# tiangexiang/OccNeRF

Hardware: AMD Instinct MI355X
Metric: rays/sec at 512x512x128spp, random-init ckpt (higher is better)
Workload: dtype f32; 1 GPU; BASELINE configs[1]: free-view frame, 512x512 image, 128 samples/ray, non-rigid motion on, seeded random-init checkpoint; synthetic SMPL-like body and camera; 183784 rays hit the body bbox (ray_mask); H2D of the ray batch and the prior and D2H of [R,5] inside the step; the frame's rays sharded over the ranks; samples whose motion-weight sum is exactly 0 are dropped after the warp (bit-identical pi; rays_per_frame=183784, samples_per_ray=128, skip_empty_samples=True, dedup_repeated_samples=False, knn_center_cache=True, warp_bone_culling=True, world_size_formed=1

## Files before the change

### include/occnerf_hip.h

```cpp
#ifndef OCCNERF_HIP_H
#define OCCNERF_HIP_H

#include <stdint.h>

#ifdef __cplusplus
extern "C" {
#endif

#define OCCNERF_ABI_VERSION 5

int occnerf_abi_version(void);
const char *occnerf_last_error(void);

int occnerf_experiment_knob(const char *name, int value);


int occnerf_grid_encode_forward(const float *inputs, const float *embeddings,
                                const int32_t *offsets, float *outputs, uint32_t B, uint32_t D,
                                uint32_t C, uint32_t L, float S, uint32_t H, float *dy_dx,
                                uint32_t gridtype, int align_corners, uint32_t interp,
                                void *stream);

int occnerf_grid_encode_backward(const float *grad, const float *inputs, const float *embeddings,
                                 const int32_t *offsets, float *grad_embeddings, uint32_t B,
                                 uint32_t D, uint32_t C, uint32_t L, float S, uint32_t H,
                                 const float *dy_dx, float *grad_inputs, uint32_t gridtype,
                                 int align_corners, uint32_t interp, void *stream);

int occnerf_grid_encode_forward_h(const float *inputs, const float *embeddings, const int32_t *offsets,
                                  const int32_t *h_offsets, float *outputs, uint32_t B, uint32_t D, uint32_t C, uint32_t L,
                                  float S, uint32_t H, float *dy_dx, uint32_t gridtype, int align_corners,
                                  uint32_t interp, void *stream);

int occnerf_grid_grad_runs(const float *grad_rows, const float *inputs, int64_t B, uint32_t D, uint32_t L, uint32_t C,
                           float *grad, void *stream);

int occnerf_grid_encode_backward_h(const float *grad, const float *inputs, const float *embeddings,
                                   const int32_t *offsets, const int32_t *h_offsets, float *grad_embeddings,
                                   uint32_t B, uint32_t D, uint32_t C, uint32_t L, float S, uint32_t H,
                                   const float *dy_dx, float *grad_inputs, uint32_t gridtype, int align_corners,
                                   uint32_t interp, void *scratch, int64_t scratch_bytes, void *stream);

int occnerf_grid_encode_forward_f16(const float *inputs, const void *embeddings, const int32_t *offsets, void *outputs,
                                    uint32_t B, uint32_t D, uint32_t C, uint32_t L, float S, uint32_t H, void *dy_dx,
                                    uint32_t gridtype, int align_corners, uint32_t interp, void *stream);
int occnerf_grid_encode_backward_f16(const void *grad, const float *inputs, const void *embeddings, const int32_t *offsets,
                                     void *grad_embeddings, uint32_t B, uint32_t D, uint32_t C, uint32_t L, float S,
                                     uint32_t H, const void *dy_dx, void *grad_inputs, uint32_t gridtype, int align_corners,
                                     uint32_t interp, void *stream);

int occnerf_grid_encode_forward_f64(const float *inputs, const double *embeddings, const int32_t *offsets, double *outputs,
                                    uint32_t B, uint32_t D, uint32_t C, uint32_t L, float S, uint32_t H, double *dy_dx,
                                    uint32_t gridtype, int align_corners, uint32_t interp, void *stream);
int occnerf_grid_encode_backward_f64(const double *grad, const float *inputs, const double *embeddings, const int32_t *offsets,
                                     double *grad_embeddings, uint32_t B, uint32_t D, uint32_t C, uint32_t L, float S,
                                     uint32_t H, const double *dy_dx, double *grad_inputs, uint32_t gridtype, int align_corners,
                                     uint32_t interp, void *stream);

int occnerf_grad_total_variation(const float *inputs, const float *embeddings, float *grad,
                                 const int32_t *offsets, float weight, uint32_t B, uint32_t D,
                                 uint32_t C, uint32_t L, float S, uint32_t H, uint32_t gridtype,
                                 int align_corners, void *stream);


int occnerf_sample_warp(const float *rays, int64_t n, int32_t S, const float *t_vals,
                        const float *t_rand, const float *Rs, const float *Ts, const float *vol,
                        int32_t nb, int32_t G, const float *h_bbox_min, const float *h_bbox_scale,
                        float *z_vals, float *pts, float *x_skel, float *mask, void *stream);
int occnerf_bone_boxes(const float *vol, int32_t nb, int32_t G, int32_t *boxes, void *stream);
int occnerf_sample_warp_culled(const float *rays, int64_t n, int32_t S, const float *t_vals,
                               const float *Rs, const float *Ts, const float *vol, int32_t nb, int32_t G,
                               const int32_t *boxes, const float *h_bbox_min, const float *h_bbox_scale,
                               float *z_vals, float *x_skel, float *mask, void *stream);

int64_t occnerf_ray_order_temp_bytes(int64_t R);
int occnerf_ray_order(const float *dirs, int64_t R, int64_t stride, int64_t *order, void *temp, int64_t temp_bytes,
                      void *stream);

int occnerf_gen_rays(const double *h_Kinv, const double *h_R, const double *h_T, int32_t f32_camera,
                     int32_t H, int32_t W, const double *h_bbox_min, const double *h_bbox_max, float *rays8,
                     uint8_t *mask, void *stream);

int64_t occnerf_nonrigid_packed_floats(void);
int occnerf_nonrigid_pack(const float *const *h_W, const float *const *h_b, float *packed,
                          void *stream);
int occnerf_nonrigid(const float *xyz_in, int64_t N, const float *cond, const float *h_hann,
                     const float *W0, const float *b0, float *packed, float *xyz_out,
                     void *stream);
int occnerf_nonrigid_rows(float *xyz, int64_t N_max, const int32_t *rows, const int32_t *n_dev,
                          const float *cond, const float *h_hann, const float *W0, const float *b0,
                          float *packed, void *stream);
int occnerf_nonrigid_direct(const float *xyz_in, int64_t N, const float *cond, const float *h_hann,
                            const float *W0, const float *b0, float *packed, float *xyz_out,
                            void *stream);

int64_t occnerf_nonrigid_packed_bf16_bytes(void);
int occnerf_nonrigid_pack_bf16(const float *const *h_W, void *packed_bf16, void *stream);
int occnerf_nonrigid_bf16x3(const float *xyz_in, int64_t N, const float *cond, const float *h_hann,
                            const float *W0, const float *b0, float *packed, const void *packed_bf16,
                            float *xyz_out, void *stream);
int occnerf_nonrigid_bf16x3_rows(float *xyz, int64_t N_max, const int32_t *rows, const int32_t *n_dev,
                                 const float *cond, const float *h_hann, const float *W0, const float *b0,
                                 float *packed, const void *packed_bf16, void *stream);

int occnerf_msknn(const float *xyz, int64_t N, const float *points, const int32_t *index_map,
                  const int32_t *h_scale_begin, const int32_t *h_seed_from_coarser,
                  int32_t nscale, int32_t *knn_idxs, void *stream);

int occnerf_msknn_clustered(const float *xyz, const float *mask, int64_t n_rays, int32_t samples_per_ray,
                            const float *points, const float *centers,
                            const int32_t *cluster_ranges, const float *cluster_radius, int32_t ncl,
                            const float *group_centers, const int32_t *group_ranges, const float *group_radius, int32_t ngrp,
                            const int32_t *h_coarse_rows, const int32_t *h_seed_from_coarser,
                            int32_t nscale, const int32_t *query_rows, const int32_t *n_query_dev, int32_t *ray_start,
                            int32_t *knn_idxs, void *stream);
int occnerf_knn_center(const float *c, const float *points, const int32_t *index_map, const int32_t *h_scale_begin,
                       int32_t nscale, float *center_out, int32_t *idx_out, void *stream);
int occnerf_msknn_clustered_centered(const float *xyz, const float *mask, int64_t n_rays, int32_t samples_per_ray,
                                     const float *points, const float *centers,
                                     const int32_t *cluster_ranges, const float *cluster_radius, int32_t ncl,
                                     const float *group_centers, const int32_t *group_ranges, const float *group_radius, int32_t ngrp,
                                     const int32_t *h_coarse_rows, const int32_t *h_seed_from_coarser,
                                     int32_t nscale, const int32_t *query_rows, const int32_t *n_query_dev, int32_t *ray_start,
                                     const float *center, const int32_t *center_idx, int32_t *knn_idxs, void *stream);

int occnerf_knn_small(const float *q, int32_t nq, const float *s, int32_t ns, int32_t k,
                      int32_t *idx, void *stream);

int occnerf_unit_normals(const double *normals, int32_t P, double *unit, void *stream);

int occnerf_point_sdf(const float *point_cloud, const float *point_base, const double *normals,
                      const double *unit_normals, const int32_t *kidx, int32_t P,
                      double *knn_base, float *dist, void *stream);

int occnerf_point_sdf_backward(const float *point_cloud, const float *point_base, const double *normals,
                               const double *unit_normals, const int32_t *kidx, int32_t P, const double *d_knn_base,
                               const float *d_dist, float *d_point_dist, void *stream);
int32_t occnerf_point_table_stride(void);
int occnerf_point_table(const double *knn_base, const float *point_sdf, const float *learnable,
                        int32_t P, float bound, float two_bound, const float *embeddings,
                        const int32_t *offsets, const int32_t *h_offsets, uint32_t L, float S,
                        uint32_t H, float *table, void *stream);

int occnerf_point_pack(const float *point_base, const double *normals, const double *unit_normals,
                       const float *counter, const float *table, int32_t P, float *point_geo,
                       float *point_tail, void *stream);
int occnerf_sample_features(const float *xyz, int64_t N, const int32_t *knn_idxs, int32_t nscale,
                            const float *point_base, const double *normals,
                            const double *unit_normals, const float *counter,
                            const float *table, float bound, float two_bound,
                            const float *embeddings, const int32_t *offsets,
                            const int32_t *h_offsets, uint32_t L, float S, uint32_t H,
                            const int32_t *geo_idxs, const float *att_in, const int32_t *rows,
                            const int32_t *n_dev, const float *point_geo, const float *point_tail, int32_t P,
                            float *mlp_in, float *raw, float *enc_in, void *stream);
int occnerf_sample_features_centered(const float *xyz, int64_t N, const int32_t *knn_idxs, int32_t nscale,
                            const float *point_base, const double *normals,
                            const double *unit_normals, const float *counter,
                            const float *table, float bound, float two_bound,
                            const float *embeddings, const int32_t *offsets,
                            const int32_t *h_offsets, uint32_t L, float S, uint32_t H,
                            const int32_t *geo_idxs, const float *att_in, const int32_t *rows,
                            const int32_t *n_dev, const float *point_geo, const float *point_tail, int32_t P,
                            const float *center, const float *center_agg,
                                     float *mlp_in, float *raw, float *enc_in, void *stream);

int occnerf_agg_forward(const float *feats, int32_t F, const int32_t *knn, const float *atts, int64_t N, int32_t K,
                        float *agg, void *stream);
int32_t occnerf_agg_backward_slices(int64_t N);
int64_t occnerf_agg_backward_scratch_bytes(int64_t N, int32_t F);
int occnerf_agg_backward(const float *grad_agg, int32_t F, const int32_t *knn, const float *atts, int64_t N,
                         int32_t K, int32_t P, float *partial, void *scratch, int64_t scratch_bytes, void *stream);

int64_t occnerf_live_rows_temp_bytes(int64_t N);
int occnerf_live_rows(const float *mask, int64_t N, int32_t *rows, int32_t *count, void *temp,
                      int64_t temp_bytes, void *stream);
int occnerf_scatter_raw(const float *raw_c, const int32_t *rows, const int32_t *n_dev, int64_t N_max,
                        float *raw_full, void *stream);

int64_t occnerf_repeat_heads_temp_bytes(int64_t N_max);
int occnerf_repeat_heads(const void *keys, int64_t stride_dwords, int32_t key_dwords, const int32_t *rows,
                         const int32_t *n_dev, int64_t N_max, int32_t *scan, int32_t *heads, int32_t *head_count,
                         float *head_mask, void *temp, int64_t temp_bytes, void *stream);
int64_t occnerf_unique_heads_temp_bytes(int64_t cap);
int occnerf_unique_heads(const void *keys, int64_t stride_dwords, int32_t key_dwords, const int32_t *heads,
                         const int32_t *n_dev, int64_t cap, int32_t *heads_out, int32_t *count_out, int32_t *scan,
                         const int32_t *n_scan_dev, int64_t scan_cap, void *temp, int64_t temp_bytes, void *stream);
int occnerf_scatter_raw_heads(const float *raw_h, const float *raw_c, const int32_t *rows, const int32_t *n_dev,
                              const int32_t *scanA, const int32_t *scanB, int64_t N_max, float *raw_full, void *stream);
int occnerf_canonical_mlp_rows(const float *mlp_in, const int32_t *in_rows, int64_t N_max, const int32_t *n_dev,
                               const float *packed, float *raw, void *stream);

int64_t occnerf_canonical_mlp_packed_floats(void);
int occnerf_canonical_mlp_pack(const float *const *h_W, const float *const *h_b, float *packed,
                               void *stream);

int occnerf_canonical_mlp(const float *mlp_in, int64_t N, const float *packed, float *raw,
                          void *stream);
int occnerf_canonical_mlp_direct(const float *mlp_in, int64_t N, const float *packed, float *raw,
                                 void *stream);
int occnerf_canonical_mlp_counted(const float *mlp_in, int64_t N_max, const int32_t *n_dev,
                                  const float *packed, float *raw, void *stream);

int64_t occnerf_canonical_mlp_packed_bf16_bytes(void);
int occnerf_canonical_mlp_pack_bf16(const float *const *h_W, void *packed_bf16, void *stream);
int occnerf_canonical_mlp_bf16x3(const float *mlp_in, int64_t N, const float *packed,
                                 const void *packed_bf16, float *raw, int32_t variant,
                                 void *stream);
int occnerf_canonical_mlp_bf16x3_rows(const float *mlp_in, const int32_t *in_rows, int64_t N_max,
                                      const int32_t *n_dev, const float *packed, const void *packed_bf16,
                                      float *raw, int32_t variant, void *stream);

int occnerf_canonical_mlp_pack_f16(const float *const *h_W, void *packed_f16, void *stream);
int occnerf_canonical_mlp_f16x3(const float *mlp_in, const int32_t *in_rows, int64_t N_max, const int32_t *n_dev,
                                const float *packed, const void *packed_f16, float *raw, uint32_t *domain_flag,
                                void *stream);
int occnerf_nonrigid_pack_f16(const float *const *h_W, void *packed_f16, void *stream);
int occnerf_nonrigid_f16x3(const float *xyz_in, int64_t N_max, const int32_t *rows, const int32_t *n_dev,
                           const float *cond, const float *h_hann, const float *W0, const float *b0, float *packed,
                           const void *packed_f16, float *xyz_out, uint32_t *domain_flag, void *stream);

int occnerf_composite(const float *raw, const float *mask, const float *z_vals, const float *rays,
                      const float *h_bgcolor, int64_t n, int32_t S, float *rgb, float *acc,
                      float *depth, float *weights, int32_t *term, const int64_t *out_rows, void *stream);


int occnerf_linear_pack(const float *W, const float *b, int32_t out_dim, int32_t in_dim, const int32_t *row_map,
                        int32_t n_pad, const int32_t *col_map, int32_t k_pad, int32_t bf16, void *Wp, void *Wt,
                        float *bias_p, void *stream);
int occnerf_linear_forward(const void *x0, int64_t ld0, int32_t k0, const void *x1, int64_t ld1, int32_t k1,
                           const void *W, const float *bias, int32_t relu, const void *mask, int64_t ldm, void *y,
                           int64_t ldy, int32_t out_f32, int32_t n_store, float *aux, int32_t aux_col,
                           int64_t aux_stride, int64_t M, int32_t n_pad, int32_t bf16, void *stream);
int32_t occnerf_linear_wgrad_slices(int64_t M);
int occnerf_linear_wgrad(const void *dz, int64_t lddz, int32_t n_pad, const void *x, int64_t ldx, int32_t k_pad,
                         int64_t M, int32_t bf16, float *part, float *dbpart, void *stream);
int occnerf_linear_wgrad_reduce(const float *part, const float *dbpart, int32_t G, int32_t n_pad, int32_t k_pad,
                                const int32_t *row_map, const int32_t *col_map, float *dW, int32_t in_dim, float *db,
                                int32_t accumulate, void *stream);

int64_t occnerf_trunks_packed_bytes(void);
int occnerf_trunks_pack_bf16(const float *const *h_W, void *packed, void *stream);
int occnerf_trunks_forward_bf16(const float *agg, const float *var, const float *enc, int64_t M, const float *packed_f32,
                                const void *packed_bf16, void *X0, void *const *h_A, void *GEO, void *const *h_B, float *raw4,
                                void *stream);

int occnerf_composite_backward(const float *raw, const float *mask, const float *z_vals, const float *rays,
                               const float *h_bgcolor, int64_t n, int32_t S, const float *g_rgb, const float *g_acc,
                               const float *g_depth, float *d_raw, float *d_mask, void *stream);

int32_t occnerf_warp_backward_slices(int64_t n_samples);
int occnerf_warp_backward(const float *rays, int64_t n, int32_t S, const float *z_vals, const float *g_mask,
                          const float *Rs, const float *Ts, const float *vol, int32_t nb, int32_t G,
                          const float *h_bbox_min, const float *h_bbox_scale, float *d_vol_part, float *d_rt_part,
                          void *stream);

int occnerf_agg_weights(const float *counter, const int32_t *knn, int64_t N, int32_t K, float *atts, float *var,
                        void *stream);

int occnerf_pose_motion_bases_backward(const float *const *h_W, const float *const *h_b, const float *posevec,
                                       const float *dst_Rs, const float *dst_Ts, const float *cnl_gtfms,
                                       const float *dRs, const float *dTs, float *const *h_dW, float *const *h_db,
                                       void *stream);

int occnerf_pose_motion_bases(const float *const *h_W, const float *const *h_b, const float *posevec, int32_t refine,
                              const float *dst_Rs, const float *dst_Ts, const float *cnl_gtfms, float *Rs, float *Ts,
                              void *stream);
int occnerf_prior_softmax(const float *decoded, const float *prior, int32_t C, int64_t V, float *vol, void *stream);
int occnerf_pack_rays(const float *rays, const float *near, const float *far, const int64_t *order, int64_t R, float *rays8,
                      void *stream);

int occnerf_assemble_image(const float *rgb, const float *alpha, const int64_t *ray_index, int64_t R, int32_t height,
                           int32_t width, const float *h_bgcolor01, uint8_t *out_rgb, uint8_t *out_alpha, void *stream);

int occnerf_convt3d_col2im(const float *cols, const float *bias, int32_t Cout, int32_t D, int32_t H, int32_t W,
                           float *out, void *stream);
int occnerf_convt3d_im2col(const float *gy, int32_t Cout, int32_t D, int32_t H, int32_t W, float *dcols, void *stream);

int32_t occnerf_adam_table_row_bytes(void);
int occnerf_adam_step(const void *table, int32_t n_tensors, const int32_t *chunks, int32_t n_chunks,
                      int32_t chunk_elems, double beta1, double beta2, double eps, double max_grad_norm, float *scratch,
                      void *stream);

int64_t occnerf_lpips_packed_floats(void);
int64_t occnerf_lpips_workspace_floats(int32_t N, int32_t H, int32_t W);
int occnerf_lpips_pack(const float *const *h_conv_w, const float *const *h_conv_b, const float *const *h_lin,
                       const float *shift, const float *scale, float *packed, void *stream);
int occnerf_lpips_forward(const float *packed, const float *in0, const float *in1, int32_t N, int32_t H, int32_t W,
                          int32_t in_nhwc, float *work, float *val, float *res, void *stream);
int occnerf_lpips_backward(const float *packed, float *work, int32_t N, int32_t H, int32_t W, int32_t in_nhwc,
                           const float *gres, float *d_in0, float *d_in1, void *stream);

int occnerf_patch_assemble(const float *rgb, const int32_t *row_of_pix, int64_t R, int32_t n_patches, int32_t size,
                           const float *h_bgcolor01, float *img, void *stream);
int occnerf_patch_assemble_backward(const float *d_img, const int32_t *pix_of_row, int64_t R, float *d_rgb, void *stream);

int32_t occnerf_patch_batch_max_patches(void);
int occnerf_patch_batch(const uint8_t *image, const uint8_t *alpha, const float *rays8, const uint8_t *box_mask, int32_t H,
                        int32_t W, int32_t n_patches, int32_t size, const double *h_u, double subject_ratio,
                        const float *h_bgcolor, int32_t *row_counts, float *rays, float *near, float *far, float *target_rgbs,
                        float *target_patches, uint8_t *patch_masks, int32_t *patch_div_indices, int32_t *xy_min,
                        int32_t *pix_of_row, int32_t *row_of_pix, int32_t *n_rows, void *stream);

int occnerf_whole_frame_count(const uint8_t *box_mask, int32_t H, int32_t W, int32_t *row_start, void *stream);
int occnerf_whole_frame_gather(const uint8_t *image, const uint8_t *alpha, const float *rays8, const uint8_t *box_mask,
                               int32_t H, int32_t W, const float *h_bgcolor, const int32_t *row_start, int32_t R,
                               int64_t *ray_index, float *rays, float *near, float *far, float *target_rgbs,
                               double *ray_alpha, uint8_t *truth_u8, float *gt_vis, float *gt_alpha, void *stream);

int occnerf_view_frame_gather(const float *rays8, const uint8_t *box_mask, int32_t H, int32_t W, const int32_t *row_start,
                              int32_t R, int64_t *ray_index, float *rays, float *near, float *far, void *stream);

#define OCCNERF_FRAME_METRICS_RECORD 14
int64_t occnerf_frame_metrics_workspace_bytes(int32_t N, int32_t H, int32_t W);
int occnerf_frame_metrics(const uint8_t *pred, const uint8_t *truth, const float *alpha, const uint8_t *body,
                          const float *gt_vis_alpha, const float *gt_alpha, int32_t N, int32_t H, int32_t W,
                          double data_range, double *record, double *ssim_map, void *workspace, void *stream);

#ifdef __cplusplus
}
#endif
#endif
```

### occnerf_amd/_lib.py

```python
import ctypes as C
import os

_HERE = os.path.dirname(os.path.abspath(__file__))
LIB_PATH = os.environ.get('OCCNERF_HIP_LIB') or os.path.join(_HERE, 'liboccnerf_hip.so')

ABI_VERSION = 5

_vp, _i32, _i64, _u32, _f32 = C.c_void_p, C.c_int32, C.c_int64, C.c_uint32, C.c_float

SIGNATURES = {
    'occnerf_abi_version': (C.c_int, []),
    'occnerf_last_error': (C.c_char_p, []),
    'occnerf_experiment_knob': (C.c_int, [C.c_char_p, C.c_int]),
    'occnerf_grid_encode_forward': (C.c_int, [_vp, _vp, _vp, _vp, _u32, _u32, _u32, _u32, _f32, _u32,
                                               _vp, _u32, C.c_int, _u32, _vp]),
    'occnerf_grid_encode_backward': (C.c_int, [_vp, _vp, _vp, _vp, _vp, _u32, _u32, _u32, _u32, _f32,
                                                _u32, _vp, _vp, _u32, C.c_int, _u32, _vp]),
    'occnerf_grid_grad_runs': (C.c_int, [_vp, _vp, _i64, _u32, _u32, _u32, _vp, _vp]),
    'occnerf_grid_encode_forward_h': (C.c_int, [_vp, _vp, _vp, _vp, _vp, _u32, _u32, _u32, _u32, _f32, _u32,
                                                 _vp, _u32, C.c_int, _u32, _vp]),
    'occnerf_grid_encode_backward_h': (C.c_int, [_vp, _vp, _vp, _vp, _vp, _vp, _u32, _u32, _u32, _u32, _f32,
                                                  _u32, _vp, _vp, _u32, C.c_int, _u32, _vp, _i64, _vp]),
    'occnerf_grid_encode_forward_f16': (C.c_int, [_vp, _vp, _vp, _vp, _u32, _u32, _u32, _u32, _f32, _u32,
                                                   _vp, _u32, C.c_int, _u32, _vp]),
    'occnerf_grid_encode_backward_f16': (C.c_int, [_vp, _vp, _vp, _vp, _vp, _u32, _u32, _u32, _u32, _f32,
                                                    _u32, _vp, _vp, _u32, C.c_int, _u32, _vp]),
    'occnerf_grid_encode_forward_f64': (C.c_int, [_vp, _vp, _vp, _vp, _u32, _u32, _u32, _u32, _f32, _u32,
                                                   _vp, _u32, C.c_int, _u32, _vp]),
    'occnerf_grid_encode_backward_f64': (C.c_int, [_vp, _vp, _vp, _vp, _vp, _u32, _u32, _u32, _u32, _f32,
                                                    _u32, _vp, _vp, _u32, C.c_int, _u32, _vp]),
    'occnerf_trunks_packed_bytes': (_i64, []),
    'occnerf_trunks_pack_bf16': (C.c_int, [_vp, _vp, _vp]),
    'occnerf_trunks_forward_bf16': (C.c_int, [_vp, _vp, _vp, _i64, _vp, _vp, _vp, _vp, _vp, _vp, _vp, _vp]),
    'occnerf_grad_total_variation': (C.c_int, [_vp, _vp, _vp, _vp, _f32, _u32, _u32, _u32, _u32, _f32,
                                                _u32, _u32, C.c_int, _vp]),
    'occnerf_sample_warp': (C.c_int, [_vp, _i64, _i32, _vp, _vp, _vp, _vp, _vp, _i32, _i32, _vp, _vp,
                                       _vp, _vp, _vp, _vp, _vp]),
    'occnerf_bone_boxes': (C.c_int, [_vp, _i32, _i32, _vp, _vp]),
    'occnerf_sample_warp_culled': (C.c_int, [_vp, _i64, _i32, _vp, _vp, _vp, _vp, _i32, _i32, _vp, _vp, _vp, _vp, _vp, _vp, _vp]),
    'occnerf_nonrigid_packed_floats': (_i64, []),
    'occnerf_nonrigid_pack': (C.c_int, [_vp, _vp, _vp, _vp]),
    'occnerf_nonrigid': (C.c_int, [_vp, _i64, _vp, _vp, _vp, _vp, _vp, _vp, _vp]),
    'occnerf_nonrigid_direct': (C.c_int, [_vp, _i64, _vp, _vp, _vp, _vp, _vp, _vp, _vp]),
    'occnerf_nonrigid_packed_bf16_bytes': (_i64, []),
    'occnerf_nonrigid_pack_bf16': (C.c_int, [_vp, _vp, _vp]),
    'occnerf_nonrigid_bf16x3': (C.c_int, [_vp, _i64, _vp, _vp, _vp, _vp, _vp, _vp, _vp, _vp]),
    'occnerf_nonrigid_bf16x3_rows': (C.c_int, [_vp, _i64, _vp, _vp, _vp, _vp, _vp, _vp, _vp, _vp, _vp]),
    'occnerf_msknn': (C.c_int, [_vp, _i64, _vp, _vp, _vp, _vp, _i32, _vp, _vp]),
    'occnerf_msknn_clustered': (C.c_int, [_vp, _vp, _i64, _i32, _vp, _vp, _vp, _vp, _i32, _vp, _vp, _vp, _i32, _vp, _vp, _i32,
                                           _vp, _vp, _vp, _vp, _vp]),
    'occnerf_msknn_clustered_centered': (C.c_int, [_vp, _vp, _i64, _i32, _vp, _vp, _vp, _vp, _i32, _vp, _vp, _vp, _i32, _vp, _vp, _i32,
                                           _vp, _vp, _vp, _vp, _vp, _vp, _vp]),
    'occnerf_knn_center': (C.c_int, [_vp, _vp, _vp, _vp, _i32, _vp, _vp, _vp]),
    'occnerf_knn_small': (C.c_int, [_vp, _i32, _vp, _i32, _i32, _vp, _vp]),
    'occnerf_unit_normals': (C.c_int, [_vp, _i32, _vp, _vp]),
    'occnerf_point_sdf': (C.c_int, [_vp, _vp, _vp, _vp, _vp, _i32, _vp, _vp, _vp]),
    'occnerf_ray_order_temp_bytes': (_i64, [_i64]),
    'occnerf_ray_order': (C.c_int, [_vp, _i64, _i64, _vp, _vp, _i64, _vp]),
    'occnerf_point_sdf_backward': (C.c_int, [_vp, _vp, _vp, _vp, _vp, _i32, _vp, _vp, _vp, _vp]),
    'occnerf_gen_rays': (C.c_int, [_vp, _vp, _vp, _i32, _i32, _i32, _vp, _vp, _vp, _vp, _vp]),
    'occnerf_agg_forward': (C.c_int, [_vp, _i32, _vp, _vp, _i64, _i32, _vp, _vp]),
    'occnerf_agg_backward_slices': (_i32, [_i64]),
    'occnerf_agg_backward_scratch_bytes': (_i64, [_i64, _i32]),
    'occnerf_agg_backward': (C.c_int, [_vp, _i32, _vp, _vp, _i64, _i32, _i32, _vp, _vp, _i64, _vp]),
    'occnerf_live_rows_temp_bytes': (_i64, [_i64]),
    'occnerf_live_rows': (C.c_int, [_vp, _i64, _vp, _vp, _vp, _i64, _vp]),
    'occnerf_scatter_raw': (C.c_int, [_vp, _vp, _vp, _i64, _vp, _vp]),
    'occnerf_repeat_heads_temp_bytes': (_i64, [_i64]),
    'occnerf_repeat_heads': (C.c_int, [_vp, _i64, _i32, _vp, _vp, _i64, _vp, _vp, _vp, _vp, _vp, _i64, _vp]),
    'occnerf_unique_heads_temp_bytes': (_i64, [_i64]),
    'occnerf_unique_heads': (C.c_int, [_vp, _i64, _i32, _vp, _vp, _i64, _vp, _vp, _vp, _vp, _i64, _vp, _i64, _vp]),
    'occnerf_scatter_raw_heads': (C.c_int, [_vp, _vp, _vp, _vp, _vp, _vp, _i64, _vp, _vp]),
    'occnerf_canonical_mlp_rows': (C.c_int, [_vp, _vp, _i64, _vp, _vp, _vp, _vp]),
    'occnerf_canonical_mlp_counted': (C.c_int, [_vp, _i64, _vp, _vp, _vp, _vp]),
    'occnerf_nonrigid_rows': (C.c_int, [_vp, _i64, _vp, _vp, _vp, _vp, _vp, _vp, _vp, _vp]),
    'occnerf_point_table_stride': (_i32, []),
    'occnerf_point_table': (C.c_int, [_vp, _vp, _vp, _i32, _f32, _f32, _vp, _vp, _vp, _u32, _f32, _u32, _vp,
                                       _vp]),
    'occnerf_point_pack': (C.c_int, [_vp, _vp, _vp, _vp, _vp, _i32, _vp, _vp, _vp]),
    'occnerf_sample_features': (C.c_int, [_vp, _i64, _vp, _i32, _vp, _vp, _vp, _vp, _vp, _f32, _f32, _vp,
                                           _vp, _vp, _u32, _f32, _u32, _vp, _vp, _vp, _vp, _vp, _vp, _i32, _vp, _vp,
                                           _vp, _vp]),
    'occnerf_sample_features_centered': (C.c_int, [_vp, _i64, _vp, _i32, _vp, _vp, _vp, _vp, _vp, _f32, _f32, _vp,
                                                    _vp, _vp, _u32, _f32, _u32, _vp, _vp, _vp, _vp, _vp, _vp, _i32, _vp, _vp,
                                                    _vp, _vp, _vp, _vp]),
    'occnerf_canonical_mlp_packed_floats': (_i64, []),
    'occnerf_canonical_mlp_pack': (C.c_int, [_vp, _vp, _vp, _vp]),
    'occnerf_canonical_mlp': (C.c_int, [_vp, _i64, _vp, _vp, _vp]),
    'occnerf_canonical_mlp_direct': (C.c_int, [_vp, _i64, _vp, _vp, _vp]),
    'occnerf_canonical_mlp_packed_bf16_bytes': (_i64, []),
    'occnerf_canonical_mlp_pack_bf16': (C.c_int, [_vp, _vp, _vp]),
    'occnerf_canonical_mlp_bf16x3': (C.c_int, [_vp, _i64, _vp, _vp, _vp, _i32, _vp]),
    'occnerf_canonical_mlp_pack_f16': (C.c_int, [_vp, _vp, _vp]),
    'occnerf_canonical_mlp_f16x3': (C.c_int, [_vp, _vp, _i64, _vp, _vp, _vp, _vp, _vp, _vp]),
    'occnerf_nonrigid_pack_f16': (C.c_int, [_vp, _vp, _vp]),
    'occnerf_nonrigid_f16x3': (C.c_int, [_vp, _i64, _vp, _vp, _vp, _vp, _vp, _vp, _vp, _vp, _vp, _vp, _vp]),
    'occnerf_canonical_mlp_bf16x3_rows': (C.c_int, [_vp, _vp, _i64, _vp, _vp, _vp, _vp, _i32, _vp]),
    'occnerf_composite': (C.c_int, [_vp, _vp, _vp, _vp, _vp, _i64, _i32, _vp, _vp, _vp, _vp, _vp, _vp, _vp]),
    'occnerf_linear_pack': (C.c_int, [_vp, _vp, _i32, _i32, _vp, _i32, _vp, _i32, _i32, _vp, _vp, _vp, _vp]),
    'occnerf_linear_forward': (C.c_int, [_vp, _i64, _i32, _vp, _i64, _i32, _vp, _vp, _i32, _vp, _i64, _vp, _i64, _i32,
                                          _i32, _vp, _i32, _i64, _i64, _i32, _i32, _vp]),
    'occnerf_linear_wgrad_slices': (_i32, [_i64]),
    'occnerf_linear_wgrad': (C.c_int, [_vp, _i64, _i32, _vp, _i64, _i32, _i64, _i32, _vp, _vp, _vp]),
    'occnerf_linear_wgrad_reduce': (C.c_int, [_vp, _vp, _i32, _i32, _i32, _vp, _vp, _vp, _i32, _vp, _i32, _vp]),
    'occnerf_composite_backward': (C.c_int, [_vp, _vp, _vp, _vp, _vp, _i64, _i32, _vp, _vp, _vp, _vp, _vp, _vp]),
    'occnerf_warp_backward_slices': (_i32, [_i64]),
    'occnerf_warp_backward': (C.c_int, [_vp, _i64, _i32, _vp, _vp, _vp, _vp, _vp, _i32, _i32, _vp, _vp, _vp, _vp, _vp]),
    'occnerf_agg_weights': (C.c_int, [_vp, _vp, _i64, _i32, _vp, _vp, _vp]),
    'occnerf_pose_motion_bases': (C.c_int, [_vp, _vp, _vp, _i32, _vp, _vp, _vp, _vp, _vp, _vp]),
    'occnerf_pose_motion_bases_backward': (C.c_int, [_vp, _vp, _vp, _vp, _vp, _vp, _vp, _vp, _vp, _vp, _vp]),
    'occnerf_prior_softmax': (C.c_int, [_vp, _vp, _i32, _i64, _vp, _vp]),
    'occnerf_pack_rays': (C.c_int, [_vp, _vp, _vp, _vp, _i64, _vp, _vp]),
    'occnerf_assemble_image': (C.c_int, [_vp, _vp, _vp, _i64, _i32, _i32, _vp, _vp, _vp, _vp]),
    'occnerf_convt3d_col2im': (C.c_int, [_vp, _vp, _i32, _i32, _i32, _i32, _vp, _vp]),
    'occnerf_convt3d_im2col': (C.c_int, [_vp, _i32, _i32, _i32, _i32, _vp, _vp]),
    'occnerf_adam_table_row_bytes': (_i32, []),
    'occnerf_adam_step': (C.c_int, [_vp, _i32, _vp, _i32, _i32] + [C.c_double] * 4 + [_vp, _vp]),
    'occnerf_lpips_packed_floats': (_i64, []),
    'occnerf_lpips_workspace_floats': (_i64, [_i32, _i32, _i32]),
    'occnerf_lpips_pack': (C.c_int, [_vp, _vp, _vp, _vp, _vp, _vp, _vp]),
    'occnerf_lpips_forward': (C.c_int, [_vp, _vp, _vp, _i32, _i32, _i32, _i32, _vp, _vp, _vp, _vp]),
    'occnerf_lpips_backward': (C.c_int, [_vp, _vp, _i32, _i32, _i32, _i32, _vp, _vp, _vp, _vp]),
    'occnerf_patch_assemble': (C.c_int, [_vp, _vp, _i64, _i32, _i32, _vp, _vp, _vp]),
    'occnerf_patch_assemble_backward': (C.c_int, [_vp, _vp, _i64, _vp, _vp]),
    'occnerf_patch_batch_max_patches': (_i32, []),
    'occnerf_patch_batch': (C.c_int, [_vp, _vp, _vp, _vp, _i32, _i32, _i32, _i32, _vp, C.c_double, _vp] + [_vp] * 12 + [_vp]),
    'occnerf_whole_frame_count': (C.c_int, [_vp, _i32, _i32, _vp, _vp]),
    'occnerf_whole_frame_gather': (C.c_int, [_vp, _vp, _vp, _vp, _i32, _i32, _vp, _vp, _i32] + [_vp] * 9 + [_vp]),
    'occnerf_view_frame_gather': (C.c_int, [_vp, _vp, _i32, _i32, _vp, _i32, _vp, _vp, _vp, _vp, _vp]),
    'occnerf_frame_metrics_workspace_bytes': (_i64, [_i32, _i32, _i32]),
    'occnerf_frame_metrics': (C.c_int, [_vp, _vp, _vp, _vp, _vp, _vp, _i32, _i32, _i32, C.c_double, _vp, _vp, _vp, _vp]),
}

_lib = None


def lib():
    global _lib
    if _lib is None:
        if not os.path.exists(LIB_PATH):
            raise ImportError(
                f'{LIB_PATH} not found: the gfx950 kernels are not built. Run '
                '`python -c "import __graft_entry__ as g; g.build()"` (or `make -C '
                'occnerf_amd/csrc`). There is no CPU fallback for this path.')
        import torch
        handle = C.CDLL(LIB_PATH)
        for name, (res, args) in SIGNATURES.items():
            fn = getattr(handle, name)
            fn.restype, fn.argtypes = res, args
        if handle.occnerf_abi_version() != ABI_VERSION:
            raise ImportError(f'liboccnerf_hip.so: ABI version {handle.occnerf_abi_version()}, this binding was written '
                              f'for {ABI_VERSION} (include/occnerf_hip.h OCCNERF_ABI_VERSION): rebuild the library')
        _lib = handle
    return _lib


def check(rc, what):
    if rc != 0:
        msg = lib().occnerf_last_error().decode(errors='replace')
        raise RuntimeError(f'{what} failed ({rc}): {msg}')
```

### occnerf_amd/config.py

```python
import argparse
import ast
import copy
import os

import yaml


class CfgNode(dict):
    def __getattr__(self, k):
        try:
            return self[k]
        except KeyError:
            raise AttributeError(k)

    def __setattr__(self, k, v):
        self[k] = v

    def get(self, k, default=None):
        return dict.get(self, k, default)

    @staticmethod
    def wrap(d):
        if isinstance(d, dict) and not isinstance(d, CfgNode):
            return CfgNode({k: CfgNode.wrap(v) for k, v in d.items()})
        return d

    def merge(self, other):
        for k, v in other.items():
            if isinstance(v, dict) and isinstance(self.get(k), dict):
                self[k].merge(v)
            else:
                self[k] = CfgNode.wrap(copy.deepcopy(v))
        return self

    def merge_from_file(self, path):
        with open(path) as f:
            return self.merge(yaml.safe_load(f) or {})

    def merge_from_list(self, opts):
        assert len(opts) % 2 == 0, 'opts must be KEY VALUE pairs'
        for key, val in zip(opts[0::2], opts[1::2]):
            node = self
            parts = key.split('.')
            for p in parts[:-1]:
                node = node[p]
            try:
                val = ast.literal_eval(val)
            except (ValueError, SyntaxError):
                pass
            node[parts[-1]] = val
        return self

    def clone(self):
        return CfgNode.wrap(copy.deepcopy(dict(self)))


_DEFAULTS = {
    'category': 'occnerf', 'task': 'zju_mocap', 'subject': 'p387', 'experiment': 'occnerf',
    'resume': False, 'eval_iter': 10000000, 'render_folder_name': '',
    'ignore_non_rigid_motions': False, 'render_skip': 1, 'render_frames': 100, 'num_workers': 4,
    'network_module': 'core.nets.occnerf.network',
    'embedder': {'module': 'core.nets.occnerf.embedders.fourier'},
    'non_rigid_embedder': {'module': 'core.nets.occnerf.embedders.hannw_fourier'},
    'canonical_mlp': {'module': 'core.nets.occnerf.canonical_mlps.occnerf_mlp', 'mlp_depth': 4,
                      'mlp_width': 256, 'multires': 10, 'i_embed': 0},
    'mweight_volume': {'module': 'core.nets.occnerf.mweight_vol_decoders.deconv_vol_decoder',
                       'embedding_size': 256, 'volume_size': 32, 'dst_voxel_size': 0.0625},
    'non_rigid_motion_mlp': {'module': 'core.nets.occnerf.non_rigid_motion_mlps.mlp_offset',
                             'condition_code_size': 69, 'mlp_width': 128, 'mlp_depth': 6,
                             'skips': [4], 'multires': 6, 'i_embed': 0, 'kick_in_iter': 100000,
                             'full_band_iter': 200000},
    'pose_decoder': {'module': 'core.nets.occnerf.pose_decoders.mlp_delta_body_pose',
                     'embedding_size': 69, 'mlp_width': 256, 'mlp_depth': 4,
                     'kick_in_iter': 2000000},
    'sex': 'neutral', 'total_bones': 24, 'bbox_offset': 0.3, 'load_net': 'latest',
    'N_samples': 128, 'perturb': 1.0, 'netchunk_per_gpu': 300000, 'chunk': 32768, 'n_gpus': 1,
    'bgcolor': [0.0, 0.0, 0.0], 'resize_img_scale': 0.5, 'show_alpha': False, 'show_truth': False,
    'patch': {'sample_subject_ratio': 0.8, 'N_patches': 6, 'size': 32},
    'freeview': {'frame_idx': 0, 'src_type': 'zju_mocap'}, 'tpose': {}, 'movement': {},
    'train': {'dataset_path': None, 'images_prescaled': False, 'seed': 0, 'prefetch': True},
    'occlude': False, 'occlusion': {'range': 405, 'mid': 451, 'width': 86},
    'eval': {'lpips': False, 'lpips_model_path': None, 'lpips_vgg16_path': None},
    'smpl_model': 'auto',
    'max_samples_per_pass': 1 << 28,
    'mlp_precision': 'fp32',
    'f16x3_domain_check': True,
    'train_fused_trunks': True,
    'skip_empty_samples': True,
    'device_rays': True,
    'device_frames': True,
    'ray_patch_order': True,
    'knn_culling': True,
    'knn_center_cache': True,
    'warp_bone_culling': True,
}

_cfg = None


def default_cfg():
    return CfgNode.wrap(copy.deepcopy(_DEFAULTS))


def get_cfg():
    global _cfg
    if _cfg is None:
        _cfg = default_cfg()
        _finish(_cfg)
    return _cfg


def set_cfg(cfg):
    global _cfg
    _cfg = cfg
    return cfg


def _finish(cfg):
    import torch
    cfg.logdir = os.path.join('experiments', cfg.category, cfg.task, cfg.subject, cfg.experiment)
    n = torch.cuda.device_count()
    cfg.n_gpus = n
    cfg.primary_gpus = [0] if n > 0 else ['cpu']
    cfg.secondary_gpus = ([g for g in range(n) if g != 0] or cfg.primary_gpus) if n > 1 \
        else cfg.primary_gpus


def make_cfg(argv=None):
    parser = argparse.ArgumentParser()
    parser.add_argument('--cfg', required=True, type=str)
    parser.add_argument('--eval', default='full', type=str)
    parser.add_argument('--type', default='skip', type=str)
    parser.add_argument('opts', default=None, nargs=argparse.REMAINDER)
    args = parser.parse_args(argv)
    cfg = default_cfg()
    here = os.path.dirname(os.path.dirname(os.path.abspath(__file__)))
    default_yaml = os.path.join(here, 'configs', 'default.yaml')
    if os.path.exists(default_yaml):
        cfg.merge_from_file(default_yaml)
    cfg.merge_from_file(args.cfg)
    cfg.merge_from_list(args.opts or [])
    _finish(cfg)
    set_cfg(cfg)
    return cfg, args
```

### occnerf_amd/csrc/common.h

```cpp
#pragma once

#include <hip/hip_runtime.h>
#include <stdint.h>

#include <cstdio>
#include <cstring>

#include "../../include/occnerf_hip.h"

#define OCC_API extern "C" __attribute__((visibility("default")))

namespace occ {

constexpr int kWave = 64;
constexpr int kNumCU = 256;

void set_error(const char *fmt, ...);

inline hipStream_t as_stream(void *s) { return reinterpret_cast<hipStream_t>(s); }

inline int check_launch(const char *what) {
    hipError_t e = hipGetLastError();
    if (e != hipSuccess) {
        set_error("%s: %s", what, hipGetErrorString(e));
        return 2;
    }
    return 0;
}

enum Knob : int { kKnobAggSlices = 0, kKnobGridXcd = 1, kKnobCount = 2 };
int knob(Knob k);

#define OCC_REQUIRE(cond, ...)         \
    do {                               \
        if (!(cond)) {                 \
            occ::set_error(__VA_ARGS__); \
            return 1;                  \
        }                              \
    } while (0)

template <typename T>
__device__ __forceinline__ T ld32(const T *base, uint32_t byte_off) {
    return *reinterpret_cast<const T *>(reinterpret_cast<const char *>(base) + byte_off);
}

constexpr int kMaxLevels = 16;

struct GridLevels {
    float scale[kMaxLevels];
    uint32_t resolution[kMaxLevels];
};

enum GridIndexMode : uint32_t { kGridDense = 0, kGridHashPow2 = 1, kGridGeneric = 2 };
struct GridModes4 {
    uint32_t mode[kMaxLevels];
};
GridModes4 make_grid_modes_d4(uint32_t L, const GridLevels &lv, const uint32_t *h_level_sizes);

GridLevels make_grid_levels(uint32_t L, float S, uint32_t H);

template <uint32_t D>
__device__ __forceinline__ uint32_t grid_index(uint32_t gridtype, bool align_corners,
                                               uint32_t hashmap_size, uint32_t resolution,
                                               const uint32_t (&pos_grid)[D]) {
    constexpr uint32_t primes[7] = {1u,          2654435761u, 805459861u, 3674653429u,
                                    2097192037u, 1434869437u, 2165219737u};
    uint32_t stride = 1, index = 0;
#pragma unroll
    for (uint32_t d = 0; d < D; d++) {
        if (stride <= hashmap_size) {
            index += pos_grid[d] * stride;
            stride *= align_corners ? resolution : (resolution + 1);
        }
    }
    if (gridtype == 0 && stride > hashmap_size) {
        uint32_t h = 0;
#pragma unroll
        for (uint32_t d = 0; d < D; d++) h ^= pos_grid[d] * primes[d];
        index = h;
    }
    return index % hashmap_size;
}

struct LevelTaps4 {
    float fr[4];
    float2 v[16];
};
__device__ __forceinline__ void encode_level_d4c2_taps(const float (&x)[4], const float2 *grid,
                                                       uint32_t hashmap_size, float scale, uint32_t resolution,
                                                       uint32_t mode, uint32_t entry0, LevelTaps4 &tp) {
    uint32_t pg[4];
#pragma unroll
    for (int d = 0; d < 4; d++) {
        float pos = __fmaf_rn(x[d], scale, 0.5f);
        const float fl = floorf(pos);
        pg[d] = (uint32_t)fl;
        pos -= fl;
        tp.fr[d] = pos;
    }
    uint32_t t[4][2];
    if (mode == kGridDense) {
        uint32_t stride = 1;
#pragma unroll
        for (int d = 0; d < 4; d++) {
            t[d][0] = pg[d] * stride;
            t[d][1] = (pg[d] + 1) * stride;
            stride *= resolution + 1;
        }
    } else if (mode == kGridHashPow2) {
        constexpr uint32_t primes[4] = {1u, 2654435761u, 805459861u, 3674653429u};
#pragma unroll
        for (int d = 0; d < 4; d++) {
            t[d][0] = pg[d] * primes[d];
            t[d][1] = (pg[d] + 1) * primes[d];
        }
    }
#pragma unroll
    for (uint32_t idx = 0; idx < 16; idx++) {
        const int b0 = idx & 1, b1 = (idx >> 1) & 1, b2 = (idx >> 2) & 1, b3 = (idx >> 3) & 1;
        uint32_t index;
        if (mode == kGridDense) {
            index = t[0][b0] + t[1][b1] + t[2][b2] + t[3][b3];
        } else if (mode == kGridHashPow2) {
            index = (t[0][b0] ^ t[1][b1] ^ t[2][b2] ^ t[3][b3]) & (hashmap_size - 1);
        } else {
            const uint32_t pl[4] = {pg[0] + b0, pg[1] + b1, pg[2] + b2, pg[3] + b3};
            index = grid_index<4>(0, false, hashmap_size, resolution, pl);
        }
        tp.v[idx] = ld32(grid, (entry0 + index) * 8u);
    }
}
__device__ __forceinline__ float2 encode_level_d4c2_reduce(const LevelTaps4 &tp) {
    float f[4][2];
#pragma unroll
    for (int d = 0; d < 4; d++) {
        f[d][0] = __fsub_rn(1.f, tp.fr[d]);
        f[d][1] = tp.fr[d];
    }
    float2 r = make_float2(0.f, 0.f);
    float w01[4];
#pragma unroll
    for (int i = 0; i < 4; i++) w01[i] = __fmul_rn(f[0][i & 1], f[1][i >> 1]);
#pragma unroll
    for (uint32_t idx = 0; idx < 16; idx++) {
        const int b0 = idx & 1, b1 = (idx >> 1) & 1, b2 = (idx >> 2) & 1, b3 = (idx >> 3) & 1;
        const float w = __fmul_rn(__fmul_rn(w01[b0 | (b1 << 1)], f[2][b2]), f[3][b3]);
        r.x = __fmaf_rn(w, tp.v[idx].x, r.x);
        r.y = __fmaf_rn(w, tp.v[idx].y, r.y);
    }
    return r;
}
__device__ __forceinline__ float2 encode_level_d4c2(const float (&x)[4], const float2 *grid,
                                                    uint32_t hashmap_size, float scale,
                                                    uint32_t resolution, uint32_t mode, uint32_t entry0 = 0) {
    LevelTaps4 tp;
    encode_level_d4c2_taps(x, grid, hashmap_size, scale, resolution, mode, entry0, tp);
    return encode_level_d4c2_reduce(tp);
}

__device__ __forceinline__ float norm3(float x, float y, float z) {
    return sqrtf(__fmaf_rn(z, z, __fmaf_rn(y, y, __fmul_rn(x, x))));
}

int64_t mlp_lds_packed_floats();
int mlp_lds_pack(const float *const *h_W, const float *const *h_b, float *packed, hipStream_t st);
int mlp_lds_launch(const float *mlp_in, const int32_t *in_rows, int64_t N, const int32_t *n_dev, const float *packed,
                   float *raw, hipStream_t st);

int64_t nr_lds_packed_floats();
int nr_lds_pack(const float *const *h_W, const float *const *h_b, float *packed, hipStream_t st);
int nr_lds_launch(const float *xyz_in, int64_t N, const int32_t *rows, const int32_t *n_dev, const float *cond,
                  const float *h_hann, const float *W0, const float *b0, float *packed, float *xyz_out,
                  hipStream_t st);

}
```

### occnerf_amd/csrc/compact.hip

```cpp
#include "common.h"

#include <hipcub/hipcub.hpp>

namespace occ {

struct LivePredicate {
    const float *mask;
    __device__ bool operator()(const int &i) const { return mask[i] != 0.0f; }
};

__global__ void scatter_raw_kernel(const float *__restrict__ raw_c, const int32_t *__restrict__ rows,
                                   const int32_t *__restrict__ n_dev, float *__restrict__ raw_full) {
    const int64_t m = (int64_t)blockIdx.x * blockDim.x + threadIdx.x;
    if (m >= (int64_t)*n_dev) return;
    const int64_t n = rows[m];
#pragma unroll
    for (int c = 0; c < 5; c++) raw_full[n * 5 + c] = raw_c[m * 5 + c];
}

struct RepeatFlag {
    const uint32_t *keys;
    int64_t stride;
    int K;
    const int32_t *rows;
    const int32_t *n_dev;
    __device__ int operator()(const int &m) const {
        if (m >= *n_dev) return 0;
        if (m == 0) return 1;
        const uint32_t *a = keys + (rows ? (int64_t)rows[m] : (int64_t)m) * stride;
        const uint32_t *b = keys + (rows ? (int64_t)rows[m - 1] : (int64_t)(m - 1)) * stride;
        if (((K | (int)stride) & 3) == 0) {
            for (int k = 0; k < K; k += 4) {
                const uint4 x = *reinterpret_cast<const uint4 *>(a + k), y = *reinterpret_cast<const uint4 *>(b + k);
                if (x.x != y.x || x.y != y.y || x.z != y.z || x.w != y.w) return 1;
            }
            return 0;
        }
        for (int k = 0; k < K; k++)
            if (a[k] != b[k]) return 1;
        return 0;
    }
};

__global__ void repeat_flags_wide_kernel(const uint4 *__restrict__ keys, int64_t stride4, int K4,
                                         const int32_t *__restrict__ rows, const int32_t *__restrict__ n_dev,
                                         int64_t N_max, int32_t *__restrict__ flags) {
    const int g = threadIdx.x & 7;
    const int64_t m = ((int64_t)blockIdx.x * blockDim.x + threadIdx.x) >> 3;
    if (m >= N_max) return;
    const int64_t n = *n_dev;
    int diff = 0;
    if (m < n && m > 0) {
        const uint4 *a = keys + (rows ? (int64_t)rows[m] : m) * stride4;
        const uint4 *b = keys + (rows ? (int64_t)rows[m - 1] : m - 1) * stride4;
        for (int k = g; k < K4; k += 8) {
            const uint4 x = a[k], y = b[k];
            diff |= (x.x != y.x) | (x.y != y.y) | (x.z != y.z) | (x.w != y.w);
        }
    }
    diff |= __shfl_xor(diff, 1, 8);
    diff |= __shfl_xor(diff, 2, 8);
    diff |= __shfl_xor(diff, 4, 8);
    if (g == 0) flags[m] = m >= n ? 0 : (m == 0 ? 1 : diff);
}

__global__ void repeat_heads_kernel(const int32_t *__restrict__ scan, const int32_t *__restrict__ rows,
                                    const int32_t *__restrict__ n_dev, int32_t *__restrict__ heads,
                                    int32_t *__restrict__ head_count, float *__restrict__ head_mask) {
    const int64_t m = (int64_t)blockIdx.x * blockDim.x + threadIdx.x;
    const int64_t n = *n_dev;
    if (m == 0 && n <= 0) *head_count = 0;
    if (m >= n) return;
    const int32_t s = scan[m], prev = m ? scan[m - 1] : 0;
    if (s != prev) {
        const int32_t r = rows ? rows[m] : (int32_t)m;
        heads[s - 1] = r;
        if (head_mask) head_mask[r] = 1.0f;
    }
    if (m == n - 1) *head_count = s;
}

__global__ void scatter_raw_heads_kernel(const float *__restrict__ raw_h, const float *__restrict__ raw_c,
                                         const int32_t *__restrict__ rows, const int32_t *__restrict__ n_dev,
                                         const int32_t *__restrict__ scanA, const int32_t *__restrict__ scanB,
                                         float *__restrict__ raw_full) {
    const int64_t m = (int64_t)blockIdx.x * blockDim.x + threadIdx.x;
    if (m >= (int64_t)*n_dev) return;
    const int64_t n = rows[m];
    const int64_t a = scanA ? scanA[m] - 1 : m;
    const int64_t h = scanB ? scanB[a] - 1 : a;
#pragma unroll
    for (int c = 0; c < 4; c++) raw_full[n * 5 + c] = raw_h[h * 5 + c];
    raw_full[n * 5 + 4] = raw_c[a * 5 + 4];
}

__device__ __forceinline__ uint64_t mix64(uint64_t h) {
    h ^= h >> 33;
    h *= 0xff51afd7ed558ccdull;
    h ^= h >> 33;
    h *= 0xc4ceb9fe1a85ec53ull;
    h ^= h >> 33;
    return h;
}

template <int G >
__global__ void unique_insert_kernel(const uint32_t *__restrict__ keys, int64_t stride, int K,
                                     const int32_t *__restrict__ heads, const int32_t *__restrict__ n_dev,
                                     int32_t *__restrict__ table, uint32_t tmask, int32_t *__restrict__ rep) {
    const int g = threadIdx.x % G;
    const int64_t j = ((int64_t)blockIdx.x * blockDim.x + threadIdx.x) / G;
    if (j >= (int64_t)*n_dev) return;
    const uint32_t *a = keys + (heads ? (int64_t)heads[j] : j) * stride;
    uint64_t h = 0x9E3779B97F4A7C15ull * (uint64_t)(g + 1);
    for (int k = g; k < K; k += G) h = mix64(h ^ ((uint64_t)a[k] + ((uint64_t)(k + 1) << 32)));
    if (G > 1) {
        h ^= __shfl_xor(h, 1, G);
        h ^= __shfl_xor(h, 2, G);
        h ^= __shfl_xor(h, 4, G);
    }
    uint32_t slot = (uint32_t)mix64(h) & tmask;
    int32_t r = (int32_t)j;
    for (int probe = 0; probe < 32; probe++) {
        int32_t prev = 0;
        if (g == 0) prev = atomicCAS(&table[slot], -1, (int32_t)j);
        if (G > 1) prev = __shfl(prev, 0, G);
        if (prev == -1) break;
        const uint32_t *b = keys + (heads ? (int64_t)heads[prev] : (int64_t)prev) * stride;
        int diff = 0;
        for (int k = g; k < K; k += G) diff |= a[k] != b[k];
        if (G > 1) {
            diff |= __shfl_xor(diff, 1, G);
            diff |= __shfl_xor(diff, 2, G);
            diff |= __shfl_xor(diff, 4, G);
        }
        if (!diff) {
            r = prev;
            break;
        }
        slot = (slot + 1) & tmask;
    }
    if (g == 0) rep[j] = r;
}

struct IsRepresentative {
    const int32_t *rep, *n_dev;
    __device__ int operator()(const int &j) const { return j < *n_dev && rep[j] == j; }
};

__global__ void unique_finish_kernel(const int32_t *__restrict__ heads, const int32_t *__restrict__ n_dev,
                                     const int32_t *__restrict__ scan2, int32_t *__restrict__ rep,
                                     int32_t *__restrict__ heads_out, int32_t *__restrict__ count_out) {
    const int64_t j = (int64_t)blockIdx.x * blockDim.x + threadIdx.x;
    const int64_t n = *n_dev;
    if (j == 0 && n <= 0) *count_out = 0;
    if (j >= n) return;
    const int32_t r = rep[j];
    if (r == (int32_t)j) heads_out[scan2[j] - 1] = heads ? heads[j] : (int32_t)j;
    if (j == n - 1) *count_out = scan2[j];
    rep[j] = scan2[r] - 1;
}

__global__ void unique_remap_kernel(int32_t *__restrict__ scan, const int32_t *__restrict__ n_scan_dev,
// ... 2 lines not shown
    if (m >= (int64_t)*n_scan_dev) return;
    scan[m] = pos[scan[m] - 1] + 1;
}

}

OCC_API int64_t occnerf_repeat_heads_temp_bytes(int64_t N) {
    using namespace occ;
    if (N <= 0 || N >= (1ll << 31)) return 0;
    size_t bytes = 0;
    hipcub::CountingInputIterator<int> it(0);
    hipcub::TransformInputIterator<int, RepeatFlag, hipcub::CountingInputIterator<int>> flags(it, RepeatFlag{});
    if (hipcub::DeviceScan::InclusiveSum(nullptr, bytes, flags, (int *)nullptr, (int)N, (hipStream_t)0) != hipSuccess)
        return -1;
    size_t bytes2 = 0;
    if (hipcub::DeviceScan::InclusiveSum(nullptr, bytes2, (int *)nullptr, (int *)nullptr, (int)N, (hipStream_t)0) != hipSuccess)
        return -1;
    return (int64_t)(bytes > bytes2 ? bytes : bytes2);
}

OCC_API int occnerf_repeat_heads(const void *keys, int64_t stride_dwords, int32_t key_dwords, const int32_t *rows,
                                 const int32_t *n_dev, int64_t N_max, int32_t *scan, int32_t *heads,
                                 int32_t *head_count, float *head_mask, void *temp, int64_t temp_bytes,
                                 void *stream) {
    using namespace occ;
    OCC_REQUIRE(keys && n_dev && scan && heads && head_count && temp, "repeat_heads: null argument");
    OCC_REQUIRE(N_max > 0 && N_max < (1ll << 31), "repeat_heads: N=%lld out of range", (long long)N_max);
    OCC_REQUIRE(key_dwords > 0 && stride_dwords >= key_dwords, "repeat_heads: key of %d dwords in rows of %lld",
                key_dwords, (long long)stride_dwords);
    size_t bytes = (size_t)temp_bytes;
    hipError_t e;
    if (key_dwords >= 32 && ((key_dwords | stride_dwords) & 3) == 0) {
        const int64_t fblocks = (N_max * 8 + 255) / 256;
        OCC_REQUIRE(fblocks < (1ll << 31), "repeat_heads: N too large");
        hipLaunchKernelGGL(repeat_flags_wide_kernel, dim3((unsigned)fblocks), dim3(256), 0, as_stream(stream),
                           reinterpret_cast<const uint4 *>(keys), stride_dwords / 4, key_dwords / 4, rows, n_dev, N_max, scan);
        e = hipcub::DeviceScan::InclusiveSum(temp, bytes, scan, scan, (int)N_max, as_stream(stream));
    } else {
        hipcub::CountingInputIterator<int> it(0);
        hipcub::TransformInputIterator<int, RepeatFlag, hipcub::CountingInputIterator<int>> flags(
            it, RepeatFlag{reinterpret_cast<const uint32_t *>(keys), stride_dwords, key_dwords, rows, n_dev});
        e = hipcub::DeviceScan::InclusiveSum(temp, bytes, flags, scan, (int)N_max, as_stream(stream));
    }
    OCC_REQUIRE(e == hipSuccess, "repeat_heads: %s", hipGetErrorString(e));
    const int64_t blocks = (N_max + 255) / 256;
    hipLaunchKernelGGL(repeat_heads_kernel, dim3((unsigned)blocks), dim3(256), 0, as_stream(stream), scan, rows, n_dev,
                       heads, head_count, head_mask);
    return check_launch("repeat_heads");
}

static inline int64_t unique_table_entries(int64_t cap) {
    int64_t t = 1024;
    while (t < cap) t <<= 1;
    return t;
}

OCC_API int64_t occnerf_unique_heads_temp_bytes(int64_t cap) {
    using namespace occ;
    if (cap <= 0 || cap >= (1ll << 30)) return 0;
    size_t bytes = 0;
    hipcub::CountingInputIterator<int> it(0);
    hipcub::TransformInputIterator<int, IsRepresentative, hipcub::CountingInputIterator<int>> flags(it, IsRepresentative{});
    if (hipcub::DeviceScan::InclusiveSum(nullptr, bytes, flags, (int *)nullptr, (int)cap, (hipStream_t)0) != hipSuccess)
        return -1;
    const int64_t words = unique_table_entries(cap) + 2 * ((cap + 63) & ~63ll);
    return words * 4 + (int64_t)((bytes + 255) & ~(size_t)255);
}

OCC_API int occnerf_unique_heads(const void *keys, int64_t stride_dwords, int32_t key_dwords, const int32_t *heads,
                                 const int32_t *n_dev, int64_t cap, int32_t *heads_out, int32_t *count_out,
                                 int32_t *scan, const int32_t *n_scan_dev, int64_t scan_cap, void *temp,
                                 int64_t temp_bytes, void *stream) {
    using namespace occ;
    OCC_REQUIRE(keys && n_dev && heads_out && count_out && temp, "unique_heads: null argument");
    OCC_REQUIRE(cap > 0 && cap < (1ll << 30), "unique_heads: cap=%lld out of range", (long long)cap);
    OCC_REQUIRE(key_dwords > 0 && stride_dwords >= key_dwords, "unique_heads: key of %d dwords in rows of %lld", key_dwords,
                (long long)stride_dwords);
    OCC_REQUIRE(!scan == !n_scan_dev, "unique_heads: scan and its length come together");
    OCC_REQUIRE(temp_bytes >= occnerf_unique_heads_temp_bytes(cap), "unique_heads: temp too small");
    const int64_t T = unique_table_entries(cap), capr = (cap + 63) & ~63ll;
    int32_t *table = reinterpret_cast<int32_t *>(temp), *rep = table + T, *scan2 = rep + capr;
    void *cub_temp = scan2 + capr;
    size_t cub_bytes = (size_t)temp_bytes - (size_t)(T + 2 * capr) * 4;
    hipStream_t st = as_stream(stream);
    OCC_REQUIRE(hipMemsetAsync(table, 0xFF, (size_t)T * 4, st) == hipSuccess, "unique_heads: memset");
    const uint32_t *k32 = reinterpret_cast<const uint32_t *>(keys);
    if (key_dwords >= 32)
        hipLaunchKernelGGL(unique_insert_kernel<8>, dim3((unsigned)((cap * 8 + 255) / 256)), dim3(256), 0, st, k32,
                           stride_dwords, key_dwords, heads, n_dev, table, (uint32_t)(T - 1), rep);
    else
        hipLaunchKernelGGL(unique_insert_kernel<1>, dim3((unsigned)((cap + 255) / 256)), dim3(256), 0, st, k32,
                           stride_dwords, key_dwords, heads, n_dev, table, (uint32_t)(T - 1), rep);
    hipcub::CountingInputIterator<int> it(0);
    hipcub::TransformInputIterator<int, IsRepresentative, hipcub::CountingInputIterator<int>> flags(
        it, IsRepresentative{rep, n_dev});
    const hipError_t e = hipcub::DeviceScan::InclusiveSum(cub_temp, cub_bytes, flags, scan2, (int)cap, st);
    OCC_REQUIRE(e == hipSuccess, "unique_heads: %s", hipGetErrorString(e));
    hipLaunchKernelGGL(unique_finish_kernel, dim3((unsigned)((cap + 255) / 256)), dim3(256), 0, st, heads, n_dev, scan2, rep,
                       heads_out, count_out);
    if (scan)
        hipLaunchKernelGGL(unique_remap_kernel, dim3((unsigned)((scan_cap + 255) / 256)), dim3(256), 0, st, scan, n_scan_dev,
                           rep);
    return check_launch("unique_heads");
}

OCC_API int occnerf_scatter_raw_heads(const float *raw_h, const float *raw_c, const int32_t *rows, const int32_t *n_dev,
                                      const int32_t *scanA, const int32_t *scanB, int64_t N_max, float *raw_full,
                                      void *stream) {
    using namespace occ;
    if (N_max <= 0) return 0;
    OCC_REQUIRE(raw_h && raw_c && rows && n_dev && raw_full, "scatter_raw_heads: null argument");
    const int64_t blocks = (N_max + 255) / 256;
    OCC_REQUIRE(blocks < (1ll << 31), "scatter_raw_heads: N too large");
    hipLaunchKernelGGL(scatter_raw_heads_kernel, dim3((unsigned)blocks), dim3(256), 0, as_stream(stream), raw_h, raw_c,
                       rows, n_dev, scanA, scanB, raw_full);
    return check_launch("scatter_raw_heads");
}

OCC_API int64_t occnerf_live_rows_temp_bytes(int64_t N) {
    using namespace occ;
    if (N <= 0 || N >= (1ll << 31)) return 0;
    size_t bytes = 0;
    hipcub::CountingInputIterator<int> it(0);
    if (hipcub::DeviceSelect::If(nullptr, bytes, it, (int *)nullptr, (int *)nullptr, (int)N, LivePredicate{nullptr},
                                 (hipStream_t)0) != hipSuccess)
        return -1;
    return (int64_t)bytes;
}

OCC_API int occnerf_live_rows(const float *mask, int64_t N, int32_t *rows, int32_t *count, void *temp,
                              int64_t temp_bytes, void *stream) {
    using namespace occ;
    OCC_REQUIRE(mask && rows && count && temp, "live_rows: null argument");
    OCC_REQUIRE(N > 0 && N < (1ll << 31), "live_rows: N=%lld out of range", (long long)N);
    size_t bytes = (size_t)temp_bytes;
    hipcub::CountingInputIterator<int> it(0);
    const hipError_t e = hipcub::DeviceSelect::If(temp, bytes, it, rows, count, (int)N, LivePredicate{mask},
                                                  as_stream(stream));
    OCC_REQUIRE(e == hipSuccess, "live_rows: %s", hipGetErrorString(e));
    return check_launch("live_rows");
}

OCC_API int occnerf_scatter_raw(const float *raw_c, const int32_t *rows, const int32_t *n_dev, int64_t N_max,
                                float *raw_full, void *stream) {
    using namespace occ;
    if (N_max <= 0) return 0;
    OCC_REQUIRE(raw_c && rows && n_dev && raw_full, "scatter_raw: null argument");
    const int64_t blocks = (N_max + 255) / 256;
    OCC_REQUIRE(blocks < (1ll << 31), "scatter_raw: N too large");
    hipLaunchKernelGGL(scatter_raw_kernel, dim3((unsigned)blocks), dim3(256), 0, as_stream(stream), raw_c, rows, n_dev,
                       raw_full);
    return check_launch("scatter_raw");
}
```

### occnerf_amd/csrc/features.hip

```cpp
#include "common.h"

#include <cstdlib>

namespace occ {

constexpr int kKnn = 10;
constexpr int kTableCols = 36;
constexpr int kTableStride = 64;

__device__ __forceinline__ double cos3_unit(const float (&a)[3], const double *__restrict__ un) {
    float na = norm3(a[0], a[1], a[2]);
    na = na < 1e-8f ? 1e-8f : na;
    const double t0 = __dmul_rn((double)__fdiv_rn(a[0], na), un[0]);
    const double t1 = __dmul_rn((double)__fdiv_rn(a[1], na), un[1]);
    const double t2 = __dmul_rn((double)__fdiv_rn(a[2], na), un[2]);
    return __dadd_rn(__dadd_rn(t0, t1), t2);
}

__global__ void unit_normals_kernel(const double *__restrict__ normals, int P,
                                    double *__restrict__ unit) {
    const int i = blockIdx.x * blockDim.x + threadIdx.x;
    if (i >= P) return;
    const double b0 = normals[i * 3], b1 = normals[i * 3 + 1], b2 = normals[i * 3 + 2];
    double nb = __dsqrt_rn(__dadd_rn(__dadd_rn(__dmul_rn(b0, b0), __dmul_rn(b1, b1)), __dmul_rn(b2, b2)));
// ... 218 lines not shown
            }
        }
        float dist = __fdiv_rn(dsum, (float)kKnn);
        if (2 * neg > kKnn) dist = -dist;
        float nd = __fdiv_rn(__fadd_rn(dist, 0.2f), 0.5f);
        nd = nd < 0.0f ? 0.0f : (nd > 1.0f ? 1.0f : nd);
        float x[4];
#pragma unroll
        for (int c = 0; c < 3; c++) x[c] = (float)__ddiv_rn(num[c], den);
        x[3] = nd;
        if (enc_in_out) {
#pragma unroll
            for (int c = 0; c < 4; c++) enc_in_out[i * 4 + c] = x[c];
        }
        raw[i * 5 + 4] = dist;

        float *out = mlp_in + i * 68;

        bool oob = false;
#pragma unroll
        for (int d = 0; d < 4; d++) oob |= (x[d] < 0.f || x[d] > 1.f);
        for (int l = 0; l < prm.L; l++) {
            float2 v = make_float2(0.f, 0.f);
            if (!oob) {
                const uint32_t o0 = (uint32_t)offsets[l];
                v = encode_level_d4c2(x, embeddings + o0, (uint32_t)offsets[l + 1] - o0,
                                      lv.scale[l], lv.resolution[l], gm.mode[l]);
            }
            *reinterpret_cast<float2 *>(out + 36 + l * 2) = v;
        }

        float att[4 * kKnn];
        float amin = INFINITY;
#pragma unroll
        for (int j = 0; j < 4 * kKnn; j++) {
            att[j] = j < nk ? (att_in ? att_in[i * nk + j] : counter[id[j]]) : INFINITY;
            amin = fminf(amin, att[j]);
        }
        float amax = -INFINITY;
#pragma unroll
        for (int j = 0; j < 4 * kKnn; j++) {
            if (j < nk) {
                att[j] = __fadd_rn(att[j], __fsub_rn(1.0f, amin));
                amax = fmaxf(amax, att[j]);
            }
        }
        float mean = 0.0f;
#pragma unroll
        for (int j = 0; j < 4 * kKnn; j++) {
            if (j < nk) {
                att[j] = __fdiv_rn(att[j], amax);
                mean = __fadd_rn(mean, att[j]);
            }
        }
        mean = __fdiv_rn(mean, (float)nk);
        float var = 0.0f, smax = -INFINITY;
#pragma unroll
        for (int j = 0; j < 4 * kKnn; j++) {
            if (j < nk) {
                const float dlt = __fsub_rn(att[j], mean);
                var = __fadd_rn(var, __fmul_rn(dlt, dlt));
                smax = fmaxf(smax, att[j]);
            }
        }
        var = __fdiv_rn(var, (float)(nk - 1));
        float ssum = 0.0f;
#pragma unroll
        for (int j = 0; j < 4 * kKnn; j++) {
            if (j < nk) {
                att[j] = expf(__fsub_rn(att[j], smax));
                ssum = __fadd_rn(ssum, att[j]);
            }
        }
        float agg[kTableCols];
#pragma unroll
        for (int f = 0; f < kTableCols; f++) agg[f] = 0.0f;
#pragma unroll
        for (int j = 0; j < 4 * kKnn; j++) {
            if (j < nk) {
                const float a = __fdiv_rn(att[j], ssum);
                const float4 *row = table + (size_t)id[j] * (kTableStride / 4);
#pragma unroll
                for (int v = 0; v < kTableCols / 4; v++) {
                    const float4 t = row[v];
                    agg[v * 4 + 0] = __fadd_rn(agg[v * 4 + 0], __fmul_rn(a, t.x));
                    agg[v * 4 + 1] = __fadd_rn(agg[v * 4 + 1], __fmul_rn(a, t.y));
                    agg[v * 4 + 2] = __fadd_rn(agg[v * 4 + 2], __fmul_rn(a, t.z));
                    agg[v * 4 + 3] = __fadd_rn(agg[v * 4 + 3], __fmul_rn(a, t.w));
                }
            }
        }
        agg[35] = var;
#pragma unroll
        for (int v = 0; v < kTableCols / 4; v++)
            *reinterpret_cast<float4 *>(out + v * 4) =
                make_float4(agg[v * 4], agg[v * 4 + 1], agg[v * 4 + 2], agg[v * 4 + 3]);
    }
}


__global__ void point_pack_kernel(const float *__restrict__ point_base, const double *__restrict__ normals,
                                  const double *__restrict__ unit, const float *__restrict__ counter,
                                  const float *__restrict__ table, int P, float *__restrict__ geo,
                                  float4 *__restrict__ tailc) {
    const int i = blockIdx.x * blockDim.x + threadIdx.x;
    if (i >= P) return;
    float *r = geo + (size_t)i * 16;
    r[0] = point_base[i * 3], r[1] = point_base[i * 3 + 1], r[2] = point_base[i * 3 + 2], r[3] = 0.0f;
    double *d = reinterpret_cast<double *>(r + 4);
    d[0] = normals[i * 3], d[1] = normals[i * 3 + 1], d[2] = normals[i * 3 + 2];
    d[3] = unit[i * 3], d[4] = unit[i * 3 + 1], d[5] = unit[i * 3 + 2];
    const float *t = table + (size_t)i * kTableStride + 32;
    tailc[i] = make_float4(t[0], t[1], t[2], counter[i]);
}

__device__ __forceinline__ float grp_sum8(float v) {
    v += __shfl_xor(v, 1, 8);
    v += __shfl_xor(v, 2, 8);
    v += __shfl_xor(v, 4, 8);
    return v;
}
__device__ __forceinline__ float grp_min8(float v) {
    v = fminf(v, __shfl_xor(v, 1, 8));
    v = fminf(v, __shfl_xor(v, 2, 8));
    return fminf(v, __shfl_xor(v, 4, 8));
}
__device__ __forceinline__ float grp_max8(float v) {
    v = fmaxf(v, __shfl_xor(v, 1, 8));
    v = fmaxf(v, __shfl_xor(v, 2, 8));
    return fmaxf(v, __shfl_xor(v, 4, 8));
}

template <int Q>
__device__ __forceinline__ float quad_bcast(float v) {
    return __builtin_bit_cast(float, __builtin_amdgcn_mov_dpp(__builtin_bit_cast(int, v), Q * 0x55, 0xf, 0xf, true));
}
template <int Q>
__device__ __forceinline__ double quad_bcast_f64(float lo, float hi) {
    return __hiloint2double(__builtin_amdgcn_mov_dpp(__builtin_bit_cast(int, hi), Q * 0x55, 0xf, 0xf, true),
                            __builtin_amdgcn_mov_dpp(__builtin_bit_cast(int, lo), Q * 0x55, 0xf, 0xf, true));
}

constexpr int kLdsTailPoints = 9216;

template <bool GENERIC ,
          bool LDS_TAIL >
__global__ __launch_bounds__(LDS_TAIL ? 768 : 256, 3) void sample_features8_kernel(
    const float *__restrict__ xyz, int64_t N_max, const int32_t *__restrict__ knn_idxs,
    const float4 *__restrict__ geo , const float4 *__restrict__ tailc ,
    const float4 *__restrict__ table, const float2 *__restrict__ embeddings,
    LevelRecs levels, LevelRecs8 levels8, FeatParams prm, const int32_t *__restrict__ rows ,
    const int32_t *__restrict__ n_dev , float *__restrict__ mlp_in, float *__restrict__ raw, float *__restrict__ enc_in_out,
    const float *__restrict__ center ,
    const float *__restrict__ center_agg ) {
    constexpr int NK = 4 * kKnn;
    float ccx = 0.f, ccy = 0.f, ccz = 0.f, cr2 = 0.f;
    if (center) ccx = center[0], ccy = center[1], ccz = center[2], cr2 = center[3];
    __shared__ float4 s_tail[LDS_TAIL ? kLdsTailPoints : 1];
    __shared__ float4 s_out[LDS_TAIL ? 768 : 256];
    static_assert(sizeof(float4) * (size_t)kLdsTailPoints + sizeof(float4) * 768 <= 160 * 1024,
                  "sample_features8_kernel<LDS_TAIL>: (tail, count) image + per-lane encoding slots exceed gfx950's 160 KiB of LDS");
    if constexpr (LDS_TAIL) {
        for (int i = threadIdx.x; i < prm.P; i += blockDim.x) s_tail[i] = tailc[i];
        __syncthreads();
    }
    const int g = threadIdx.x & 7;
    const int lane64 = threadIdx.x & 63;
    const int tr = ((lane64 & 7) << 3) | (lane64 >> 3);
    const int64_t N = n_dev ? (int64_t)*n_dev : N_max;
    if (N <= 0) return;
    const int64_t group0 = ((int64_t)blockIdx.x * blockDim.x + threadIdx.x) >> 3;
    const int64_t ngroups = ((int64_t)gridDim.x * blockDim.x) >> 3;
    const int64_t iters = (N + ngroups - 1) / ngroups;

    struct StageA {
        float p[3];
        int idg, id89;
        int id5[5];
    };
    auto out_row = [&](int64_t it) {
        const int64_t i_raw = group0 + it * ngroups;
        return i_raw < N ? i_raw : N - 1;
    };
    auto load_a = [&](int64_t i, StageA &a) {
        const int32_t *id = knn_idxs + i * NK;
        struct __attribute__((packed, aligned(4))) F3 { float v[3]; };
        struct __attribute__((packed, aligned(4))) I4 { int v[4]; };
        const F3 pq = *reinterpret_cast<const F3 *>(xyz + i * 3);
        a.p[0] = pq.v[0], a.p[1] = pq.v[1], a.p[2] = pq.v[2];
        a.idg = id[g];
        a.id89 = id[8 + (g >> 2)];
        const I4 q = *reinterpret_cast<const I4 *>(id + g * 5);
        a.id5[0] = q.v[0], a.id5[1] = q.v[1], a.id5[2] = q.v[2], a.id5[3] = q.v[3];
        a.id5[4] = id[g * 5 + 4];
    };
    StageA cur, nxt;
    int32_t i1;
    {
        const int64_t o0 = out_row(0), o1 = out_row(1);
        load_a(rows ? (int64_t)rows[o0] : o0, cur);
        i1 = rows ? rows[o1] : (int32_t)o1;
    }
    for (int64_t it = 0; it < iters; it++) {
        const bool live = group0 + it * ngroups < N;
        const int64_t o = out_row(it);
        const int64_t o2 = out_row(it + 2);
        float *out = mlp_in + o * 68;

        bool cached_agg = false;
        if (cr2 > 0.0f) {
            const float dx = cur.p[0] - ccx, dy = cur.p[1] - ccy, dz = cur.p[2] - ccz;
            const bool inside = __builtin_fmaf(dz, dz, __builtin_fmaf(dy, dy, dx * dx)) < cr2;
            cached_agg = __builtin_amdgcn_ballot_w64(live && !inside) == 0;
        }
        float4 tl[5];
#pragma unroll
        for (int k = 0; k < 5; k++) tl[k] = make_float4(0.f, 0.f, 0.f, 0.f);
        if (!cached_agg) {
#pragma unroll
            for (int k = 0; k < 5; k++) tl[k] = LDS_TAIL ? s_tail[cur.id5[k]] : ld32(tailc, (uint32_t)cur.id5[k] * 16u);
        }

        float nrm[5];
        int negf[5];
        double t_att[2] = {0.0, 0.0}, t_num[2][3] = {{0.0, 0.0, 0.0}, {0.0, 0.0, 0.0}};
        {
            float4 pc[5];
#pragma unroll
            for (int k = 0; k < 5; k++) {
                const int nid = k < 4 ? __shfl(cur.idg, 2 * k + (g >> 2), 8) : cur.id89;
                pc[k] = ld32(geo, (uint32_t)nid * 64u + (uint32_t)(g & 3) * 16u);
            }
#pragma unroll
            for (int k = 0; k < 5; k++) {
                const float nbr[3] = {quad_bcast<0>(pc[k].x), quad_bcast<0>(pc[k].y), quad_bcast<0>(pc[k].z)};
                const double nx = quad_bcast_f64<1>(pc[k].x, pc[k].y), ny = quad_bcast_f64<1>(pc[k].z, pc[k].w);
                const double nz = quad_bcast_f64<2>(pc[k].x, pc[k].y);
                float dir[3];
#pragma unroll
                for (int c = 0; c < 3; c++) dir[c] = __fsub_rn(cur.p[c], nbr[c]);
                double dot = __dadd_rn(0.0, __dmul_rn((double)dir[0], nx));
                dot = __dadd_rn(dot, __dmul_rn((double)dir[1], ny));
                dot = __dadd_rn(dot, __dmul_rn((double)dir[2], nz));
                negf[k] = dot < 0.0;
                nrm[k] = norm3(dir[0], dir[1], dir[2]);
                if (k < 2) {
                    const double un[3] = {quad_bcast_f64<2>(pc[k].z, pc[k].w), quad_bcast_f64<3>(pc[k].x, pc[k].y),
                                          quad_bcast_f64<3>(pc[k].z, pc[k].w)};
                    t_att[k] = fabs(cos3_unit(dir, un));
#pragma unroll
                    for (int c = 0; c < 3; c++) {
                        const float pn = __fdiv_rn(__fadd_rn(nbr[c], prm.bound), prm.two_bound);
                        t_num[k][c] = __dmul_rn(t_att[k], (double)pn);
                    }
                }
            }
        }
        float dsum = 0.0f;
        int neg = 0;
#pragma unroll
        for (int j = 0; j < kKnn; j++) {
            dsum = __fadd_rn(dsum, __shfl(nrm[j >> 1], 4 * (j & 1), 8));
            neg += __shfl(negf[j >> 1], 4 * (j & 1), 8);
        }
        double num[3] = {0.0, 0.0, 0.0}, den = 0.0;
#pragma unroll
        for (int j = 0; j < 3; j++) {
#pragma unroll
            for (int c = 0; c < 3; c++) num[c] = __dadd_rn(num[c], __shfl(t_num[j >> 1][c], 4 * (j & 1), 8));
            den = __dadd_rn(den, __shfl(t_att[j >> 1], 4 * (j & 1), 8));
        }
        float dist = __fdiv_rn(dsum, (float)kKnn);
        if (2 * neg > kKnn) dist = -dist;
        float nd = __fdiv_rn(__fadd_rn(dist, 0.2f), 0.5f);
        nd = nd < 0.0f ? 0.0f : (nd > 1.0f ? 1.0f : nd);
        float x[4];
#pragma unroll
        for (int c = 0; c < 3; c++) x[c] = (float)__ddiv_rn(num[c], den);
        x[3] = nd;
        if (live && g == 0) {
            raw[o * 5 + 4] = dist;
            if (enc_in_out) *reinterpret_cast<float4 *>(enc_in_out + o * 4) = make_float4(x[0], x[1], x[2], x[3]);
        }

        float a5[5] = {0.f, 0.f, 0.f, 0.f, 0.f};
        float var = 0.0f;
        float tail[3] = {0.f, 0.f, 0.f};
        if (!cached_agg) {
            float lmin = INFINITY;
#pragma unroll
            for (int k = 0; k < 5; k++) {
                a5[k] = tl[k].w;
                lmin = fminf(lmin, a5[k]);
            }
            const float amin = grp_min8(lmin);
            float lmax = -INFINITY;
#pragma unroll
            for (int k = 0; k < 5; k++) {
                a5[k] = __fadd_rn(a5[k], __fsub_rn(1.0f, amin));
                lmax = fmaxf(lmax, a5[k]);
            }
            const float amax = grp_max8(lmax);
            float lsum = 0.0f;
#pragma unroll
            for (int k = 0; k < 5; k++) {
                a5[k] = __fdiv_rn(a5[k], amax);
                lsum += a5[k];
            }
            const float mean = __fdiv_rn(grp_sum8(lsum), (float)NK);
            float lvar = 0.0f, lsm = -INFINITY;
#pragma unroll
            for (int k = 0; k < 5; k++) {
                const float dl = a5[k] - mean;
                lvar += dl * dl;
                lsm = fmaxf(lsm, a5[k]);
            }
            var = __fdiv_rn(grp_sum8(lvar), (float)(NK - 1));
            const float smax = grp_max8(lsm);
            float le = 0.0f;
#pragma unroll
            for (int k = 0; k < 5; k++) {
                a5[k] = expf(__fsub_rn(a5[k], smax));
                le += a5[k];
            }
            const float ssum = grp_sum8(le);
#pragma unroll
            for (int k = 0; k < 5; k++) a5[k] = __fdiv_rn(a5[k], ssum);

#pragma unroll
            for (int k = 0; k < 5; k++) {
                tail[0] += a5[k] * tl[k].x;
                tail[1] += a5[k] * tl[k].y;
                tail[2] += a5[k] * tl[k].z;
            }
        }

        bool cached_enc = false;
        if (cached_agg) {
            const bool eq = __float_as_uint(x[0]) == __float_as_uint(center_agg[36]) && __float_as_uint(x[1]) == __float_as_uint(center_agg[37]) &&
                            __float_as_uint(x[2]) == __float_as_uint(center_agg[38]) && __float_as_uint(x[3]) == __float_as_uint(center_agg[39]);
            cached_enc = __builtin_amdgcn_ballot_w64(live && !eq) == 0;
        }
        float2 ev[2];
        int32_t i2;
        if (!cached_enc) {
            LevelTaps4 tp[2];
            bool oob = false;
            float xt[4];
#pragma unroll
            for (int d = 0; d < 4; d++) xt[d] = __shfl(x[d], tr);
#pragma unroll
            for (int d = 0; d < 4; d++) oob |= (xt[d] < 0.f || xt[d] > 1.f);
            __builtin_amdgcn_sched_barrier(0);
            if (oob) {
#pragma unroll
                for (int d = 0; d < 4; d++) xt[d] = 0.5f;
            }
#pragma unroll
            for (int a = 0; a < 2; a++) {
                if constexpr (GENERIC) {
                    const LevelRec4 lr = levels.r[2 * (lane64 >> 3) + a];
                    encode_level_d4c2_taps(xt, embeddings, lr.size, lr.scale, lr.res_mode & 0xFFFFFFu, lr.res_mode >> 24,
                                           lr.entry0, tp[a]);
                } else {
                    level_taps_select(xt, embeddings, levels8.r[2 * (lane64 >> 3) + a], tp[a]);
                }
            }
            load_a(i1, nxt);
            i2 = rows ? rows[o2] : (int32_t)o2;
            __builtin_amdgcn_sched_barrier(0);
            float2 evt[2];
#pragma unroll
            for (int a = 0; a < 2; a++) {
                evt[a] = encode_level_d4c2_reduce(tp[a]);
                if (oob) evt[a] = make_float2(0.f, 0.f);
            }
#pragma unroll
            for (int a = 0; a < 2; a++) ev[a] = make_float2(__shfl(evt[a].x, tr), __shfl(evt[a].y, tr));
        } else {
            load_a(i1, nxt);
            i2 = rows ? rows[o2] : (int32_t)o2;
            const float4 ce = *reinterpret_cast<const float4 *>(center_agg + 40 + 4 * g);
            ev[0] = make_float2(ce.x, ce.y), ev[1] = make_float2(ce.z, ce.w);
        }
        s_out[threadIdx.x] = make_float4(ev[0].x, ev[0].y, ev[1].x, ev[1].y);

        float agg[4] = {0.f, 0.f, 0.f, 0.f};
        if (!cached_agg) {
            const uint32_t piece = (uint32_t)g * 16u;
            auto issue_chunk = [&](int c, float4 (&t)[10]) {
#pragma unroll
                for (int h = 0; h < 2; h++) {
#pragma unroll
                    for (int k = 0; k < 5; k++)
#ifdef OCC_FEAT_EXP_RESIDENT_ROWS
                        t[h * 5 + k] = ld32(table, (uint32_t)(__shfl(cur.id5[k], 2 * c + h, 8) & 15) * (uint32_t)(kTableStride * 4) + piece);
#else
                        t[h * 5 + k] = ld32(table, (uint32_t)__shfl(cur.id5[k], 2 * c + h, 8) * (uint32_t)(kTableStride * 4) + piece);
#endif
                }
            };
            float4 b0[10], b1[10], b2[10];
            issue_chunk(0, b0);
            issue_chunk(1, b1);
    #pragma unroll 1
            for (int c = 0; c < 4; c++) {
                const int cn = c + 2 < 4 ? c + 2 : 3;
                issue_chunk(cn, b2);
#pragma unroll
                for (int h = 0; h < 2; h++) {
#pragma unroll
                    for (int k = 0; k < 5; k++) {
                        const float w = __shfl(a5[k], 2 * c + h, 8);
                        const float4 t = b0[h * 5 + k];
                        agg[0] = __fadd_rn(agg[0], __fmul_rn(w, t.x));
                        agg[1] = __fadd_rn(agg[1], __fmul_rn(w, t.y));
                        agg[2] = __fadd_rn(agg[2], __fmul_rn(w, t.z));
                        agg[3] = __fadd_rn(agg[3], __fmul_rn(w, t.w));
                    }
                }
#pragma unroll
                for (int k = 0; k < 10; k++) b0[k] = b1[k], b1[k] = b2[k];
            }
#pragma unroll
            for (int c = 0; c < 3; c++) tail[c] = grp_sum8(tail[c]);
        } else {
            const float4 ca = *reinterpret_cast<const float4 *>(center_agg + 4 * g);
            agg[0] = ca.x, agg[1] = ca.y, agg[2] = ca.z, agg[3] = ca.w;
            tail[0] = center_agg[32], tail[1] = center_agg[33], tail[2] = center_agg[34], var = center_agg[35];
        }
        if (live) {
            *reinterpret_cast<float4 *>(out + 4 * g) = make_float4(agg[0], agg[1], agg[2], agg[3]);
            if (g == 0) *reinterpret_cast<float4 *>(out + 32) = make_float4(tail[0], tail[1], tail[2], var);
            *reinterpret_cast<float4 *>(out + 36 + 4 * g) = s_out[threadIdx.x];
        }
        cur = nxt;
        i1 = i2;
    }
}


}

OCC_API int occnerf_unit_normals(const double *normals, int32_t P, double *unit, void *stream) {
    using namespace occ;
    OCC_REQUIRE(normals && unit, "unit_normals: null argument");
    if (P <= 0) return 0;
    hipLaunchKernelGGL(unit_normals_kernel, dim3((P + 255) / 256), dim3(256), 0, as_stream(stream), normals, P, unit);
    return check_launch("unit_normals");
}

OCC_API int occnerf_point_sdf(const float *point_cloud, const float *point_base,
                              const double *normals, const double *unit_normals,
                              const int32_t *kidx, int32_t P, double *knn_base, float *dist,
                              void *stream) {
    using namespace occ;
    OCC_REQUIRE(point_cloud && point_base && normals && unit_normals && kidx && knn_base && dist,
                "point_sdf: null argument");
    if (P <= 0) return 0;
    hipLaunchKernelGGL(point_sdf_kernel, dim3((P + 255) / 256), dim3(256), 0, as_stream(stream), point_cloud,
                       point_base, normals, unit_normals, kidx, P, knn_base, dist);
    return check_launch("point_sdf");
}

OCC_API int occnerf_point_sdf_backward(const float *point_cloud, const float *point_base, const double *normals,
                                       const double *unit_normals, const int32_t *kidx, int32_t P, const double *d_knn_base,
                                       const float *d_dist, float *d_point_dist, void *stream) {
    using namespace occ;
    OCC_REQUIRE(point_cloud && point_base && normals && unit_normals && kidx && d_knn_base && d_dist && d_point_dist,
                "point_sdf_backward: null argument");
    if (P <= 0) return 0;
    hipLaunchKernelGGL(point_sdf_backward_kernel, dim3((P + 255) / 256), dim3(256), 0, as_stream(stream), point_cloud, point_base,
                       normals, unit_normals, kidx, P, d_knn_base, d_dist, d_point_dist);
    return check_launch("point_sdf_backward");
}

OCC_API int32_t occnerf_point_table_stride(void) { return occ::kTableStride; }

OCC_API int occnerf_point_table(const double *knn_base, const float *point_sdf,
                                const float *learnable, int32_t P, float bound, float two_bound,
                                const float *embeddings, const int32_t *offsets,
                                const int32_t *h_offsets, uint32_t L, float S, uint32_t H, float *table,
                                void *stream) {
    using namespace occ;
    OCC_REQUIRE(knn_base && point_sdf && learnable && embeddings && offsets && table, "point_table: null argument");
    OCC_REQUIRE(L >= 1 && L <= 16, "point_table: L=%u unsupported", L);
    if (P <= 0) return 0;
    const GridLevels lv = make_grid_levels(L, S, H);
    const GridModes4 gm = modes_from_host_offsets(L, lv, h_offsets);
    hipLaunchKernelGGL(point_table_kernel, dim3((P + 255) / 256), dim3(256), 0, as_stream(stream), knn_base,
                       point_sdf, learnable, P, bound, two_bound, reinterpret_cast<const float2 *>(embeddings),
                       offsets, (int)L, lv, gm, table);
    return check_launch("point_table");
}

OCC_API int occnerf_point_pack(const float *point_base, const double *normals, const double *unit_normals,
                               const float *counter, const float *table, int32_t P, float *point_geo,
                               float *point_tail, void *stream) {
    using namespace occ;
    OCC_REQUIRE(point_base && normals && unit_normals && counter && table && point_geo && point_tail,
                "point_pack: null argument");
    if (P <= 0) return 0;
    hipLaunchKernelGGL(point_pack_kernel, dim3((P + 255) / 256), dim3(256), 0, as_stream(stream), point_base, normals,
                       unit_normals, counter, table, P, point_geo, reinterpret_cast<float4 *>(point_tail));
    return check_launch("point_pack");
}

OCC_API int occnerf_sample_features(const float *xyz, int64_t N, const int32_t *knn_idxs,
                                    int32_t nscale, const float *point_base, const double *normals,
                                    const double *unit_normals, const float *counter,
                                    const float *table, float bound, float two_bound,
                                    const float *embeddings, const int32_t *offsets,
                                    const int32_t *h_offsets, uint32_t L, float S, uint32_t H,
                                    const int32_t *geo_idxs,
                                    const float *att_in, const int32_t *rows, const int32_t *n_dev,
                                    const float *point_geo, const float *point_tail, int32_t P,
                                    float *mlp_in, float *raw, float *enc_in, void *stream) {
    return occnerf_sample_features_centered(xyz, N, knn_idxs, nscale, point_base, normals, unit_normals, counter, table, bound,
                                            two_bound, embeddings, offsets, h_offsets, L, S, H, geo_idxs, att_in, rows, n_dev,
                                            point_geo, point_tail, P, nullptr, nullptr, mlp_in, raw, enc_in, stream);
}

OCC_API int occnerf_sample_features_centered(const float *xyz, int64_t N, const int32_t *knn_idxs,
                                             int32_t nscale, const float *point_base, const double *normals,
                                             const double *unit_normals, const float *counter,
                                             const float *table, float bound, float two_bound,
                                             const float *embeddings, const int32_t *offsets,
                                             const int32_t *h_offsets, uint32_t L, float S, uint32_t H,
                                             const int32_t *geo_idxs,
                                             const float *att_in, const int32_t *rows, const int32_t *n_dev,
                                             const float *point_geo, const float *point_tail, int32_t P,
                                             const float *center, const float *center_agg,
                                             float *mlp_in, float *raw, float *enc_in, void *stream) {
    using namespace occ;
    OCC_REQUIRE(!center == !center_agg, "sample_features: center and center_agg come together");
    if (N <= 0) return 0;
    OCC_REQUIRE(xyz && knn_idxs && point_base && normals && unit_normals && (counter || att_in) && table &&
                    embeddings && offsets && mlp_in && raw, "sample_features: null argument");
    OCC_REQUIRE(nscale >= 1 && nscale <= 4, "sample_features: nscale=%d unsupported", nscale);
    OCC_REQUIRE(L == 16, "sample_features: built for the 16-level encoder of occnerf_mlp.py:45 (L=%u)", L);
    if (N <= 0) return 0;
    const GridLevels lv = make_grid_levels(L, S, H);
    const GridModes4 gm = modes_from_host_offsets(L, lv, h_offsets);
    FeatParams prm{bound, two_bound, nscale, (int)L, (int)P};
    OCC_REQUIRE(!n_dev || rows, "sample_features: a device-side count needs the row list");
    OCC_REQUIRE(!point_geo == !point_tail, "sample_features: point_geo and point_tail come together (occnerf_point_pack)");
    const bool lanes8 = nscale == 4 && !geo_idxs && !att_in && counter && h_offsets && point_geo;
    OCC_REQUIRE(!rows || lanes8,
                "sample_features: a row list is only supported on the renderer's path (4 scales, per-point inputs, "
                "packed point records)");
    if (lanes8) {
        LevelRecs levels;
        for (uint32_t l = 0; l < kMaxLevels; l++)
            levels.r[l] = LevelRec4{(uint32_t)h_offsets[l], (uint32_t)(h_offsets[l + 1] - h_offsets[l]), lv.scale[l],
                                    lv.resolution[l] | (gm.mode[l] << 24)};
        LevelRecs8 levels8;
        bool generic = false;
        for (uint32_t l = 0; l < kMaxLevels; l++) {
            const uint32_t size = (uint32_t)(h_offsets[l + 1] - h_offsets[l]), r1 = lv.resolution[l] + 1;
            const bool dense = gm.mode[l] == kGridDense;
            generic |= gm.mode[l] == kGridGeneric;
            levels8.r[l] = LevelRec8{(uint32_t)h_offsets[l], dense ? 0xFFFFFFFFu : size - 1, lv.scale[l], dense ? 1u : 0u,
                                     dense ? r1 : 2654435761u, dense ? r1 * r1 : 805459861u,
                                     dense ? r1 * r1 * r1 : 3674653429u, 0u};
        }
        OCC_REQUIRE(P > 0, "sample_features: P=%d rows of packed point records", P);
        const bool lds_tail = P <= kLdsTailPoints && N >= 96 * 64;
        const int threads = lds_tail ? 768 : 256;
        int64_t blocks8 = (N * 8 + threads - 1) / threads;
        const int64_t cap = lds_tail ? (int64_t)kNumCU : (int64_t)kNumCU * 32;
        if (blocks8 > cap) blocks8 = cap;
        auto kern = generic ? (lds_tail ? sample_features8_kernel<true, true> : sample_features8_kernel<true, false>)
                            : (lds_tail ? sample_features8_kernel<false, true> : sample_features8_kernel<false, false>);
        hipLaunchKernelGGL(kern, dim3((unsigned)blocks8), dim3(threads), 0, as_stream(stream), xyz,
                           N, knn_idxs, reinterpret_cast<const float4 *>(point_geo),
                           reinterpret_cast<const float4 *>(point_tail),
                           reinterpret_cast<const float4 *>(table), reinterpret_cast<const float2 *>(embeddings),
                           levels, levels8, prm, rows, n_dev, mlp_in, raw, enc_in, center, center_agg);
        return check_launch("sample_features");
    }
    OCC_REQUIRE(!center, "sample_features: the centre aggregate is only supported on the renderer's path");
    int64_t blocks = (N + 255) / 256;
    if (blocks > (int64_t)kNumCU * 16) blocks = (int64_t)kNumCU * 16;
    hipLaunchKernelGGL(sample_features_kernel, dim3((unsigned)blocks), dim3(256), 0, as_stream(stream), xyz, N,
                       knn_idxs, point_base, normals, unit_normals, counter,
                       reinterpret_cast<const float4 *>(table), reinterpret_cast<const float2 *>(embeddings),
                       offsets, lv, gm, prm, geo_idxs, att_in, mlp_in, raw, enc_in);
    return check_launch("sample_features");
}
```

### occnerf_amd/csrc/knn.hip

```cpp
#include "common.h"

#include <map>
#include <mutex>
#include <utility>

#include <cmath>
#include <vector>

namespace occ {

typedef float f32x2 __attribute__((ext_vector_type(2)));

constexpr int kK = 10;

struct KBest {
    float s[kK];
    int i[kK];
};

__device__ __forceinline__ void kbest_reset(KBest &b) {
#pragma unroll
    for (int p = 0; p < kK; p++) {
        b.s[p] = INFINITY;
        b.i[p] = 0;
// ... 216 lines not shown
            OCC_PT1(p0) OCC_PT1(p1) OCC_PT1(p2) OCC_PT1(p3)                                 \
        }                                                                                   \
    }
#define OCC_EMIT1(L)                                                                        \
    if (q.live) {                                                                           \
        struct __attribute__((packed, aligned(4))) I4 { int v[4]; };                        \
        struct __attribute__((packed, aligned(4))) I2 { int v[2]; };                        \
        int32_t *out = knn_idxs + (qi * sc.nscale + (L)) * kK;                              \
        int r_[kK];                                                                         \
        _Pragma("unroll") for (int p = 0; p < kK; p++) r_[p] = key_row(best.k[p]) & 0xFFFF; \
        *reinterpret_cast<I4 *>(out) = I4{{r_[0], r_[1], r_[2], r_[3]}};                    \
        *reinterpret_cast<I4 *>(out + 4) = I4{{r_[4], r_[5], r_[6], r_[7]}};                \
        *reinterpret_cast<I2 *>(out + 8) = I2{{r_[8], r_[9]}};                              \
    }

__device__ __forceinline__ void search_one_query(const OneQuery q, const int64_t qi, const int lane,
                                                 const float4 *__restrict__ points, const float4 *__restrict__ centers,
                                                 const int2 *__restrict__ ranges, const float *__restrict__ radius,
                                                 const float4 *__restrict__ gcenters, const int2 *__restrict__ granges,
                                                 const float *__restrict__ gradius, const ClusteredScales &sc,
                                                 int32_t *__restrict__ knn_idxs) {
    KBest64 best;
    float thr = q.live ? INFINITY : -1.0f, sb = INFINITY;
    kbest64_reset(best);
    OCC_SCAN1(sc.coarse_begin, sc.coarse_end)
    OCC_EMIT1(sc.nscale - 1)
    const unsigned long long lv = __builtin_amdgcn_ballot_w64(q.live);
    const int first = lv ? __builtin_ctzll(lv) : 0;
    const float rx = __shfl(q.x, first), ry = __shfl(q.y, first), rz = __shfl(q.z, first);
    for (int l = sc.nscale - 2; l >= 0; l--) {
        sb = sc.seed[l] ? key_dist(best.k[kK - 1]) : INFINITY;
        thr = q.live ? filter_bound(sb) : -1.0f;
        kbest64_reset(best);
        const int2 *rg = ranges + (size_t)l * sc.ncl;
        const float *rd = radius + (size_t)l * sc.ncl;
        int k_first;
        {
            float bd = INFINITY;
            int bk = 0;
            for (int k = lane; k < sc.ncl; k += kWave) {
                const float4 c = centers[k];
                const float dx = rx - c.x, dy = ry - c.y, dz = rz - c.z;
                const float d = dx * dx + dy * dy + dz * dz;
                const bool has = rg[k].x < rg[k].y;
                if (has && d < bd) {
                    bd = d;
                    bk = k;
                }
            }
#pragma unroll
            for (int o = 32; o > 0; o >>= 1) {
                const float od = __shfl_xor(bd, o);
                const int ok = __shfl_xor(bk, o);
                if (od < bd || (od == bd && ok < bk)) {
                    bd = od;
                    bk = ok;
                }
            }
            k_first = __builtin_amdgcn_readfirstlane(bk);
        }
        {
            const int2 range = rg[k_first];
            OCC_SCAN1(range.x, range.y)
        }
        auto in_reach = [&](const float4 c, const float r) -> bool {
            const float dx = q.x - c.x, dy = q.y - c.y, dz = q.z - c.z;
            const float d2 = __builtin_fmaf(dz, dz, __builtin_fmaf(dy, dy, dx * dx));
            const float lim = (sb + r) * 1.00001f;
            return __builtin_amdgcn_ballot_w64(q.live && !(d2 > lim * lim)) != 0;
        };
        const int ngrp = sc.ngrp > 0 ? sc.ngrp : 1;
        for (int gi = 0; gi < ngrp; gi++) {
            int k_lo = 0, k_hi = sc.ncl;
            if (sc.ngrp > 0) {
                const float gr = gradius[(size_t)l * sc.ngrp + gi];
                if (gr < 0.0f) continue;
                if (!in_reach(gcenters[gi], gr)) continue;
                const int2 gk = granges[gi];
                k_lo = gk.x, k_hi = gk.y;
            }
            for (int k = k_lo; k < k_hi; k++) {
                if (k == k_first) continue;
                const int2 range = rg[k];
                if (range.x >= range.y) continue;
                if (!in_reach(centers[k], rd[k])) continue;
                OCC_SCAN1(range.x, range.y)
            }
        }
        OCC_EMIT1(l)
    }
}
#undef OCC_PT1
#undef OCC_SCAN1
#undef OCC_EMIT1

constexpr float kSplitExtent2 = 0.04f;

template <bool SPLIT >
__global__ __launch_bounds__(256) void msknn_clustered_kernel(
    const float *__restrict__ xyz, const float *__restrict__ mask , int64_t n_rays, int S,
    const float4 *__restrict__ points, const float4 *__restrict__ centers,
    const int2 *__restrict__ ranges , const float *__restrict__ radius ,
    const float4 *__restrict__ gcenters , const int2 *__restrict__ granges ,
    const float *__restrict__ gradius ,
    ClusteredScales sc, int32_t *__restrict__ knn_idxs, unsigned *__restrict__ ticket,
    const int32_t *__restrict__ qrows ,
    const int32_t *__restrict__ ray_start ,
    const float *__restrict__ center ,
    const int32_t *__restrict__ center_idx ,
    const float split_extent2 ) {
    const int lane = threadIdx.x & 63;
    float ccx = 0.f, ccy = 0.f, ccz = 0.f, cr2 = 0.f;
    if (center) ccx = center[0], ccy = center[1], ccz = center[2], cr2 = center[3];
    const int tiles_per_chunk = (S + 3) / 4;
    const int64_t n_tiles = ((n_rays + 63) / 64) * tiles_per_chunk;
    for (;;) {
        unsigned t32 = 0;
        if (lane == 0) t32 = atomicAdd(ticket, 1u);
        const int64_t job = (int64_t)(unsigned)__builtin_amdgcn_readfirstlane((int)t32);
        const int64_t tile = SPLIT ? job >> 2 : job;
        const int part = SPLIT ? (int)(job & 3) : 0;
        if (tile >= n_tiles) break;
        const int64_t n_blocks = (n_rays + 63) / 64;
        const int64_t blk = qrows ? tile % n_blocks : tile / tiles_per_chunk;
        const int64_t ray = blk * 64 + lane;
        const int s0 = (int)(qrows ? tile / n_blocks : tile % tiles_per_chunk) * 4;
        int64_t qi[kQ];
        bool live[kQ];
        f32x2 qx[2], qy[2], qz[2];
        int32_t hs = 0, hn = 0;
        if (qrows) {
            const int64_t r = ray < n_rays ? ray : n_rays - 1;
            hs = ray_start[r];
            hn = ray < n_rays ? ray_start[r + 1] - hs : 0;
        }
#pragma unroll
        for (int a = 0; a < kQ; a++) {
            live[a] = ray < n_rays && (s0 + a) < S;
            const int64_t r = ray < n_rays ? ray : n_rays - 1;
            const int sm = (s0 + a) < S ? (s0 + a) : S - 1;
            qi[a] = r * S + sm;
            if (qrows) {
                live[a] = (s0 + a) < hn;
                qi[a] = live[a] ? (int64_t)qrows[hs + s0 + a] : r * S;
            }
            if (mask && mask[qi[a]] == 0.0f) live[a] = false;
            qx[a >> 1][a & 1] = xyz[qi[a] * 3 + 0];
            qy[a >> 1][a & 1] = xyz[qi[a] * 3 + 1];
            qz[a >> 1][a & 1] = xyz[qi[a] * 3 + 2];
        }
        if (cr2 > 0.0f) {
#pragma unroll
            for (int a = 0; a < kQ; a++) {
                const float dx = qx[a >> 1][a & 1] - ccx, dy = qy[a >> 1][a & 1] - ccy, dz = qz[a >> 1][a & 1] - ccz;
                const float d2 = __builtin_fmaf(dz, dz, __builtin_fmaf(dy, dy, dx * dx));
                if (live[a] && d2 < cr2) {
                    live[a] = false;
                    struct __attribute__((packed, aligned(4))) I4 { int v[4]; };
                    struct __attribute__((packed, aligned(4))) I2 { int v[2]; };
                    for (int l = 0; part == 0 && l < sc.nscale; l++) {
                        int32_t *out = knn_idxs + (qi[a] * sc.nscale + l) * kK;
                        const int32_t *ci = center_idx + l * kK;
                        *reinterpret_cast<I4 *>(out) = I4{{ci[0], ci[1], ci[2], ci[3]}};
                        *reinterpret_cast<I4 *>(out + 4) = I4{{ci[4], ci[5], ci[6], ci[7]}};
                        *reinterpret_cast<I2 *>(out + 8) = I2{{ci[8], ci[9]}};
                    }
                }
            }
        }
        if (__builtin_amdgcn_ballot_w64(live[0] || live[1] || live[2] || live[3]) == 0) continue;
        if constexpr (SPLIT) {
            float lo[3] = {INFINITY, INFINITY, INFINITY}, hi[3] = {-INFINITY, -INFINITY, -INFINITY};
#pragma unroll
            for (int a = 0; a < kQ; a++) {
                if (live[a]) {
                    const float v[3] = {qx[a >> 1][a & 1], qy[a >> 1][a & 1], qz[a >> 1][a & 1]};
#pragma unroll
                    for (int d = 0; d < 3; d++) lo[d] = fminf(lo[d], v[d]), hi[d] = fmaxf(hi[d], v[d]);
                }
            }
#pragma unroll
            for (int o = 32; o > 0; o >>= 1) {
#pragma unroll
                for (int d = 0; d < 3; d++) {
                    lo[d] = fminf(lo[d], __shfl_xor(lo[d], o));
                    hi[d] = fmaxf(hi[d], __shfl_xor(hi[d], o));
                }
            }
            const float ex = hi[0] - lo[0], ey = hi[1] - lo[1], ez = hi[2] - lo[2];
            const float ext2 = __int_as_float(__builtin_amdgcn_readfirstlane(__float_as_int(ex * ex + ey * ey + ez * ez)));
            const bool spread = ext2 > split_extent2;
            if (!spread && part != 0) continue;
            if (spread) {
                OneQuery q1{0.f, 0.f, 0.f, false};
                int64_t q1i = 0;
#pragma unroll
                for (int a = 0; a < kQ; a++) {
                    if (a == part) {
                        q1 = OneQuery{qx[a >> 1][a & 1], qy[a >> 1][a & 1], qz[a >> 1][a & 1], live[a]};
                        q1i = qi[a];
                    }
                }
                if (__builtin_amdgcn_ballot_w64(q1.live) != 0)
                    search_one_query(q1, q1i, lane, points, centers, ranges, radius, gcenters, granges, gradius, sc, knn_idxs);
                continue;
            }
        }
        KBest64 best[kQ];
        float thr[kQ], sb[kQ];

     \
#define OCC_PT4(P)                                                                          \
    {                                                                                       \
        const f32x2 dx0 = qx[0] - P.x, dy0 = qy[0] - P.y, dz0 = qz[0] - P.z;                \
        const f32x2 dx1 = qx[1] - P.x, dy1 = qy[1] - P.y, dz1 = qz[1] - P.z;                \
        const f32x2 da = __builtin_elementwise_fma(dz0, dz0, __builtin_elementwise_fma(dy0, dy0, dx0 * dx0)); \
        const f32x2 db = __builtin_elementwise_fma(dz1, dz1, __builtin_elementwise_fma(dy1, dy1, dx1 * dx1)); \
        if ((da[0] < thr[0]) | (da[1] < thr[1]) | (db[0] < thr[2]) | (db[1] < thr[3])) {    \
            const int row = __float_as_int(P.w);                                            \
            consider_lex(best[0], thr[0], sb[0], da[0], row);                               \
            consider_lex(best[1], thr[1], sb[1], da[1], row);                               \
            consider_lex(best[2], thr[2], sb[2], db[0], row);                               \
            consider_lex(best[3], thr[3], sb[3], db[1], row);                               \
        }                                                                                   \
    }
        \
#define OCC_SCAN(JB, JE)                                                                    \
    {                                                                                       \
        const int je_ = (JE);                                                               \
        int j = (JB);                                                                       \
        float4 n0 = points[j], n1 = points[j + 1], n2 = points[j + 2], n3 = points[j + 3];  \
        for (; j < je_; j += 4) {                                                           \
            const float4 p0 = n0, p1 = n1, p2 = n2, p3 = n3;                                \
            const int jn = j + 4 < je_ ? j + 4 : j;                                         \
            n0 = points[jn], n1 = points[jn + 1], n2 = points[jn + 2], n3 = points[jn + 3]; \
            OCC_PT4(p0) OCC_PT4(p1) OCC_PT4(p2) OCC_PT4(p3)                                 \
        }                                                                                   \
    }
       \
#define OCC_EMIT(L)                                                                         \
    _Pragma("unroll") for (int a = 0; a < kQ; a++) {                                        \
        if (live[a]) {                                                                      \
            struct __attribute__((packed, aligned(4))) I4 { int v[4]; };                    \
            struct __attribute__((packed, aligned(4))) I2 { int v[2]; };                    \
            int32_t *out = knn_idxs + (qi[a] * sc.nscale + (L)) * kK;                       \
            int r_[kK];                                                                     \
            _Pragma("unroll") for (int p = 0; p < kK; p++) r_[p] = key_row(best[a].k[p]) & 0xFFFF; \
            *reinterpret_cast<I4 *>(out) = I4{{r_[0], r_[1], r_[2], r_[3]}};                \
            *reinterpret_cast<I4 *>(out + 4) = I4{{r_[4], r_[5], r_[6], r_[7]}};            \
            *reinterpret_cast<I2 *>(out + 8) = I2{{r_[8], r_[9]}};                          \
        }                                                                                   \
    }

#pragma unroll
        for (int a = 0; a < kQ; a++) {
            thr[a] = live[a] ? INFINITY : -1.0f;
            sb[a] = INFINITY;
            kbest64_reset(best[a]);
        }
        OCC_SCAN(sc.coarse_begin, sc.coarse_end)
        OCC_EMIT(sc.nscale - 1)

        for (int l = sc.nscale - 2; l >= 0; l--) {
#pragma unroll
            for (int a = 0; a < kQ; a++) {
                sb[a] = sc.seed[l] ? key_dist(best[a].k[kK - 1]) : INFINITY;
                thr[a] = live[a] ? filter_bound(sb[a]) : -1.0f;
                kbest64_reset(best[a]);
            }
            const int2 *rg = ranges + (size_t)l * sc.ncl;
            const float *rd = radius + (size_t)l * sc.ncl;
            int k_first;
            {
                const float rx = __int_as_float(__builtin_amdgcn_readfirstlane(__float_as_int(qx[0][0])));
                const float ry = __int_as_float(__builtin_amdgcn_readfirstlane(__float_as_int(qy[0][0])));
                const float rz = __int_as_float(__builtin_amdgcn_readfirstlane(__float_as_int(qz[0][0])));
                float bd = INFINITY;
                int bk = 0;
                for (int k = lane; k < sc.ncl; k += kWave) {
                    const float4 c = centers[k];
                    const float dx = rx - c.x, dy = ry - c.y, dz = rz - c.z;
                    const float d = dx * dx + dy * dy + dz * dz;
                    const bool has = rg[k].x < rg[k].y;
                    if (has && d < bd) {
                        bd = d;
                        bk = k;
                    }
                }
#pragma unroll
                for (int o = 32; o > 0; o >>= 1) {
                    const float od = __shfl_xor(bd, o);
                    const int ok = __shfl_xor(bk, o);
                    if (od < bd || (od == bd && ok < bk)) {
                        bd = od;
                        bk = ok;
                    }
                }
                k_first = __builtin_amdgcn_readfirstlane(bk);
            }
            {
                const int2 range = rg[k_first];
                OCC_SCAN(range.x, range.y)
            }
            auto in_reach = [&](const float4 c, const float r) -> bool {
                bool want = false;
#pragma unroll
                for (int h = 0; h < 2; h++) {
                    const f32x2 dx = qx[h] - c.x, dy = qy[h] - c.y, dz = qz[h] - c.z;
                    const f32x2 d2 = __builtin_elementwise_fma(dz, dz, __builtin_elementwise_fma(dy, dy, dx * dx));
// ... 271 lines not shown
```

### occnerf_amd/network.py

```python
import os

import numpy as np
import torch
import torch.nn as nn

from . import geometry, ops
from .canonical_mlp import CanonicalMLP
from .config import get_cfg
from .rayorder import ray_patch_order
from .modules import (BodyPoseRefiner, MotionBasisComputer, MotionWeightVolumeDecoder,
                      NonRigidMotionMLP, hann_window_weights)


class _Replica(nn.Module):

    def __init__(self, module):
        super().__init__()
        self.module = module

    def forward(self, *a, **k):
        return self.module(*a, **k)


def _load_smpl(cfg):
# ... 76 lines not shown
    def _f16x3_enqueue_check(self, flag, what):
        self._frames_rendered = getattr(self, '_frames_rendered', 0) + 1
        host = torch.empty(1, dtype=torch.int32, pin_memory=True)
        host.copy_(flag, non_blocking=True)
        flag.zero_()
        done = torch.cuda.Event()
        done.record(torch.cuda.current_stream(flag.device))
        self.__dict__.setdefault('_f16x3_pending', []).append((done, host, f'{what} {self._frames_rendered}'))

    def check_f16x3_domain(self, wait=True):
        pending = self.__dict__.get('_f16x3_pending')
        while pending:
            done, host, frame_no = pending[0]
            if not wait and not done.query():
                return
            done.synchronize()
            pending.pop(0)
            if int(host[0]) != 0:
                pending.clear()
                raise RuntimeError(f"occnerf_amd: {frame_no} of this Network left the domain of the f16x3 kernels (a hidden activation "
                                   'reached 4 094): its results are not fp32-grade -- use mlp_precision=\'fp32\' / '
                                   "train_nonrigid_f16x3=False (a render with cfg.f16x3_domain_check=True falls back by itself, at the "
                                   'price of one wait per frame)')

    def invalidate_cache(self):
        self._ctx = self._packed = self._wconst = None
        self._ray_orders = {}
        self.__dict__.pop('_per_step_graph', None)

    def load_state_dict(self, *a, **k):
        out = super().load_state_dict(*a, **k)
        self.invalidate_cache()
        return out

    def _apply(self, fn, *a, **k):
        out = super()._apply(fn, *a, **k)
        self.invalidate_cache()
        return out

    def _context(self):
        dev = self.point_base.device
        if self._ctx is not None and self._ctx['device'] == dev:
            return self._ctx
        base = self.point_base.detach()
        P = base.shape[0]
        sets = [torch.arange(P)] + [f.long() for f in self.fps_index]
        rows, imap, begin = [], [], [0]
        for idx in sets:
            pts = base[idx.to(dev)]
            pad = (-pts.shape[0]) % 4
            rows.append(torch.cat([pts, torch.full((pad, 3), float('inf'), device=dev)]))
            imap.append(torch.cat([idx, torch.zeros(pad, dtype=idx.dtype)]))
            begin.append(begin[-1] + pts.shape[0] + pad)
        pts4 = torch.cat(rows)
        pts4 = torch.cat([pts4, torch.zeros(pts4.shape[0], 1, device=dev)], dim=1).contiguous()
        as_sets = [set(s.tolist()) for s in sets]
        seed = [int(l + 1 < len(sets) and as_sets[l + 1] <= as_sets[l]) for l in range(len(sets))]
        normals = self.point_norms.to(dev).double().contiguous()
        cl = geometry.build_knn_clusters(base.cpu().numpy(), [s.numpy() for s in sets])
        clusters = {k: (torch.from_numpy(np.ascontiguousarray(v)).to(dev) if k in
                        ('points', 'index_map', 'centers', 'ranges', 'radius', 'group_centers', 'group_ranges', 'group_radius') else v)
                    for k, v in cl.items()}
        self._ctx = {
            'clusters': clusters,
            'device': dev, 'points': pts4, 'index_map': torch.cat(imap).int().to(dev),
            'scale_begin': begin, 'seed': seed, 'normals': normals,
            'unit': ops.unit_normals(normals),
            'bound32': float(np.float32(self.bound)),
            'two_bound32': float(np.float32(2 * np.float64(self.bound))),
        }
        return self._ctx

    def _packed_weights(self):
        cm, nr = self.cnl_mlp.module, self.non_rigid_mlp.module
        nr_lin = [m for m in nr.block_mlps if isinstance(m, nn.Linear)]
        cw, cb = cm.linear_params()
        prec = str(self.cfg.get('mlp_precision', 'fp32'))
        if prec not in ('fp32', 'bf16x3', 'f16x3'):
            raise RuntimeError(f"cfg.mlp_precision must be 'fp32', 'f16x3' or 'bf16x3', got {prec!r}")
        pack_c = {'bf16x3': ops.canonical_mlp_pack_bf16, 'f16x3': ops.canonical_mlp_pack_f16}.get(prec)
        pack_n = {'bf16x3': ops.nonrigid_pack_bf16, 'f16x3': ops.nonrigid_pack_f16}.get(prec)
        srcs = cw + cb + [m.weight for m in nr_lin] + [m.bias for m in nr_lin]
        key = (prec, str(self.cfg.get('f16x3_domain_check', True))) + tuple((t.data_ptr(), t._version) for t in srcs)
        if self._packed is not None and self._packed['key'] == key:
            return self._packed
        self._packed = {
            'key': key,
            'cnl': ops.canonical_mlp_pack(cw, cb),
            'cnl_bf16': pack_c(cw) if pack_c else None,
            'nr': ops.nonrigid_pack([m.weight.detach() for m in nr_lin],
                                    [m.bias.detach() for m in nr_lin]),
            'nr_bf16': pack_n([m.weight.detach() for m in nr_lin]) if pack_n else None,
            'nr_w0': nr_lin[0].weight.detach(), 'nr_b0': nr_lin[0].bias.detach(),
            'domain_flag': torch.zeros(1, device=cw[0].device, dtype=torch.int32)
            if (prec == 'f16x3' and self.cfg.get('f16x3_domain_check', True)) else None,
        }
        return self._packed

    def _weight_constants(self):
        dec_mod = self.mweight_vol_decoder
        enc = self.cnl_mlp.module.encoder
        srcs = list(dec_mod.parameters()) + [self.point_dist, self.point_base, enc.embeddings]
        key = tuple((t.data_ptr(), t._version) for t in srcs)
        if self._wconst is not None and self._wconst['key'] == key:
            return self._wconst
        with torch.no_grad():
            dec = dec_mod.decoder.forward_gemm(dec_mod.const_embedding[None])[0].contiguous()
            table = self._point_stage(self._context())
        self._wconst = {'key': key, 'dec': dec, 'table': table}
        return self._wconst

    def _point_pack(self, wc):
        srcs = [self.point_counter, self.point_base]
        key = (wc['table'].data_ptr(),) + tuple((t.data_ptr(), t._version) for t in srcs)
        if wc.get('pack_key') != key:
            ctx = self._context()
            wc['pack'] = ops.point_pack(self.point_base.detach(), ctx['normals'], ctx['unit'],
                                        self.point_counter.detach(), wc['table'])
            wc['pack_key'] = key
        return wc['pack']

    def _point_stage(self, ctx):
        enc = self.cnl_mlp.module.encoder
        pc = self.point_cloud.detach().float().contiguous()
        base = self.point_base.detach()
        kidx = ops.knn_small(pc, base, 3)
        knn_base, sdf = ops.point_sdf(pc, base, ctx['normals'], ctx['unit'], kidx)
        table = ops.point_table(knn_base, sdf, pc, ctx['bound32'], ctx['two_bound32'],
                                enc.embeddings.detach(), enc.offsets, enc.log2_per_level_scale,
                                enc.base_resolution)
        return table

    def _stage_features(self, rays8, z, xyz, mask, pk, cond, hann, table, pack, center=None):
        cfg, ctx = self.cfg, self._context()
        S = int(cfg.N_samples)
        enc = self.cnl_mlp.module.encoder
        rows, count = ops.live_rows(mask)
        self.last_live_count = count
        dedup = bool(cfg.get('dedup_repeated_samples', True))
        scan_a = scan_b = mrows = mcount = None
        frows, fcount, kmask = rows, count, mask
        if not cfg.ignore_non_rigid_motions:
            if pk['nr_bf16'] is not None:
                ops.nonrigid_bf16x3_rows(xyz, rows, count, cond, hann, pk['nr_w0'], pk['nr_b0'], pk['nr'], pk['nr_bf16'],
                                         domain_flag=pk['domain_flag'])
            else:
                ops.nonrigid_rows(xyz, rows, count, cond, hann, pk['nr_w0'], pk['nr_b0'], pk['nr'])
        if dedup:
            scan_a, frows, fcount, kmask = ops.repeat_heads(xyz, 3, count, rows=rows,
                                                            want_mask=not cfg.get('knn_query_list', True))
            if cfg.get('dedup_global_positions', False):
                frows, fcount = ops.unique_heads(xyz, 3, frows, fcount, scan=scan_a, scan_count=count)
        self.last_head_counts = (fcount, None)
        if cfg.get('knn_query_list', True):
            knn = ops.msknn_clustered(xyz, rays8.shape[0], S, ctx['clusters'], ctx['seed'], rows=frows, count=fcount, center=center)
        else:
            knn = ops.msknn_clustered(xyz, rays8.shape[0], S, ctx['clusters'], ctx['seed'], mask=kmask, center=center)
        if center is not None and len(center) > 3 and center[3] != self._center_stamp(table):
            raise RuntimeError('stale kNN centre: its cached feature row was computed from another table / counter / embedding '
                               'version than this frame\'s (ops.sample_features freshness contract)')
        mlp_in, raw_c, _ = ops.sample_features(
            xyz, knn, self.point_base.detach(), ctx['normals'], ctx['unit'],
            self.point_counter.detach(), table, ctx['bound32'], ctx['two_bound32'],
            enc.embeddings.detach(), enc.offsets, enc.log2_per_level_scale, enc.base_resolution,
            rows=frows, count=fcount, pack=pack, center=None if center is None else center[0],
            center_agg=None if center is None else center[2])
        del knn
        if dedup:
            scan_b, mrows, mcount, _ = ops.repeat_heads(mlp_in, 68, fcount)
            if cfg.get('dedup_global', True):
                mrows, mcount = ops.unique_heads(mlp_in, 68, mrows, mcount, scan=scan_b, scan_count=fcount)
            self.last_head_counts = (fcount, mcount)
        return {'dedup': dedup, 'rays8': rays8, 'z': z, 'mask': mask, 'rows': rows, 'count': count, 'mlp_in': mlp_in,
                'raw_c': raw_c, 'scan_a': scan_a, 'scan_b': scan_b, 'mrows': mrows, 'mcount': mcount, 'cnl': pk['cnl'],
                'cnl_bf16': pk['cnl_bf16'], 'domain_flag': pk['domain_flag'], 'N': xyz.shape[0]}

    @staticmethod
    def _stage_mlp_composite(st, bgcolor, out, out_rows):
        dev, N = st['mlp_in'].device, st['N']

        def mlp(raw_out, count, in_rows=None):
            if st['cnl_bf16'] is not None:
                ops.canonical_mlp_bf16x3(st['mlp_in'], st['cnl'], st['cnl_bf16'], raw_out, count=count, in_rows=in_rows,
                                         domain_flag=st['domain_flag'])
            else:
                ops.canonical_mlp(st['mlp_in'], st['cnl'], raw_out, count=count, in_rows=in_rows)
        if st['dedup']:
            raw_h = torch.empty(st['mlp_in'].shape[0], 5, device=dev)
            mlp(raw_h, st['mcount'], st['mrows'])
            raw = ops.scatter_raw_heads(raw_h, st['raw_c'], st['rows'], st['count'], st['scan_a'], st['scan_b'],
                                        torch.zeros(N, 5, device=dev))
        else:
            mlp(st['raw_c'], st['count'])
            raw = ops.scatter_raw(st['raw_c'], st['rows'], st['count'], torch.zeros(N, 5, device=dev))
        st['mlp_in'] = None
        return ops.composite(raw, st['mask'], st['z'], st['rays8'], bgcolor, out=out, out_rows=out_rows)[:3]

    def _nonrigid_f16_pack(self):
        pk = self._packed_weights()
        if pk.get('nr_f16_train') is None:
            nr_lin = [m for m in self.non_rigid_mlp.module.block_mlps if isinstance(m, nn.Linear)]
            pk['nr_f16_train'] = pk['nr_bf16'] if (pk['nr_bf16'] is not None and pk['nr_bf16'].dtype == torch.float16) else \
                ops.nonrigid_pack_f16([m.weight.detach() for m in nr_lin])
        return pk['nr_f16_train']

    def _knn_center_lists(self, cond, hann):
        ctx, pk = self._context(), self._packed_weights()
        c = torch.zeros(64, 3, device=self.point_base.device)
        if not self.cfg.ignore_non_rigid_motions:
            c = ops.nonrigid(c, cond, hann, pk['nr_w0'], pk['nr_b0'], pk['nr'], direct=True)
        return ops.knn_center(c[0].contiguous(), ctx['points'], ctx['index_map'], ctx['scale_begin'])

    def _knn_center(self, cond, hann, table, pack):
        ctx, pk = self._context(), self._packed_weights()
        c = torch.zeros(64, 3, device=self.point_base.device)
        if not self.cfg.ignore_non_rigid_motions:
            c = ops.nonrigid(c, cond, hann, pk['nr_w0'], pk['nr_b0'], pk['nr'], direct=True)
        center, idx = ops.knn_center(c[0].contiguous(), ctx['points'], ctx['index_map'], ctx['scale_begin'])
        enc = self.cnl_mlp.module.encoder
        row, _, enc_in = ops.sample_features(
            c[:8].contiguous(), idx[None].expand(8, -1, -1).contiguous(), self.point_base.detach(), ctx['normals'], ctx['unit'],
            self.point_counter.detach(), table, ctx['bound32'], ctx['two_bound32'], enc.embeddings.detach(), enc.offsets,
            enc.log2_per_level_scale, enc.base_resolution, pack=pack, want_enc_in=True)
        return center, idx, ops.center_row(row[0], enc_in[0]), self._center_stamp(table)

    def _center_stamp(self, table):
        return (table.data_ptr(), table._version, self.point_counter._version, self.cnl_mlp.module.encoder.embeddings._version)

    def _render_rays(self, rays8, Rs, Ts, vol, bbox_min, bbox_scale, bgcolor, cond, hann,
                     table, t_rand=None, out=None, out_rows=None, pack=None, boxes=None, center=None):
        cfg, ctx = self.cfg, self._context()
        S = int(cfg.N_samples)
        enc = self.cnl_mlp.module.encoder
        t_vals = torch.linspace(0., 1., steps=S, device=rays8.device)
        z, xyz, mask, _ = ops.sample_warp(rays8, S, t_vals, Rs, Ts, vol, bbox_min, bbox_scale,
                                          t_rand=t_rand, boxes=boxes)
        pk = self._packed_weights()
        N = xyz.shape[0]
        if cfg.get('skip_empty_samples', True) and cfg.get('knn_culling', True):
            st = self._stage_features(rays8, z, xyz, mask, pk, cond, hann, table, pack, center)
            return self._stage_mlp_composite(st, bgcolor, out, out_rows)

        if not cfg.ignore_non_rigid_motions:
            if pk['nr_bf16'] is not None:
                ops.nonrigid_bf16x3(xyz, cond, hann, pk['nr_w0'], pk['nr_b0'], pk['nr'], pk['nr_bf16'], out=xyz, domain_flag=pk['domain_flag'])
            else:
                ops.nonrigid(xyz, cond, hann, pk['nr_w0'], pk['nr_b0'], pk['nr'], out=xyz)
        if cfg.get('knn_culling', True):
            knn = ops.msknn_clustered(xyz, rays8.shape[0], S, ctx['clusters'], ctx['seed'], center=center)
        else:
            knn = ops.msknn(xyz, ctx['points'], ctx['index_map'], ctx['scale_begin'], ctx['seed'])
        mlp_in, raw, _ = ops.sample_features(
            xyz, knn, self.point_base.detach(), ctx['normals'], ctx['unit'],
            self.point_counter.detach(), table, ctx['bound32'], ctx['two_bound32'],
            enc.embeddings.detach(), enc.offsets, enc.log2_per_level_scale, enc.base_resolution, pack=pack)
        del knn
        if pk['cnl_bf16'] is not None:
            ops.canonical_mlp_bf16x3(mlp_in, pk['cnl'], pk['cnl_bf16'], raw, domain_flag=pk['domain_flag'])
        else:
            ops.canonical_mlp(mlp_in, pk['cnl'], raw)
        del mlp_in
        return ops.composite(raw, mask, z, rays8, bgcolor, out=out, out_rows=out_rows)[:3]

    @staticmethod
    def _ray_patch_order(rays_d):
        return ray_patch_order(rays_d)

    @staticmethod
    def _host3(v):
        return ops.host_float3(v)

    @torch.no_grad()
    def live_samples_per_ray(self, rays, dst_Rs, dst_Ts, cnl_gtfms, motion_weights_priors, dst_posevec=None,
                             near=None, far=None, iter_val=1e7, **kwargs):
        cfg, dev = self.cfg, self.point_base.device
        f32 = lambda t: t.detach().float().contiguous().to(dev)
        wc = self._weight_constants()
        refine = iter_val >= cfg.pose_decoder.get('kick_in_iter', 0)
        Rs, Ts = ops.pose_motion_bases(self.pose_decoder, f32(dst_posevec).reshape(-1), refine, f32(dst_Rs), f32(dst_Ts),
                                       f32(cnl_gtfms))
        vol = ops.prior_softmax(wc['dec'], f32(motion_weights_priors))
        rays8 = ops.pack_rays(f32(rays).reshape(2, -1, 3), f32(near).reshape(-1), f32(far).reshape(-1), None)
        S = int(cfg.N_samples)
        t_vals = torch.linspace(0., 1., steps=S, device=dev)
        boxes = ops.bone_boxes(vol, Rs.shape[0]) if cfg.get('warp_bone_culling', True) else None
        _, _, mask, _ = ops.sample_warp(rays8, S, t_vals, Rs, Ts, vol, self._host3(kwargs['cnl_bbox_min_xyz']),
                                        self._host3(kwargs['cnl_bbox_scale_xyz']), boxes=boxes)
        return (mask.view(-1, S) != 0).sum(dim=1)

    @torch.no_grad()
    def render_preamble(self, data, iter_val=1e7):
        f32 = lambda t: t.detach().float().contiguous().to(self.point_base.device)
        wc = self._weight_constants()
        refine = iter_val >= self.cfg.pose_decoder.get('kick_in_iter', 0)
        Rs, Ts = ops.pose_motion_bases(self.pose_decoder, f32(data['dst_posevec']).reshape(-1), refine, f32(data['dst_Rs']),
                                       f32(data['dst_Ts']), f32(data['cnl_gtfms']))
        return Rs, Ts, ops.prior_softmax(wc['dec'], f32(data['motion_weights_priors']))

    def forward(self, rays, dst_Rs, dst_Ts, cnl_gtfms, motion_weights_priors, dst_posevec=None,
                near=None, far=None, iter_val=1e7, **kwargs):
        cfg = self.cfg
        dev = self.point_base.device
        if dev.type != 'cuda':
            raise RuntimeError('occnerf_amd.Network renders on a GPU only; move the module with '
                               '.cuda() first (the reference has no CPU path either)')
        dst_Rs, dst_Ts = dst_Rs[None], dst_Ts[None]
        dst_posevec, cnl_gtfms = dst_posevec[None], cnl_gtfms[None]
        motion_weights_priors = motion_weights_priors[None]
        want_grad = torch.is_grad_enabled()
        fused = not want_grad and not self.training
        R = int(near.numel())
        shape = list(rays[1].shape[:-1])
        if R == 0:
            z = torch.zeros(0, device=dev)
            return {'rgb': z.reshape(shape + [3]), 'alpha': z.reshape(shape), 'depth': z.reshape(shape),
                    'comp_loss': torch.zeros(0 if self.training else 1, device=dev)}

        nr = cfg.non_rigid_motion_mlp
        hann = hann_window_weights(nr.multires, iter_val, nr.kick_in_iter, nr.full_band_iter)
        refine = iter_val >= cfg.pose_decoder.get('kick_in_iter', 0)
# ... 118 lines not shown
```

### occnerf_amd/ops.py

```python
import ctypes as C

import numpy as np
import torch

from . import _lib

_f32p = C.POINTER(C.c_float)


def _chk(t, dtype, name):
    if not torch.is_tensor(t):
        raise RuntimeError(f'{name} must be a tensor')
    if not t.is_cuda:
        raise RuntimeError(f'{name} must be a CUDA(HIP) tensor; there is no CPU path')
    if not t.is_contiguous():
        raise RuntimeError(f'{name} must be a contiguous tensor')
    if t.dtype != dtype:
        raise RuntimeError(f'{name} must be {dtype}, got {t.dtype}')
    return t.data_ptr()


def _guard_dev(dev):
    if torch.device(dev).type != 'cuda':
        raise RuntimeError(f'tensors are on {dev}: this path runs on a GPU only, there is no CPU path')
# ... 102 lines not shown
                         dy_dx=None, grad_inputs=None, gridtype=0, align_corners=False, interp=0):
    dt = _encoder_dtype(grad, 'grid_encode_backward')
    fp32 = dt == torch.float32
    scratch = torch.empty(int(L) * int(B), device=inputs.device, dtype=torch.int64) if (fp32 and int(D) == 4 and int(Cc) == 2
                                                                                      and int(B) >= 32768) else None
    with _guard(inputs):
        args = [_chk(grad, dt, 'grad'), _chk(inputs, torch.float32, 'inputs'), _chk(embeddings, dt, 'embeddings'),
                _chk(offsets, torch.int32, 'offsets')]
        if fp32:
            args.append(_host_offsets(offsets))
        args += [_chk(grad_embeddings, dt, 'grad_embeddings'), int(B), int(D), int(Cc), int(L), float(S), int(H),
                 _opt(dy_dx, dt, 'dy_dx'), _opt(grad_inputs, dt, 'grad_inputs'), int(gridtype), int(bool(align_corners)),
                 int(interp)]
        if fp32:
            args += [None if scratch is None else scratch.data_ptr(), 0 if scratch is None else scratch.numel() * 8]
        rc = getattr(_lib.lib(), 'occnerf_grid_encode_backward' + _ENCODER_ENTRY[dt])(*args, _stream(inputs))
    _lib.check(rc, 'grid_encode_backward')


def grad_total_variation(inputs, embeddings, grad, offsets, weight, B, D, Cc, L, S, H, gridtype=0,
                         align_corners=False):
    rc = _lib.lib().occnerf_grad_total_variation(None, None, None, None, float(weight), int(B), int(D),
                                                 int(Cc), int(L), float(S), int(H), int(gridtype),
                                                 int(bool(align_corners)), None)
    _lib.check(rc, 'grad_total_variation')


def _host_f64(vals, n):
    a = np.ascontiguousarray(np.asarray(vals, dtype=np.float64).ravel())
    assert a.size == n, (a.size, n)
    return a, a.ctypes.data_as(C.c_void_p)


def gen_rays(K, E, H, W, bbox_min, bbox_max, device, out=None):
    dev = torch.device(device)
    if dev.type != 'cuda':
        raise RuntimeError(f'gen_rays: needs a GPU device, got {dev}')
    f32 = int(np.asarray(K).dtype == np.float32 and np.asarray(E).dtype == np.float32)
    E = np.asarray(E, dtype=np.float64)
    k0, pk = _host_f64(np.linalg.inv(np.asarray(K)).astype(np.float64), 9)
    r0, pr = _host_f64(E[:3, :3], 9)
    t0, pt = _host_f64(E[:3, 3], 3)
    l0, pl = _host_f64(bbox_min, 3)
    h0, ph = _host_f64(bbox_max, 3)
    if out is None:
        rays8 = torch.empty(H * W, 8, device=dev, dtype=torch.float32)
        mask = torch.empty(H * W, device=dev, dtype=torch.uint8)
    else:
        rays8, mask = out
        _chk(rays8, torch.float32, 'rays8'), _chk(mask, torch.uint8, 'mask')
        if rays8.numel() != H * W * 8 or mask.numel() != H * W or rays8.device != mask.device:
            raise RuntimeError(f'gen_rays: out must be rays8[{H * W},8] and mask[{H * W}] on one device')
    with _guard_dev(rays8.device):
        rc = _lib.lib().occnerf_gen_rays(pk, pr, pt, f32, int(H), int(W), pl, ph, rays8.data_ptr(),
                                         mask.data_ptr(), _stream(rays8))
    _lib.check(rc, 'gen_rays')
    return rays8, mask


def bone_boxes(vol, nb):
    boxes = torch.empty(nb, 6, device=vol.device, dtype=torch.int32)
    with _guard(vol):
        rc = _lib.lib().occnerf_bone_boxes(_chk(vol, torch.float32, 'vol'), int(nb), int(vol.shape[-1]), boxes.data_ptr(), _stream(vol))
    _lib.check(rc, 'bone_boxes')
    return boxes


def sample_warp(rays8, S, t_vals, Rs, Ts, vol, bbox_min, bbox_scale, t_rand=None, want_pts=False, boxes=None):
    n = rays8.shape[0]
    dev = rays8.device
    if boxes is not None and t_rand is None and not want_pts:
        z = torch.empty(n, S, device=dev, dtype=torch.float32)
        xs = torch.empty(n * S, 3, device=dev, dtype=torch.float32)
        mk = torch.empty(n * S, device=dev, dtype=torch.float32)
        _kmin, pmin = _host_f32(bbox_min, 3)
        _ksc, psc = _host_f32(bbox_scale, 3)
        with _guard_dev(dev):
            rc = _lib.lib().occnerf_sample_warp_culled(
                _chk(rays8, torch.float32, 'rays'), n, int(S), _chk(t_vals, torch.float32, 't_vals'),
                _chk(Rs, torch.float32, 'Rs'), _chk(Ts, torch.float32, 'Ts'), _chk(vol, torch.float32, 'vol'), int(Rs.shape[0]),
                int(vol.shape[-1]), _chk(boxes, torch.int32, 'boxes'), pmin, psc, z.data_ptr(), xs.data_ptr(), mk.data_ptr(),
                _stream(rays8))
        _lib.check(rc, 'sample_warp_culled')
        return z, xs, mk, None
    z = torch.empty(n, S, device=dev, dtype=torch.float32)
    xs = torch.empty(n * S, 3, device=dev, dtype=torch.float32)
    mk = torch.empty(n * S, device=dev, dtype=torch.float32)
    pts = torch.empty(n * S, 3, device=dev, dtype=torch.float32) if want_pts else None
    _kmin, pmin = _host_f32(bbox_min, 3)
    _ksc, psc = _host_f32(bbox_scale, 3)
    with _guard_dev(dev):
        rc = _lib.lib().occnerf_sample_warp(
            _chk(rays8, torch.float32, 'rays'), n, int(S), _chk(t_vals, torch.float32, 't_vals'),
            _opt(t_rand, torch.float32, 't_rand'), _chk(Rs, torch.float32, 'Rs'),
            _chk(Ts, torch.float32, 'Ts'), _chk(vol, torch.float32, 'vol'), int(Rs.shape[0]),
            int(vol.shape[-1]), pmin, psc, z.data_ptr(), None if pts is None else pts.data_ptr(),
            xs.data_ptr(), mk.data_ptr(), _stream(rays8))
    _lib.check(rc, 'sample_warp')
    return z, xs, mk, pts


def nonrigid_pack(weights, biases):
    dev = weights[0].device
    n = _lib.lib().occnerf_nonrigid_packed_floats()
    packed = torch.zeros(n, device=dev, dtype=torch.float32)
    with _guard_dev(dev):
        rc = _lib.lib().occnerf_nonrigid_pack(_ptr_table(weights, 'W'), _ptr_table(biases, 'b'),
                                              packed.data_ptr(), _stream(packed))
    _lib.check(rc, 'nonrigid_pack')
    return packed


def nonrigid(xyz, cond, hann, W0, b0, packed, out=None, direct=False):
    out = torch.empty_like(xyz) if out is None else out
    _kh, ph = _host_f32(hann, 6)
    fn = _lib.lib().occnerf_nonrigid_direct if direct else _lib.lib().occnerf_nonrigid
    with _guard(xyz):
        rc = fn(
            _chk(xyz, torch.float32, 'xyz'), xyz.shape[0], _chk(cond, torch.float32, 'cond'), ph,
            _chk(W0, torch.float32, 'W0'), _chk(b0, torch.float32, 'b0'),
            _chk(packed, torch.float32, 'packed'), _chk(out, torch.float32, 'xyz_out'), _stream(xyz))
    _lib.check(rc, 'nonrigid')
    return out


def nonrigid_rows(xyz, rows, count, cond, hann, W0, b0, packed):
    _kh, ph = _host_f32(hann, 6)
    with _guard(xyz):
        rc = _lib.lib().occnerf_nonrigid_rows(
            _chk(xyz, torch.float32, 'xyz'), rows.shape[0], _chk(rows, torch.int32, 'rows'),
            _chk(count, torch.int32, 'count'), _chk(cond, torch.float32, 'cond'), ph,
            _chk(W0, torch.float32, 'W0'), _chk(b0, torch.float32, 'b0'), _chk(packed, torch.float32, 'packed'),
            _stream(xyz))
    _lib.check(rc, 'nonrigid_rows')
    return xyz


def live_rows(mask):
    N = mask.shape[0]
    dev = mask.device
    nbytes = int(_lib.lib().occnerf_live_rows_temp_bytes(N))
    if nbytes < 0:
        raise RuntimeError('live_rows: temp size query failed')
    temp = torch.empty(max(nbytes, 16), device=dev, dtype=torch.uint8)
    rows = torch.empty(N, device=dev, dtype=torch.int32)
    count = torch.empty(1, device=dev, dtype=torch.int32)
    with _guard(mask):
        rc = _lib.lib().occnerf_live_rows(_chk(mask, torch.float32, 'mask'), N, rows.data_ptr(), count.data_ptr(),
                                          temp.data_ptr(), nbytes, _stream(mask))
    _lib.check(rc, 'live_rows')
    return rows, count


def scatter_raw(raw_c, rows, count, raw_full):
    with _guard(raw_c):
        rc = _lib.lib().occnerf_scatter_raw(_chk(raw_c, torch.float32, 'raw_c'), _chk(rows, torch.int32, 'rows'),
                                            _chk(count, torch.int32, 'count'), rows.shape[0],
                                            _chk(raw_full, torch.float32, 'raw_full'), _stream(raw_c))
    _lib.check(rc, 'scatter_raw')
    return raw_full


def repeat_heads(keys, key_cols, count, rows=None, want_mask=False):
    dev = keys.device
    if keys.dim() != 2 or not keys.is_contiguous() or keys.element_size() != 4:
        raise RuntimeError('repeat_heads: keys must be a contiguous [M, C] tensor of 4-byte elements')
    cap = keys.shape[0] if rows is None else rows.shape[0]
    scan = torch.empty(cap, device=dev, dtype=torch.int32)
    heads = torch.empty(cap, device=dev, dtype=torch.int32)
    head_count = torch.empty(1, device=dev, dtype=torch.int32)
    head_mask = torch.zeros(keys.shape[0], device=dev, dtype=torch.float32) if want_mask else None
    if cap == 0:
        head_count.zero_()
        return scan, heads, head_count, head_mask
    nbytes = int(_lib.lib().occnerf_repeat_heads_temp_bytes(cap))
    if nbytes < 0:
        raise RuntimeError('repeat_heads: temp size query failed')
    temp = torch.empty(max(nbytes, 16), device=dev, dtype=torch.uint8)
    with _guard_dev(dev):
        rc = _lib.lib().occnerf_repeat_heads(
            keys.data_ptr(), keys.shape[1], int(key_cols), _opt(rows, torch.int32, 'rows'),
            _chk(count, torch.int32, 'count'), cap, scan.data_ptr(), heads.data_ptr(), head_count.data_ptr(),
            None if head_mask is None else head_mask.data_ptr(), temp.data_ptr(), nbytes, _stream(keys))
    _lib.check(rc, 'repeat_heads')
    return scan, heads, head_count, head_mask


def unique_heads(keys, key_cols, heads, count, scan=None, scan_count=None):
    dev = keys.device
    if keys.dim() != 2 or not keys.is_contiguous() or keys.element_size() != 4:
        raise RuntimeError('unique_heads: keys must be a contiguous [M, C] tensor of 4-byte elements')
    cap = keys.shape[0] if heads is None else heads.shape[0]
    heads_out = torch.empty(cap, device=dev, dtype=torch.int32)
    count_out = torch.empty(1, device=dev, dtype=torch.int32)
    if cap == 0:
        count_out.zero_()
        return heads_out, count_out
    nbytes = int(_lib.lib().occnerf_unique_heads_temp_bytes(cap))
    if nbytes <= 0:
        raise RuntimeError('unique_heads: temp size query failed')
    temp = torch.empty(nbytes, device=dev, dtype=torch.uint8)
    with _guard_dev(dev):
        rc = _lib.lib().occnerf_unique_heads(
            keys.data_ptr(), keys.shape[1], int(key_cols), _opt(heads, torch.int32, 'heads'),
            _chk(count, torch.int32, 'count'), cap, heads_out.data_ptr(), count_out.data_ptr(),
            _opt(scan, torch.int32, 'scan'), _opt(scan_count, torch.int32, 'scan_count'),
            0 if scan is None else scan.shape[0], temp.data_ptr(), nbytes, _stream(keys))
    _lib.check(rc, 'unique_heads')
    return heads_out, count_out


def scatter_raw_heads(raw_h, raw_c, rows, count, scan_a, scan_b, raw_full):
    with _guard(raw_c):
        rc = _lib.lib().occnerf_scatter_raw_heads(
            _chk(raw_h, torch.float32, 'raw_h'), _chk(raw_c, torch.float32, 'raw_c'), _chk(rows, torch.int32, 'rows'),
            _chk(count, torch.int32, 'count'), _opt(scan_a, torch.int32, 'scan_a'), _opt(scan_b, torch.int32, 'scan_b'),
            rows.shape[0], _chk(raw_full, torch.float32, 'raw_full'), _stream(raw_c))
    _lib.check(rc, 'scatter_raw_heads')
    return raw_full


def nonrigid_pack_bf16(weights):
    dev = weights[0].device
    n = _lib.lib().occnerf_nonrigid_packed_bf16_bytes()
    packed = torch.zeros(n // 2, device=dev, dtype=torch.bfloat16)
    with _guard_dev(dev):
        rc = _lib.lib().occnerf_nonrigid_pack_bf16(_ptr_table(weights[:6], 'W'), packed.data_ptr(), _stream(packed))
    _lib.check(rc, 'nonrigid_pack_bf16')
    return packed


def nonrigid_pack_f16(weights):
    dev = weights[0].device
    n = _lib.lib().occnerf_nonrigid_packed_bf16_bytes()
    packed = torch.zeros(n // 2, device=dev, dtype=torch.float16)
    with _guard_dev(dev):
        rc = _lib.lib().occnerf_nonrigid_pack_f16(_ptr_table(weights[:6], 'W'), packed.data_ptr(), _stream(packed))
    _lib.check(rc, 'nonrigid_pack_f16')
    return packed


def _nonrigid_f16x3(xyz, rows, count, cond, hann, W0, b0, packed, packed_f16, out, domain_flag=None):
    _kh, ph = _host_f32(hann, 6)
    n_max = xyz.shape[0] if rows is None else rows.shape[0]
    with _guard(xyz):
        rc = _lib.lib().occnerf_nonrigid_f16x3(
            _chk(xyz, torch.float32, 'xyz'), n_max, _opt(rows, torch.int32, 'rows'), _opt(count, torch.int32, 'count'),
            _chk(cond, torch.float32, 'cond'), ph, _chk(W0, torch.float32, 'W0'), _chk(b0, torch.float32, 'b0'),
            _chk(packed, torch.float32, 'packed'), _chk(packed_f16, torch.float16, 'packed_f16'),
            _chk(out, torch.float32, 'xyz_out'), _opt(domain_flag, torch.int32, 'domain_flag'), _stream(xyz))
    _lib.check(rc, 'nonrigid_f16x3')
    return out


def nonrigid_bf16x3(xyz, cond, hann, W0, b0, packed, packed_bf16, out=None, domain_flag=None):
    out = torch.empty_like(xyz) if out is None else out
    if packed_bf16.dtype == torch.float16:
        return _nonrigid_f16x3(xyz, None, None, cond, hann, W0, b0, packed, packed_bf16, out, domain_flag)
    _kh, ph = _host_f32(hann, 6)
    with _guard(xyz):
        rc = _lib.lib().occnerf_nonrigid_bf16x3(
            _chk(xyz, torch.float32, 'xyz'), xyz.shape[0], _chk(cond, torch.float32, 'cond'), ph,
            _chk(W0, torch.float32, 'W0'), _chk(b0, torch.float32, 'b0'), _chk(packed, torch.float32, 'packed'),
            _chk(packed_bf16, torch.bfloat16, 'packed_bf16'), _chk(out, torch.float32, 'xyz_out'), _stream(xyz))
    _lib.check(rc, 'nonrigid_bf16x3')
    return out


def nonrigid_bf16x3_rows(xyz, rows, count, cond, hann, W0, b0, packed, packed_bf16, domain_flag=None):
    if packed_bf16.dtype == torch.float16:
        return _nonrigid_f16x3(xyz, rows, count, cond, hann, W0, b0, packed, packed_bf16, xyz, domain_flag)
    _kh, ph = _host_f32(hann, 6)
    with _guard(xyz):
        rc = _lib.lib().occnerf_nonrigid_bf16x3_rows(
            _chk(xyz, torch.float32, 'xyz'), rows.shape[0], _chk(rows, torch.int32, 'rows'), _chk(count, torch.int32, 'count'),
            _chk(cond, torch.float32, 'cond'), ph, _chk(W0, torch.float32, 'W0'), _chk(b0, torch.float32, 'b0'),
            _chk(packed, torch.float32, 'packed'), _chk(packed_bf16, torch.bfloat16, 'packed_bf16'), _stream(xyz))
    _lib.check(rc, 'nonrigid_bf16x3_rows')
    return xyz


def msknn(xyz, points, index_map, scale_begin, seed_from_coarser):
    N = xyz.shape[0]
    nscale = len(scale_begin) - 1
    out = torch.empty(N, nscale, 10, device=xyz.device, dtype=torch.int32)
    _kb, pb = _host_i32(scale_begin)
    _ks, ps = _host_i32(seed_from_coarser)
    with _guard(xyz):
        rc = _lib.lib().occnerf_msknn(_chk(xyz, torch.float32, 'xyz'), N,
                                      _chk(points, torch.float32, 'points'),
                                      _chk(index_map, torch.int32, 'index_map'), pb, ps, nscale,
                                      out.data_ptr(), _stream(xyz))
    _lib.check(rc, 'msknn')
    return out


def knn_center(c, points, index_map, scale_begin):
    nscale = len(scale_begin) - 1
    center = torch.empty(4, device=c.device, dtype=torch.float32)
    idx = torch.empty(nscale, 10, device=c.device, dtype=torch.int32)
    _kb, pb = _host_i32(scale_begin)
    with _guard(c):
        rc = _lib.lib().occnerf_knn_center(_chk(c, torch.float32, 'c'), _chk(points, torch.float32, 'points'),
                                           _chk(index_map, torch.int32, 'index_map'), pb, nscale, center.data_ptr(), idx.data_ptr(),
                                           _stream(c))
    _lib.check(rc, 'knn_center')
    return center, idx


def msknn_clustered(xyz, n_rays, S, cl, seed_from_coarser, mask=None, rows=None, count=None, out=None, center=None):
    nscale = int(cl['ranges'].shape[0]) + 1
    if out is None:
        out = torch.empty(n_rays * S, nscale, 10, device=xyz.device, dtype=torch.int32)
    if (rows is None) != (count is None) or (rows is not None and mask is not None):
        raise RuntimeError('msknn_clustered: rows and count come together, instead of mask')
    ray_start = torch.empty(n_rays + 1, device=xyz.device, dtype=torch.int32) if rows is not None else None
    _kc, pc = _host_i32(cl['coarse_rows'])
    _ks, ps = _host_i32(seed_from_coarser)
    with _guard(xyz):
        rc = _lib.lib().occnerf_msknn_clustered_centered(
            _chk(xyz, torch.float32, 'xyz'), _opt(mask, torch.float32, 'mask'), int(n_rays), int(S),
            _chk(cl['points'], torch.float32, 'points'), _chk(cl['centers'], torch.float32, 'centers'), _chk(cl['ranges'], torch.int32, 'cluster_ranges'),
            _chk(cl['radius'], torch.float32, 'cluster_radius'), int(cl['ncl']),
            _opt(cl.get('group_centers'), torch.float32, 'group_centers'), _opt(cl.get('group_ranges'), torch.int32, 'group_ranges'),
            _opt(cl.get('group_radius'), torch.float32, 'group_radius'), int(cl.get('ngrp', 0)), pc, ps, nscale,
            _opt(rows, torch.int32, 'rows'), _opt(count, torch.int32, 'count'),
            None if ray_start is None else ray_start.data_ptr(),
            None if center is None else _chk(center[0], torch.float32, 'center'),
            None if center is None else _chk(center[1], torch.int32, 'center_idx'), out.data_ptr(), _stream(xyz))
    _lib.check(rc, 'msknn_clustered')
    return out


def knn_small(q, s, k):
    out = torch.empty(q.shape[0], k, device=q.device, dtype=torch.int32)
    with _guard(q):
        rc = _lib.lib().occnerf_knn_small(_chk(q, torch.float32, 'q'), q.shape[0],
                                          _chk(s, torch.float32, 's'), s.shape[0], int(k),
                                          out.data_ptr(), _stream(q))
    _lib.check(rc, 'knn_small')
    return out


def unit_normals(normals):
    out = torch.empty_like(normals)
    with _guard(normals):
        rc = _lib.lib().occnerf_unit_normals(_chk(normals, torch.float64, 'normals'), normals.shape[0],
                                             out.data_ptr(), _stream(normals))
    _lib.check(rc, 'unit_normals')
    return out


def point_sdf(point_cloud, point_base, normals, unit, kidx):
    P = point_cloud.shape[0]
    kb = torch.empty(P, 3, device=point_cloud.device, dtype=torch.float64)
    dist = torch.empty(P, device=point_cloud.device, dtype=torch.float32)
    with _guard(point_cloud):
        rc = _lib.lib().occnerf_point_sdf(
            _chk(point_cloud, torch.float32, 'point_cloud'), _chk(point_base, torch.float32, 'point_base'),
            _chk(normals, torch.float64, 'normals'), _chk(unit, torch.float64, 'unit_normals'),
            _chk(kidx, torch.int32, 'kidx'), P, kb.data_ptr(), dist.data_ptr(), _stream(point_cloud))
    _lib.check(rc, 'point_sdf')
    return kb, dist


def table_stride():
    return int(_lib.lib().occnerf_point_table_stride())


def point_table(knn_base, sdf, learnable, bound32, two_bound32, embeddings, offsets, S, H):
    P = knn_base.shape[0]
    table = torch.empty(P, table_stride(), device=knn_base.device, dtype=torch.float32)
    with _guard(knn_base):
        rc = _lib.lib().occnerf_point_table(
            _chk(knn_base, torch.float64, 'knn_base'), _chk(sdf, torch.float32, 'point_sdf'),
            _chk(learnable, torch.float32, 'learnable'), P, float(bound32), float(two_bound32),
            _chk(embeddings, torch.float32, 'embeddings'), _chk(offsets, torch.int32, 'offsets'),
            _host_offsets(offsets), int(offsets.shape[0] - 1), float(S), int(H), table.data_ptr(),
            _stream(knn_base))
    _lib.check(rc, 'point_table')
    return table


def point_pack(point_base, normals, unit, counter, table):
    P, dev = point_base.shape[0], point_base.device
    geo = torch.empty(P, 16, device=dev, dtype=torch.float32)
    tail = torch.empty(P, 4, device=dev, dtype=torch.float32)
    with _guard_dev(dev):
        rc = _lib.lib().occnerf_point_pack(
            _chk(point_base, torch.float32, 'point_base'), _chk(normals, torch.float64, 'normals'),
            _chk(unit, torch.float64, 'unit_normals'), _chk(counter, torch.float32, 'counter'),
            _chk(table, torch.float32, 'table'), P, geo.data_ptr(), tail.data_ptr(), _stream(point_base))
    _lib.check(rc, 'point_pack')
    return geo, tail


def center_row(mlp_in_row, enc_in_row):
    return torch.cat([mlp_in_row[:36], enc_in_row[:4], mlp_in_row[36:68]]).contiguous()


def sample_features(xyz, knn_idxs, point_base, normals, unit, counter, table, bound32, two_bound32,
                    embeddings, offsets, S, H, raw=None, want_enc_in=False, geo_idxs=None,
                    att_in=None, rows=None, count=None, pack=None, center=None, center_agg=None):
    N = xyz.shape[0] if rows is None else rows.shape[0]
    dev = xyz.device
    if (pack is None and N > 0 and knn_idxs.shape[1] == 4 and geo_idxs is None and att_in is None
            and counter is not None and table.dim() == 2 and table.shape[1] == table_stride()):
        pack = point_pack(point_base, normals, unit, counter, table)
    geo, tail = pack if pack is not None else (None, None)
    if table.dim() != 2 or table.shape[1] != table_stride():
        raise RuntimeError(f'sample_features: table must be [P,{table_stride()}] (ops.point_table), got {tuple(table.shape)}')
    mlp_in = torch.empty(N, 68, device=dev, dtype=torch.float32)
    raw = torch.empty(N, 5, device=dev, dtype=torch.float32) if raw is None else raw
    enc_in = torch.empty(N, 4, device=dev, dtype=torch.float32) if want_enc_in else None
    with _guard_dev(dev):
        rc = _lib.lib().occnerf_sample_features_centered(
            _chk(xyz, torch.float32, 'xyz'), N, _chk(knn_idxs, torch.int32, 'knn_idxs'),
            int(knn_idxs.shape[1]), _chk(point_base, torch.float32, 'point_base'),
            _chk(normals, torch.float64, 'normals'), _chk(unit, torch.float64, 'unit_normals'),
            _opt(counter, torch.float32, 'counter'), _chk(table, torch.float32, 'table'),
            float(bound32), float(two_bound32), _chk(embeddings, torch.float32, 'embeddings'),
            _chk(offsets, torch.int32, 'offsets'), _host_offsets(offsets), int(offsets.shape[0] - 1),
            float(S), int(H), _opt(geo_idxs, torch.int32, 'geo_idxs'), _opt(att_in, torch.float32, 'att_in'),
            _opt(rows, torch.int32, 'rows'), _opt(count, torch.int32, 'count'),
            _opt(geo, torch.float32, 'point_geo'), _opt(tail, torch.float32, 'point_tail'),
            0 if geo is None else int(geo.shape[0]),
            _opt(center, torch.float32, 'center'), _opt(center_agg, torch.float32, 'center_agg'),
            mlp_in.data_ptr(), _chk(raw, torch.float32, 'raw'),
            None if enc_in is None else enc_in.data_ptr(), _stream(xyz))
    _lib.check(rc, 'sample_features')
    return mlp_in, raw, enc_in


def canonical_mlp_pack(weights, biases):
    dev = weights[0].device
    n = _lib.lib().occnerf_canonical_mlp_packed_floats()
    packed = torch.zeros(n, device=dev, dtype=torch.float32)
    with _guard_dev(dev):
        rc = _lib.lib().occnerf_canonical_mlp_pack(_ptr_table(weights, 'W'), _ptr_table(biases, 'b'),
                                                   packed.data_ptr(), _stream(packed))
    _lib.check(rc, 'canonical_mlp_pack')
    return packed


def canonical_mlp(mlp_in, packed, raw, direct=False, count=None, in_rows=None):
    if in_rows is not None:
        with _guard(mlp_in):
            rc = _lib.lib().occnerf_canonical_mlp_rows(
                _chk(mlp_in, torch.float32, 'mlp_in'), _chk(in_rows, torch.int32, 'in_rows'), in_rows.shape[0],
                _chk(count, torch.int32, 'count'), _chk(packed, torch.float32, 'packed'),
                _chk(raw, torch.float32, 'raw'), _stream(mlp_in))
        _lib.check(rc, 'canonical_mlp_rows')
        return raw
    if count is not None:
        with _guard(mlp_in):
            rc = _lib.lib().occnerf_canonical_mlp_counted(
                _chk(mlp_in, torch.float32, 'mlp_in'), mlp_in.shape[0], _chk(count, torch.int32, 'count'),
                _chk(packed, torch.float32, 'packed'), _chk(raw, torch.float32, 'raw'), _stream(mlp_in))
        _lib.check(rc, 'canonical_mlp_counted')
        return raw
    fn = _lib.lib().occnerf_canonical_mlp_direct if direct else _lib.lib().occnerf_canonical_mlp
    with _guard(mlp_in):
        rc = fn(_chk(mlp_in, torch.float32, 'mlp_in'), mlp_in.shape[0], _chk(packed, torch.float32, 'packed'),
                _chk(raw, torch.float32, 'raw'), _stream(mlp_in))
    _lib.check(rc, 'canonical_mlp')
    return raw


def trunks_pack_bf16(weights, out=None):
    dev = weights[0].device
    if out is None:
        out = torch.zeros(_lib.lib().occnerf_trunks_packed_bytes() // 2, device=dev, dtype=torch.bfloat16)
    with _guard_dev(dev):
        rc = _lib.lib().occnerf_trunks_pack_bf16(_ptr_table(weights[:9], 'W'), out.data_ptr(), _stream(out))
    _lib.check(rc, 'trunks_pack_bf16')
    return out


def trunks_forward_bf16(agg, var, enc, packed_f32, packed_bf16):
    M, dev, bf = agg.shape[0], agg.device, torch.bfloat16
    X0 = torch.empty(M, 96, device=dev, dtype=bf)
    A = [torch.empty(M, 256, device=dev, dtype=bf) for _ in range(4)]
    GEO = torch.empty(M, 96, device=dev, dtype=bf)
    B = [torch.empty(M, 256, device=dev, dtype=bf) for _ in range(4)]
    raw4 = torch.empty(M, 4, device=dev, dtype=torch.float32)
    pa = (C.c_void_p * 4)(*[t.data_ptr() for t in A])
    pb = (C.c_void_p * 4)(*[t.data_ptr() for t in B])
    with _guard(agg):
        rc = _lib.lib().occnerf_trunks_forward_bf16(
            _chk(agg, torch.float32, 'agg'), _chk(var, torch.float32, 'var'), _chk(enc, torch.float32, 'enc'), M,
            _chk(packed_f32, torch.float32, 'packed_f32'), _chk(packed_bf16, torch.bfloat16, 'packed_bf16'), X0.data_ptr(), pa,
            GEO.data_ptr(), pb, raw4.data_ptr(), _stream(agg))
    _lib.check(rc, 'trunks_forward_bf16')
    return X0, A, GEO, B, raw4


def canonical_mlp_pack_bf16(weights):
    dev = weights[0].device
    n = _lib.lib().occnerf_canonical_mlp_packed_bf16_bytes()
    packed = torch.zeros(n // 2, device=dev, dtype=torch.bfloat16)
    with _guard_dev(dev):
        rc = _lib.lib().occnerf_canonical_mlp_pack_bf16(_ptr_table(weights, 'W'), packed.data_ptr(),
                                                        _stream(packed))
    _lib.check(rc, 'canonical_mlp_pack_bf16')
    return packed


def canonical_mlp_pack_f16(weights):
    dev = weights[0].device
    n = _lib.lib().occnerf_canonical_mlp_packed_bf16_bytes()
    packed = torch.zeros(n // 2, device=dev, dtype=torch.float16)
    with _guard_dev(dev):
        rc = _lib.lib().occnerf_canonical_mlp_pack_f16(_ptr_table(weights, 'W'), packed.data_ptr(), _stream(packed))
    _lib.check(rc, 'canonical_mlp_pack_f16')
    return packed


def canonical_mlp_bf16x3(mlp_in, packed, packed_bf16, raw, variant=0, count=None, in_rows=None, domain_flag=None):
    if packed_bf16.dtype == torch.float16:
        n_max = mlp_in.shape[0] if in_rows is None else in_rows.shape[0]
        with _guard(mlp_in):
            rc = _lib.lib().occnerf_canonical_mlp_f16x3(
                _chk(mlp_in, torch.float32, 'mlp_in'), _opt(in_rows, torch.int32, 'in_rows'), n_max,
                _opt(count, torch.int32, 'count'), _chk(packed, torch.float32, 'packed'),
                _chk(packed_bf16, torch.float16, 'packed_f16'), _chk(raw, torch.float32, 'raw'),
                _opt(domain_flag, torch.int32, 'domain_flag'), _stream(mlp_in))
        _lib.check(rc, 'canonical_mlp_f16x3')
        return raw
    with _guard(mlp_in):
        if count is None:
            assert in_rows is None
            rc = _lib.lib().occnerf_canonical_mlp_bf16x3(
                _chk(mlp_in, torch.float32, 'mlp_in'), mlp_in.shape[0], _chk(packed, torch.float32, 'packed'),
                _chk(packed_bf16, torch.bfloat16, 'packed_bf16'), _chk(raw, torch.float32, 'raw'),
                int(variant), _stream(mlp_in))
        else:
            n_max = mlp_in.shape[0] if in_rows is None else in_rows.shape[0]
            rc = _lib.lib().occnerf_canonical_mlp_bf16x3_rows(
                _chk(mlp_in, torch.float32, 'mlp_in'), _opt(in_rows, torch.int32, 'in_rows'), n_max,
                _chk(count, torch.int32, 'count'), _chk(packed, torch.float32, 'packed'),
                _chk(packed_bf16, torch.bfloat16, 'packed_bf16'), _chk(raw, torch.float32, 'raw'), int(variant),
                _stream(mlp_in))
    _lib.check(rc, 'canonical_mlp_bf16x3')
    return raw


def composite(raw, mask, z_vals, rays8, bgcolor, want_weights=False, want_term=False, out=None, out_rows=None):
    n, S = z_vals.shape
    dev = raw.device
    if out is None:
        if out_rows is not None:
            raise RuntimeError('composite: out_rows needs caller-allocated outputs')
        out = (torch.empty(n, 3, device=dev, dtype=torch.float32), torch.empty(n, device=dev, dtype=torch.float32),
               torch.empty(n, device=dev, dtype=torch.float32))
    rgb, acc, dep = out
    for t, nm in ((rgb, 'rgb'), (acc, 'acc'), (dep, 'depth')):
        _chk(t, torch.float32, nm)
    w = torch.empty(n, S, device=dev, dtype=torch.float32) if want_weights else None
    tp = torch.empty(n, device=dev, dtype=torch.int32) if want_term else None
    _kbg, pbg = _host_f32(bgcolor, 3)
    with _guard_dev(dev):
        rc = _lib.lib().occnerf_composite(
            _chk(raw, torch.float32, 'raw'), _chk(mask, torch.float32, 'mask'),
            _chk(z_vals, torch.float32, 'z_vals'), _chk(rays8, torch.float32, 'rays'), pbg, n, int(S),
            rgb.data_ptr(), acc.data_ptr(), dep.data_ptr(), None if w is None else w.data_ptr(),
            None if tp is None else tp.data_ptr(), _opt(out_rows, torch.int64, 'out_rows'), _stream(raw))
    _lib.check(rc, 'composite')
    return rgb, acc, dep, w, tp


def pose_motion_bases(pose_decoder, posevec, refine, dst_Rs, dst_Ts, cnl_gtfms):
    import torch.nn as nn
    dev = dst_Rs.device
    lin = [m for m in pose_decoder.block_mlps if isinstance(m, nn.Linear)]
    if len(lin) != 5 or lin[0].in_features != 69 or lin[0].out_features != 256 or lin[4].out_features != 69:
        raise RuntimeError('pose_motion_bases: the fused kernel is built for the 69 -> 256 x4 -> 69 refiner of occnerf.yaml')
    Rs = torch.empty(24, 3, 3, device=dev, dtype=torch.float32)
    Ts = torch.empty(24, 3, device=dev, dtype=torch.float32)
    with _guard_dev(dev):
        rc = _lib.lib().occnerf_pose_motion_bases(
            _ptr_table([m.weight.detach() for m in lin], 'W'), _ptr_table([m.bias.detach() for m in lin], 'b'),
            _chk(posevec, torch.float32, 'posevec'), int(bool(refine)), _chk(dst_Rs, torch.float32, 'dst_Rs'),
            _chk(dst_Ts, torch.float32, 'dst_Ts'), _chk(cnl_gtfms, torch.float32, 'cnl_gtfms'), Rs.data_ptr(),
# ... 323 lines not shown
```

Measured before the change: 1.216 million rays/s.

## Split samples by kNN centre sphere and give near samples a specialised feature kernel

Adds a three-way partition that splits live samples into those inside and outside the cached kNN-centre sphere. Only the far samples go through the full kNN search and sample_features kernel, which now writes to permuted output positions. Near samples go to a new kernel that reuses the cached centre neighbours and aggregate row, and re-encodes the hash grid only when the per-sample input differs from the centre's. This avoids the per-sample kNN search and the full feature work for samples near the centre, at the cost of an extra partition pass, an extra launch and scattered writes.

```diff
diff --git a/include/occnerf_hip.h b/include/occnerf_hip.h
--- a/include/occnerf_hip.h
+++ b/include/occnerf_hip.h
@@ -165,6 +165,23 @@
                             const float *center, const float *center_agg,
                                      float *mlp_in, float *raw, float *enc_in, void *stream);
 
+int occnerf_sample_features_pos(const float *xyz, int64_t N, const int32_t *knn_idxs, int32_t nscale,
+                            const float *point_base, const double *normals,
+                            const double *unit_normals, const float *counter,
+                            const float *table, float bound, float two_bound,
+                            const float *embeddings, const int32_t *offsets,
+                            const int32_t *h_offsets, uint32_t L, float S, uint32_t H,
+                            const int32_t *geo_idxs, const float *att_in, const int32_t *rows,
+                            const int32_t *n_dev, const float *point_geo, const float *point_tail, int32_t P,
+                            const float *center, const float *center_agg, const int32_t *out_pos,
+                            float *mlp_in, float *raw, float *enc_in, void *stream);
+int32_t occnerf_center_features_applies(const int32_t *h_offsets, uint32_t L, float S, uint32_t H);
+int occnerf_center_features(const float *xyz, const int32_t *near_rows, const int32_t *near_pos,
+                            const int32_t *near_count, int64_t cap, const int32_t *center_idx,
+                            const float *center_agg, const float *point_geo, int32_t P, float bound,
+                            float two_bound, const float *embeddings, const int32_t *h_offsets, uint32_t L, float S,
+                            uint32_t H, float *mlp_in, float *raw, float *enc_in, void *stream);
+
 int occnerf_agg_forward(const float *feats, int32_t F, const int32_t *knn, const float *atts, int64_t N, int32_t K,
                         float *agg, void *stream);
 int32_t occnerf_agg_backward_slices(int64_t N);
@@ -177,6 +194,10 @@
                       int64_t temp_bytes, void *stream);
 int occnerf_scatter_raw(const float *raw_c, const int32_t *rows, const int32_t *n_dev, int64_t N_max,
                         float *raw_full, void *stream);
+int64_t occnerf_center_split_temp_bytes(int64_t cap);
+int occnerf_center_split(const float *xyz, const int32_t *rows, const int32_t *n_dev, int64_t cap, const float *center,
+                         int32_t *far_rows, int32_t *far_pos, int32_t *near_rows, int32_t *near_pos, int32_t *counts,
+                         void *temp, int64_t temp_bytes, void *stream);
 
 int64_t occnerf_repeat_heads_temp_bytes(int64_t N_max);
 int occnerf_repeat_heads(const void *keys, int64_t stride_dwords, int32_t key_dwords, const int32_t *rows,
diff --git a/occnerf_amd/_lib.py b/occnerf_amd/_lib.py
--- a/occnerf_amd/_lib.py
+++ b/occnerf_amd/_lib.py
@@ -84,6 +84,14 @@
     'occnerf_sample_features_centered': (C.c_int, [_vp, _i64, _vp, _i32, _vp, _vp, _vp, _vp, _vp, _f32, _f32, _vp,
                                                     _vp, _vp, _u32, _f32, _u32, _vp, _vp, _vp, _vp, _vp, _vp, _i32, _vp, _vp,
                                                     _vp, _vp, _vp, _vp]),
+    'occnerf_sample_features_pos': (C.c_int, [_vp, _i64, _vp, _i32, _vp, _vp, _vp, _vp, _vp, _f32, _f32, _vp,
+                                               _vp, _vp, _u32, _f32, _u32, _vp, _vp, _vp, _vp, _vp, _vp, _i32, _vp, _vp,
+                                               _vp, _vp, _vp, _vp, _vp]),
+    'occnerf_center_features_applies': (_i32, [_vp, _u32, _f32, _u32]),
+    'occnerf_center_features': (C.c_int, [_vp, _vp, _vp, _vp, _i64, _vp, _vp, _vp, _i32, _f32, _f32, _vp, _vp, _u32, _f32,
+                                           _u32, _vp, _vp, _vp, _vp]),
+    'occnerf_center_split_temp_bytes': (_i64, [_i64]),
+    'occnerf_center_split': (C.c_int, [_vp, _vp, _vp, _i64, _vp, _vp, _vp, _vp, _vp, _vp, _vp, _i64, _vp]),
     'occnerf_canonical_mlp_packed_floats': (_i64, []),
     'occnerf_canonical_mlp_pack': (C.c_int, [_vp, _vp, _vp, _vp]),
     'occnerf_canonical_mlp': (C.c_int, [_vp, _i64, _vp, _vp, _vp]),
diff --git a/occnerf_amd/config.py b/occnerf_amd/config.py
--- a/occnerf_amd/config.py
+++ b/occnerf_amd/config.py
@@ -92,6 +92,7 @@
     'ray_patch_order': True,
     'knn_culling': True,
     'knn_center_cache': True,
+    'center_split': True,
     'warp_bone_culling': True,
 }
 
diff --git a/occnerf_amd/csrc/common.h b/occnerf_amd/csrc/common.h
--- a/occnerf_amd/csrc/common.h
+++ b/occnerf_amd/csrc/common.h
@@ -162,6 +162,11 @@
     return sqrtf(__fmaf_rn(z, z, __fmaf_rn(y, y, __fmul_rn(x, x))));
 }
 
+__device__ __forceinline__ bool inside_center(float px, float py, float pz, float cx, float cy, float cz, float r2) {
+    const float dx = px - cx, dy = py - cy, dz = pz - cz;
+    return __builtin_fmaf(dz, dz, __builtin_fmaf(dy, dy, dx * dx)) < r2;
+}
+
 int64_t mlp_lds_packed_floats();
 int mlp_lds_pack(const float *const *h_W, const float *const *h_b, float *packed, hipStream_t st);
 int mlp_lds_launch(const float *mlp_in, const int32_t *in_rows, int64_t N, const int32_t *n_dev, const float *packed,
diff --git a/occnerf_amd/csrc/compact.hip b/occnerf_amd/csrc/compact.hip
--- a/occnerf_amd/csrc/compact.hip
+++ b/occnerf_amd/csrc/compact.hip
@@ -1,6 +1,7 @@
 #include "common.h"
 
 #include <hipcub/hipcub.hpp>
+#include <rocprim/rocprim.hpp>
 
 namespace occ {
 
@@ -8,6 +9,29 @@
     const float *mask;
     __device__ bool operator()(const int &i) const { return mask[i] != 0.0f; }
 };
+
+using SplitEntry = rocprim::tuple<int, int>;
+struct CenterSide {
+    const float *xyz;
+    const int32_t *n_dev;
+    const float *center;
+    bool want_inside;
+    __device__ bool operator()(const SplitEntry &e) const {
+        if (rocprim::get<0>(e) >= *n_dev) return false;
+        const int64_t r = rocprim::get<1>(e);
+        return inside_center(xyz[r * 3], xyz[r * 3 + 1], xyz[r * 3 + 2], center[0], center[1], center[2], center[3]) == want_inside;
+    }
+};
+
+static hipError_t center_split_run(void *temp, size_t &bytes, const float *xyz, const int32_t *rows, const int32_t *n_dev,
+                                   int64_t cap, const float *center, int32_t *far_rows, int32_t *far_pos, int32_t *near_rows,
+                                   int32_t *near_pos, int32_t *counts, hipStream_t st) {
+    auto in = rocprim::make_zip_iterator(rocprim::make_tuple(rocprim::counting_iterator<int>(0), rows));
+    auto far = rocprim::make_zip_iterator(rocprim::make_tuple(far_pos, far_rows));
+    auto near = rocprim::make_zip_iterator(rocprim::make_tuple(near_pos, near_rows));
+    return rocprim::partition_three_way(temp, bytes, in, far, near, rocprim::discard_iterator(), counts, (size_t)cap,
+                                        CenterSide{xyz, n_dev, center, false}, CenterSide{xyz, n_dev, center, true}, st);
+}
 
 __global__ void scatter_raw_kernel(const float *__restrict__ raw_c, const int32_t *__restrict__ rows,
                                    const int32_t *__restrict__ n_dev, float *__restrict__ raw_full) {
@@ -316,3 +340,27 @@
                        raw_full);
     return check_launch("scatter_raw");
 }
+
+OCC_API int64_t occnerf_center_split_temp_bytes(int64_t cap) {
+    using namespace occ;
+    if (cap <= 0 || cap >= (1ll << 31)) return 0;
+    size_t bytes = 0;
+    if (center_split_run(nullptr, bytes, nullptr, nullptr, nullptr, cap, nullptr, nullptr, nullptr, nullptr, nullptr, nullptr,
+                         (hipStream_t)0) != hipSuccess)
+        return -1;
+    return (int64_t)bytes;
+}
+
+OCC_API int occnerf_center_split(const float *xyz, const int32_t *rows, const int32_t *n_dev, int64_t cap, const float *center,
+                                 int32_t *far_rows, int32_t *far_pos, int32_t *near_rows, int32_t *near_pos, int32_t *counts,
+                                 void *temp, int64_t temp_bytes, void *stream) {
+    using namespace occ;
+    OCC_REQUIRE(xyz && rows && n_dev && center && far_rows && far_pos && near_rows && near_pos && counts && temp,
+                "center_split: null argument");
+    OCC_REQUIRE(cap > 0 && cap < (1ll << 31), "center_split: cap=%lld out of range", (long long)cap);
+    size_t bytes = (size_t)temp_bytes;
+    const hipError_t e = center_split_run(temp, bytes, xyz, rows, n_dev, cap, center, far_rows, far_pos, near_rows, near_pos,
+                                          counts, as_stream(stream));
+    OCC_REQUIRE(e == hipSuccess, "center_split: %s", hipGetErrorString(e));
+    return check_launch("center_split");
+}
diff --git a/occnerf_amd/csrc/features.hip b/occnerf_amd/csrc/features.hip
--- a/occnerf_amd/csrc/features.hip
+++ b/occnerf_amd/csrc/features.hip
@@ -394,7 +394,8 @@
     LevelRecs levels, LevelRecs8 levels8, FeatParams prm, const int32_t *__restrict__ rows ,
     const int32_t *__restrict__ n_dev , float *__restrict__ mlp_in, float *__restrict__ raw, float *__restrict__ enc_in_out,
     const float *__restrict__ center ,
-    const float *__restrict__ center_agg ) {
+    const float *__restrict__ center_agg ,
+    const int32_t *__restrict__ out_pos ) {
     constexpr int NK = 4 * kKnn;
     float ccx = 0.f, ccy = 0.f, ccz = 0.f, cr2 = 0.f;
     if (center) ccx = center[0], ccy = center[1], ccz = center[2], cr2 = center[3];
@@ -447,12 +448,12 @@
         const bool live = group0 + it * ngroups < N;
         const int64_t o = out_row(it);
         const int64_t o2 = out_row(it + 2);
-        float *out = mlp_in + o * 68;
+        const int64_t ow = out_pos ? (int64_t)out_pos[o] : o;
+        float *out = mlp_in + ow * 68;
 
         bool cached_agg = false;
         if (cr2 > 0.0f) {
-            const float dx = cur.p[0] - ccx, dy = cur.p[1] - ccy, dz = cur.p[2] - ccz;
-            const bool inside = __builtin_fmaf(dz, dz, __builtin_fmaf(dy, dy, dx * dx)) < cr2;
+            const bool inside = inside_center(cur.p[0], cur.p[1], cur.p[2], ccx, ccy, ccz, cr2);
             cached_agg = __builtin_amdgcn_ballot_w64(live && !inside) == 0;
         }
         float4 tl[5];
@@ -521,8 +522,8 @@
         for (int c = 0; c < 3; c++) x[c] = (float)__ddiv_rn(num[c], den);
         x[3] = nd;
         if (live && g == 0) {
-            raw[o * 5 + 4] = dist;
-            if (enc_in_out) *reinterpret_cast<float4 *>(enc_in_out + o * 4) = make_float4(x[0], x[1], x[2], x[3]);
+            raw[ow * 5 + 4] = dist;
+            if (enc_in_out) *reinterpret_cast<float4 *>(enc_in_out + ow * 4) = make_float4(x[0], x[1], x[2], x[3]);
         }
 
         float a5[5] = {0.f, 0.f, 0.f, 0.f, 0.f};
@@ -681,6 +682,123 @@
     }
 }
 
+constexpr int kCenterThreads = 256;
+
+__global__ __launch_bounds__(kCenterThreads) void center_features_kernel(
+    const float *__restrict__ xyz, const int32_t *__restrict__ near_rows, const int32_t *__restrict__ near_pos,
+    const int32_t *__restrict__ near_count, const int32_t *__restrict__ center_idx ,
+    const float4 *__restrict__ geo , const float4 *__restrict__ center_agg ,
+    const float2 *__restrict__ embeddings, LevelRecs8 levels8, FeatParams prm, float *__restrict__ mlp_in,
+    float *__restrict__ raw, float *__restrict__ enc_in_out) {
+    const int64_t n = (int64_t)*near_count;
+    const int64_t base = (int64_t)blockIdx.x * kCenterThreads;
+    if (base >= n) return;
+    __shared__ float4 s_geo[kKnn * 4];
+    __shared__ float4 s_row[18];
+    __shared__ LevelRec8 s_lv[kMaxLevels];
+    if (threadIdx.x < kKnn * 4) s_geo[threadIdx.x] = geo[(size_t)center_idx[threadIdx.x >> 2] * 4 + (threadIdx.x & 3)];
+    else if (threadIdx.x >= 64 && threadIdx.x < 64 + 18) s_row[threadIdx.x - 64] = center_agg[threadIdx.x - 64];
+    else if (threadIdx.x >= 128 && threadIdx.x < 128 + kMaxLevels) s_lv[threadIdx.x - 128] = levels8.r[threadIdx.x - 128];
+    __syncthreads();
+
+    const int lane = threadIdx.x & 63;
+    const int64_t j = base + threadIdx.x;
+    const bool live = j < n;
+    const int64_t jc = live ? j : n - 1;
+    const int64_t i = near_rows[jc];
+    const int32_t ow = near_pos[jc];
+    struct __attribute__((packed, aligned(4))) F3 { float v[3]; };
+    const F3 pq = *reinterpret_cast<const F3 *>(xyz + i * 3);
+    const float p[3] = {pq.v[0], pq.v[1], pq.v[2]};
+
+    float dsum = 0.0f;
+    int neg = 0;
+    double num[3] = {0.0, 0.0, 0.0}, den = 0.0;
+#pragma unroll
+    for (int k = 0; k < kKnn; k++) {
+        const float4 r0 = s_geo[k * 4], r1 = s_geo[k * 4 + 1], r2 = s_geo[k * 4 + 2], r3 = s_geo[k * 4 + 3];
+        const float nbr[3] = {r0.x, r0.y, r0.z};
+        const double nx = __hiloint2double(__float_as_int(r1.y), __float_as_int(r1.x));
+        const double ny = __hiloint2double(__float_as_int(r1.w), __float_as_int(r1.z));
+        const double nz = __hiloint2double(__float_as_int(r2.y), __float_as_int(r2.x));
+        float dir[3];
+#pragma unroll
+        for (int c = 0; c < 3; c++) dir[c] = __fsub_rn(p[c], nbr[c]);
+        double dot = __dadd_rn(0.0, __dmul_rn((double)dir[0], nx));
+        dot = __dadd_rn(dot, __dmul_rn((double)dir[1], ny));
+        dot = __dadd_rn(dot, __dmul_rn((double)dir[2], nz));
+        neg += dot < 0.0;
+        dsum = __fadd_rn(dsum, norm3(dir[0], dir[1], dir[2]));
+        if (k < 3) {
+            const double un[3] = {__hiloint2double(__float_as_int(r2.w), __float_as_int(r2.z)),
+                                  __hiloint2double(__float_as_int(r3.y), __float_as_int(r3.x)),
+                                  __hiloint2double(__float_as_int(r3.w), __float_as_int(r3.z))};
+            const double att = fabs(cos3_unit(dir, un));
+#pragma unroll
+            for (int c = 0; c < 3; c++) {
+                const float pn = __fdiv_rn(__fadd_rn(nbr[c], prm.bound), prm.two_bound);
+                num[c] = __dadd_rn(num[c], __dmul_rn(att, (double)pn));
+            }
+            den = __dadd_rn(den, att);
+        }
+    }
+    float dist = __fdiv_rn(dsum, (float)kKnn);
+    if (2 * neg > kKnn) dist = -dist;
+    float nd = __fdiv_rn(__fadd_rn(dist, 0.2f), 0.5f);
+    nd = nd < 0.0f ? 0.0f : (nd > 1.0f ? 1.0f : nd);
+    float x[4];
+#pragma unroll
+    for (int c = 0; c < 3; c++) x[c] = (float)__ddiv_rn(num[c], den);
+    x[3] = nd;
+    if (live) {
+        raw[(int64_t)ow * 5 + 4] = dist;
+        if (enc_in_out) *reinterpret_cast<float4 *>(enc_in_out + (int64_t)ow * 4) = make_float4(x[0], x[1], x[2], x[3]);
+    }
+
+    const float4 cx = s_row[9];
+    const bool eq = __float_as_uint(x[0]) == __float_as_uint(cx.x) && __float_as_uint(x[1]) == __float_as_uint(cx.y) &&
+                    __float_as_uint(x[2]) == __float_as_uint(cx.z) && __float_as_uint(x[3]) == __float_as_uint(cx.w);
+    uint64_t own = __builtin_amdgcn_ballot_w64(live && !eq);
+    const int64_t wave_base = base + (threadIdx.x & ~63);
+    const int nlive = (int)(n - wave_base < 64 ? n - wave_base : 64);
+#pragma unroll 1
+    for (int t = 0; t < 17; t++) {
+        const int f = t * 64 + lane;
+        const int s = f / 17, piece = f - s * 17;
+        const int32_t ows = __shfl(ow, s);
+        const bool skip = s >= nlive || (piece >= 9 && ((own >> s) & 1ull));
+        if (!skip) *reinterpret_cast<float4 *>(mlp_in + (int64_t)ows * 68 + piece * 4) = s_row[piece + (piece >= 9)];
+    }
+
+    while (own) {
+        int src[4];
+#pragma unroll
+        for (int q = 0; q < 4; q++) {
+            src[q] = own ? (int)__builtin_ctzll(own) : -1;
+            if (own) own &= own - 1;
+        }
+        const int q = lane >> 4, level = lane & 15;
+        const int sl = q == 0 ? src[0] : (q == 1 ? src[1] : (q == 2 ? src[2] : src[3]));
+        const int slc = sl < 0 ? 0 : sl;
+        float xs[4];
+#pragma unroll
+        for (int d = 0; d < 4; d++) xs[d] = __shfl(x[d], slc);
+        const int32_t ows = __shfl(ow, slc);
+        bool oob = false;
+#pragma unroll
+        for (int d = 0; d < 4; d++) oob |= (xs[d] < 0.f || xs[d] > 1.f);
+        if (oob) {
+#pragma unroll
+            for (int d = 0; d < 4; d++) xs[d] = 0.5f;
+        }
+        LevelTaps4 tp;
+        level_taps_select(xs, embeddings, s_lv[level], tp);
+        float2 ev = encode_level_d4c2_reduce(tp);
+        if (oob) ev = make_float2(0.f, 0.f);
+        if (sl >= 0) *reinterpret_cast<float2 *>(mlp_in + (int64_t)ows * 68 + 36 + 2 * level) = ev;
+    }
+}
+
 
 }
 
@@ -774,6 +892,22 @@
                                              const float *point_geo, const float *point_tail, int32_t P,
                                              const float *center, const float *center_agg,
                                              float *mlp_in, float *raw, float *enc_in, void *stream) {
+    return occnerf_sample_features_pos(xyz, N, knn_idxs, nscale, point_base, normals, unit_normals, counter, table, bound,
+                                       two_bound, embeddings, offsets, h_offsets, L, S, H, geo_idxs, att_in, rows, n_dev,
+                                       point_geo, point_tail, P, center, center_agg, nullptr, mlp_in, raw, enc_in, stream);
+}
+
+OCC_API int occnerf_sample_features_pos(const float *xyz, int64_t N, const int32_t *knn_idxs,
+                                        int32_t nscale, const float *point_base, const double *normals,
+                                        const double *unit_normals, const float *counter,
+                                        const float *table, float bound, float two_bound,
+                                        const float *embeddings, const int32_t *offsets,
+                                        const int32_t *h_offsets, uint32_t L, float S, uint32_t H,
+                                        const int32_t *geo_idxs,
+                                        const float *att_in, const int32_t *rows, const int32_t *n_dev,
+                                        const float *point_geo, const float *point_tail, int32_t P,
+                                        const float *center, const float *center_agg, const int32_t *out_pos,
+                                        float *mlp_in, float *raw, float *enc_in, void *stream) {
     using namespace occ;
     OCC_REQUIRE(!center == !center_agg, "sample_features: center and center_agg come together");
     if (N <= 0) return 0;
@@ -788,6 +922,7 @@
     OCC_REQUIRE(!n_dev || rows, "sample_features: a device-side count needs the row list");
     OCC_REQUIRE(!point_geo == !point_tail, "sample_features: point_geo and point_tail come together (occnerf_point_pack)");
     const bool lanes8 = nscale == 4 && !geo_idxs && !att_in && counter && h_offsets && point_geo;
+    OCC_REQUIRE(!out_pos || rows, "sample_features: output positions come with the row list");
     OCC_REQUIRE(!rows || lanes8,
                 "sample_features: a row list is only supported on the renderer's path (4 scales, per-point inputs, "
                 "packed point records)");
@@ -818,7 +953,7 @@
                            N, knn_idxs, reinterpret_cast<const float4 *>(point_geo),
                            reinterpret_cast<const float4 *>(point_tail),
                            reinterpret_cast<const float4 *>(table), reinterpret_cast<const float2 *>(embeddings),
-                           levels, levels8, prm, rows, n_dev, mlp_in, raw, enc_in, center, center_agg);
+                           levels, levels8, prm, rows, n_dev, mlp_in, raw, enc_in, center, center_agg, out_pos);
         return check_launch("sample_features");
     }
     OCC_REQUIRE(!center, "sample_features: the centre aggregate is only supported on the renderer's path");
@@ -830,3 +965,45 @@
                        offsets, lv, gm, prm, geo_idxs, att_in, mlp_in, raw, enc_in);
     return check_launch("sample_features");
 }
+
+OCC_API int32_t occnerf_center_features_applies(const int32_t *h_offsets, uint32_t L, float S, uint32_t H) {
+    using namespace occ;
+    if (!h_offsets || L != 16) return 0;
+    const GridLevels lv = make_grid_levels(L, S, H);
+    const GridModes4 gm = modes_from_host_offsets(L, lv, h_offsets);
+    for (uint32_t l = 0; l < L; l++)
+        if (gm.mode[l] == kGridGeneric) return 0;
+    return 1;
+}
+
+OCC_API int occnerf_center_features(const float *xyz, const int32_t *near_rows, const int32_t *near_pos,
+                                    const int32_t *near_count, int64_t cap, const int32_t *center_idx,
+                                    const float *center_agg, const float *point_geo, int32_t P, float bound,
+                                    float two_bound, const float *embeddings, const int32_t *h_offsets, uint32_t L, float S,
+                                    uint32_t H, float *mlp_in, float *raw, float *enc_in, void *stream) {
+    using namespace occ;
+    if (cap <= 0) return 0;
+    OCC_REQUIRE(xyz && near_rows && near_pos && near_count && center_idx && center_agg && point_geo && embeddings && h_offsets &&
+                    mlp_in && raw, "center_features: null argument");
+    OCC_REQUIRE(P > 0, "center_features: P=%d rows of packed point records", P);
+    OCC_REQUIRE(occnerf_center_features_applies(h_offsets, L, S, H),
+                "center_features: built for 16 levels that are dense or hashed with a power-of-two size (occnerf_center_features_applies)");
+    const GridLevels lv = make_grid_levels(L, S, H);
+    const GridModes4 gm = modes_from_host_offsets(L, lv, h_offsets);
+    LevelRecs8 levels8;
+    for (uint32_t l = 0; l < kMaxLevels; l++) {
+        const uint32_t size = (uint32_t)(h_offsets[l + 1] - h_offsets[l]), r1 = lv.resolution[l] + 1;
+        const bool dense = gm.mode[l] == kGridDense;
+        levels8.r[l] = LevelRec8{(uint32_t)h_offsets[l], dense ? 0xFFFFFFFFu : size - 1, lv.scale[l], dense ? 1u : 0u,
+                                 dense ? r1 : 2654435761u, dense ? r1 * r1 : 805459861u,
+                                 dense ? r1 * r1 * r1 : 3674653429u, 0u};
+    }
+    FeatParams prm{bound, two_bound, 4, (int)L, (int)P};
+    const int64_t blocks = (cap + kCenterThreads - 1) / kCenterThreads;
+    OCC_REQUIRE(blocks < (1ll << 31), "center_features: list too long");
+    hipLaunchKernelGGL(center_features_kernel, dim3((unsigned)blocks), dim3(kCenterThreads), 0, as_stream(stream), xyz,
+                       near_rows, near_pos, near_count, center_idx, reinterpret_cast<const float4 *>(point_geo),
+                       reinterpret_cast<const float4 *>(center_agg), reinterpret_cast<const float2 *>(embeddings), levels8, prm,
+                       mlp_in, raw, enc_in);
+    return check_launch("center_features");
+}
diff --git a/occnerf_amd/csrc/knn.hip b/occnerf_amd/csrc/knn.hip
--- a/occnerf_amd/csrc/knn.hip
+++ b/occnerf_amd/csrc/knn.hip
@@ -392,9 +392,7 @@
         if (cr2 > 0.0f) {
 #pragma unroll
             for (int a = 0; a < kQ; a++) {
-                const float dx = qx[a >> 1][a & 1] - ccx, dy = qy[a >> 1][a & 1] - ccy, dz = qz[a >> 1][a & 1] - ccz;
-                const float d2 = __builtin_fmaf(dz, dz, __builtin_fmaf(dy, dy, dx * dx));
-                if (live[a] && d2 < cr2) {
+                if (live[a] && inside_center(qx[a >> 1][a & 1], qy[a >> 1][a & 1], qz[a >> 1][a & 1], ccx, ccy, ccz, cr2)) {
                     live[a] = false;
                     struct __attribute__((packed, aligned(4))) I4 { int v[4]; };
                     struct __attribute__((packed, aligned(4))) I2 { int v[2]; };
diff --git a/occnerf_amd/network.py b/occnerf_amd/network.py
--- a/occnerf_amd/network.py
+++ b/occnerf_amd/network.py
@@ -252,6 +252,10 @@
             if cfg.get('dedup_global_positions', False):
                 frows, fcount = ops.unique_heads(xyz, 3, frows, fcount, scan=scan_a, scan_count=count)
         self.last_head_counts = (fcount, None)
+        if (center is not None and len(center) > 2 and pack is not None and cfg.get('center_split', True)
+                and cfg.get('knn_query_list', True)
+                and ops.center_features_applies(enc.offsets, enc.log2_per_level_scale, enc.base_resolution)):
+            return self._stage_features_split(rays8, z, xyz, mask, pk, table, pack, center, rows, count, frows, fcount, scan_a, dedup)
         if cfg.get('knn_query_list', True):
             knn = ops.msknn_clustered(xyz, rays8.shape[0], S, ctx['clusters'], ctx['seed'], rows=frows, count=fcount, center=center)
         else:
@@ -266,6 +270,37 @@
             rows=frows, count=fcount, pack=pack, center=None if center is None else center[0],
             center_agg=None if center is None else center[2])
         del knn
+        if dedup:
+            scan_b, mrows, mcount, _ = ops.repeat_heads(mlp_in, 68, fcount)
+            if cfg.get('dedup_global', True):
+                mrows, mcount = ops.unique_heads(mlp_in, 68, mrows, mcount, scan=scan_b, scan_count=fcount)
+            self.last_head_counts = (fcount, mcount)
+        return {'dedup': dedup, 'rays8': rays8, 'z': z, 'mask': mask, 'rows': rows, 'count': count, 'mlp_in': mlp_in,
+                'raw_c': raw_c, 'scan_a': scan_a, 'scan_b': scan_b, 'mrows': mrows, 'mcount': mcount, 'cnl': pk['cnl'],
+                'cnl_bf16': pk['cnl_bf16'], 'domain_flag': pk['domain_flag'], 'N': xyz.shape[0]}
+
+    def _stage_features_split(self, rays8, z, xyz, mask, pk, table, pack, center, rows, count, frows, fcount, scan_a, dedup):
+        cfg, ctx = self.cfg, self._context()
+        S = int(cfg.N_samples)
+        enc = self.cnl_mlp.module.encoder
+        if len(center) > 3 and center[3] != self._center_stamp(table):
+            raise RuntimeError('stale kNN centre: its cached feature row was computed from another table / counter / embedding '
+                               'version than this frame\'s (ops.sample_features freshness contract)')
+        far_rows, far_pos, far_count, near_rows, near_pos, near_count = ops.center_split(xyz, frows, fcount, center[0])
+        self.last_center_split = (far_count, near_count)
+        knn = ops.msknn_clustered(xyz, rays8.shape[0], S, ctx['clusters'], ctx['seed'], rows=far_rows, count=far_count)
+        cap = frows.shape[0]
+        mlp_in = torch.empty(cap, 68, device=xyz.device, dtype=torch.float32)
+        raw_c = torch.empty(cap, 5, device=xyz.device, dtype=torch.float32)
+        ops.sample_features(
+            xyz, knn, self.point_base.detach(), ctx['normals'], ctx['unit'],
+            self.point_counter.detach(), table, ctx['bound32'], ctx['two_bound32'],
+            enc.embeddings.detach(), enc.offsets, enc.log2_per_level_scale, enc.base_resolution,
+            rows=far_rows, count=far_count, pack=pack, out_pos=far_pos, mlp_in=mlp_in, raw=raw_c)
+        del knn
+        ops.center_features(xyz, near_rows, near_pos, near_count, center[1], center[2], pack, ctx['bound32'], ctx['two_bound32'],
+                            enc.embeddings.detach(), enc.offsets, enc.log2_per_level_scale, enc.base_resolution, mlp_in, raw_c)
+        scan_b = mrows = mcount = None
         if dedup:
             scan_b, mrows, mcount, _ = ops.repeat_heads(mlp_in, 68, fcount)
             if cfg.get('dedup_global', True):
diff --git a/occnerf_amd/ops.py b/occnerf_amd/ops.py
--- a/occnerf_amd/ops.py
+++ b/occnerf_amd/ops.py
@@ -278,6 +278,24 @@
     return rows, count
 
 
+def center_split(xyz, rows, count, center):
+    cap, dev = rows.shape[0], rows.device
+    far_rows, far_pos, near_rows, near_pos = (torch.empty(cap, device=dev, dtype=torch.int32) for _ in range(4))
+    counts = torch.zeros(2, device=dev, dtype=torch.int32)
+    if cap > 0:
+        nbytes = int(_lib.lib().occnerf_center_split_temp_bytes(cap))
+        if nbytes < 0:
+            raise RuntimeError('center_split: temp size query failed')
+        temp = torch.empty(max(nbytes, 16), device=dev, dtype=torch.uint8)
+        with _guard(xyz):
+            rc = _lib.lib().occnerf_center_split(
+                _chk(xyz, torch.float32, 'xyz'), _chk(rows, torch.int32, 'rows'), _chk(count, torch.int32, 'count'), cap,
+                _chk(center, torch.float32, 'center'), far_rows.data_ptr(), far_pos.data_ptr(), near_rows.data_ptr(),
+                near_pos.data_ptr(), counts.data_ptr(), temp.data_ptr(), nbytes, _stream(xyz))
+        _lib.check(rc, 'center_split')
+    return far_rows, far_pos, counts[0:1], near_rows, near_pos, counts[1:2]
+
+
 def scatter_raw(raw_c, rows, count, raw_full):
     with _guard(raw_c):
         rc = _lib.lib().occnerf_scatter_raw(_chk(raw_c, torch.float32, 'raw_c'), _chk(rows, torch.int32, 'rows'),
@@ -527,7 +545,8 @@
 
 def sample_features(xyz, knn_idxs, point_base, normals, unit, counter, table, bound32, two_bound32,
                     embeddings, offsets, S, H, raw=None, want_enc_in=False, geo_idxs=None,
-                    att_in=None, rows=None, count=None, pack=None, center=None, center_agg=None):
+                    att_in=None, rows=None, count=None, pack=None, center=None, center_agg=None, out_pos=None, mlp_in=None,
+                    enc_in=None):
     N = xyz.shape[0] if rows is None else rows.shape[0]
     dev = xyz.device
     if (pack is None and N > 0 and knn_idxs.shape[1] == 4 and geo_idxs is None and att_in is None
@@ -536,11 +555,16 @@
     geo, tail = pack if pack is not None else (None, None)
     if table.dim() != 2 or table.shape[1] != table_stride():
         raise RuntimeError(f'sample_features: table must be [P,{table_stride()}] (ops.point_table), got {tuple(table.shape)}')
-    mlp_in = torch.empty(N, 68, device=dev, dtype=torch.float32)
+    if out_pos is not None and (rows is None or out_pos.shape[0] != rows.shape[0]):
+        raise RuntimeError('sample_features: out_pos comes with rows, one position per listed sample')
+    mlp_in = torch.empty(N, 68, device=dev, dtype=torch.float32) if mlp_in is None else mlp_in
     raw = torch.empty(N, 5, device=dev, dtype=torch.float32) if raw is None else raw
-    enc_in = torch.empty(N, 4, device=dev, dtype=torch.float32) if want_enc_in else None
-    with _guard_dev(dev):
-        rc = _lib.lib().occnerf_sample_features_centered(
+    if enc_in is None:
+        enc_in = torch.empty(N, 4, device=dev, dtype=torch.float32) if want_enc_in else None
+    if mlp_in.shape != (N, 68) or raw.shape != (N, 5) or (enc_in is not None and enc_in.shape != (N, 4)):
+        raise RuntimeError(f'sample_features: outputs must have {N} rows')
+    with _guard_dev(dev):
+        rc = _lib.lib().occnerf_sample_features_pos(
             _chk(xyz, torch.float32, 'xyz'), N, _chk(knn_idxs, torch.int32, 'knn_idxs'),
             int(knn_idxs.shape[1]), _chk(point_base, torch.float32, 'point_base'),
             _chk(normals, torch.float64, 'normals'), _chk(unit, torch.float64, 'unit_normals'),
@@ -552,9 +576,35 @@
             _opt(geo, torch.float32, 'point_geo'), _opt(tail, torch.float32, 'point_tail'),
             0 if geo is None else int(geo.shape[0]),
             _opt(center, torch.float32, 'center'), _opt(center_agg, torch.float32, 'center_agg'),
-            mlp_in.data_ptr(), _chk(raw, torch.float32, 'raw'),
-            None if enc_in is None else enc_in.data_ptr(), _stream(xyz))
+            _opt(out_pos, torch.int32, 'out_pos'),
+            _chk(mlp_in, torch.float32, 'mlp_in'), _chk(raw, torch.float32, 'raw'),
+            _opt(enc_in, torch.float32, 'enc_in'), _stream(xyz))
     _lib.check(rc, 'sample_features')
+    return mlp_in, raw, enc_in
+
+
+def center_features_applies(offsets, S, H):
+    return bool(_lib.lib().occnerf_center_features_applies(_host_offsets(offsets), int(offsets.shape[0] - 1), float(S), int(H)))
+
+
+def center_features(xyz, near_rows, near_pos, near_count, center_idx, center_agg, pack, bound32, two_bound32, embeddings,
+                    offsets, S, H, mlp_in, raw, enc_in=None):
+    geo = pack[0]
+    M = mlp_in.shape[0]
+    if near_rows.shape[0] > M or near_pos.shape[0] != near_rows.shape[0] or raw.shape[0] != M or \
+            (enc_in is not None and enc_in.shape[0] != M):
+        raise RuntimeError('center_features: the lists hold at most one entry per output row')
+    if center_agg.shape != (72,) or center_idx.numel() < 10:
+        raise RuntimeError('center_features: center_agg is ops.center_row (72 floats), center_idx ops.knn_center\'s idx')
+    with _guard(xyz):
+        rc = _lib.lib().occnerf_center_features(
+            _chk(xyz, torch.float32, 'xyz'), _chk(near_rows, torch.int32, 'near_rows'), _chk(near_pos, torch.int32, 'near_pos'),
+            _chk(near_count, torch.int32, 'near_count'), near_rows.shape[0], _chk(center_idx, torch.int32, 'center_idx'),
+            _chk(center_agg, torch.float32, 'center_agg'), _chk(geo, torch.float32, 'point_geo'), int(geo.shape[0]),
+            float(bound32), float(two_bound32), _chk(embeddings, torch.float32, 'embeddings'), _host_offsets(offsets),
+            int(offsets.shape[0] - 1), float(S), int(H), _chk(mlp_in, torch.float32, 'mlp_in'), _chk(raw, torch.float32, 'raw'),
+            _opt(enc_in, torch.float32, 'enc_in'), _stream(xyz))
+    _lib.check(rc, 'center_features')
     return mlp_in, raw, enc_in
 
 
```

Result: no change. 1.223 million rays/s (median of 6 runs) (+0.6%).
